# andrewcsmith/vox_box.rs

Hardware: AMD Instinct MI355X
Metric: frames/sec (pitch+LPC+formants), 48 kHz 25 ms/10 ms hop, 1→8 MI355X (higher is better)
Workload: dtype f64

## Files before the change

vox_box.rs_amd/csrc/k_spectral.hip:

```cpp
#include "vbx_spectral_1200.hpp"

namespace vbx {

static size_t spectral_lds_bytes(int n) {
    size_t need = (size_t)pitch_refine_lds_bytes(n);
    const size_t t2_end = (size_t)SP_T2_LDS_OFFSET + 60 * sizeof(double2);
    if (t2_end > need) need = t2_end;
    return (need + 15) & ~(size_t)15;
}

int spectral_plan(int n) {
    static const int min_n = [] { const char *e = getenv("VBX_SPECTRAL_MIN_N"); return e ? atoi(e) : SPECTRAL_MIN_N; }();
    if (n < min_n || n < 64) return SPECTRAL_PLAN_NONE;
    if (n <= 1024) return SPECTRAL_PLAN_1024;
    if (n <= SP_N) return SPECTRAL_PLAN_1200;
    if (n <= 2048) return SPECTRAL_PLAN_2048;
    if (n <= 4096) return SPECTRAL_PLAN_4096;
    return SPECTRAL_PLAN_NONE;
}

int spectral_plan_nc(int plan) {
    return plan == SPECTRAL_PLAN_1200 ? SP_N : plan == SPECTRAL_PLAN_1024 ? 1024 : plan == SPECTRAL_PLAN_2048 ? 2048 :
           plan == SPECTRAL_PLAN_4096 ? 4096 : 0;
}

int spectral_tab_complex(int plan) {
    return plan == SPECTRAL_PLAN_1200 ? SPECTRAL_TAB_COMPLEX : spectral_pow2_tab_complex(plan);
}

void spectral_fill_tab(int plan, double *h) {
    if (plan != SPECTRAL_PLAN_1200) { spectral_pow2_fill_tab(plan, h); return; }
    const long double two_pi = 6.283185307179586476925286766559005768L;
    size_t o = 0;
    auto put = [&](long num, long den) {
        const long double ang = two_pi * (long double)(num % den) / (long double)den;
        h[o++] = (double)cosl(ang); h[o++] = (double)(-sinl(ang));
    };
    for (long np = 0; np < 60; np++) for (long ka = 0; ka < 20; ka++) put(np * ka, 1200);
    for (long c = 0; c < 3; c++) for (long kb = 0; kb < 20; kb++) put(c * kb, 60);
    for (long m = 0; m <= 600; m++) put(m, 2400);
}

bool spectral_supported(int n, int lpc_order, int mfcc_nb, int mfcc_b_lo, int num_coeffs) {
    const int plan = spectral_plan(n);
    if (plan == SPECTRAL_PLAN_NONE) return false;
    if (lpc_order != 0 && lpc_order != SP_LPC_P) return false;
    if (num_coeffs != 0 && ((2 * spectral_plan_nc(plan)) % n != 0 || (n & 1) || num_coeffs > 64 || mfcc_nb < 1 || mfcc_b_lo < 0 || mfcc_b_lo + mfcc_nb > n / 2)) return false;
    return true;
}

int spectral_plan_mfcc(int n) {
    const int plan = spectral_plan(n);
    if (plan == SPECTRAL_PLAN_NONE) return plan;
    if ((2 * spectral_plan_nc(plan)) % n == 0) return plan;
    if (n <= SP_N && (2 * SP_N) % n == 0 && !(n & 1)) return SPECTRAL_PLAN_1200;
    return plan;
}
bool spectral_supported_plan(int plan, int n, int lpc_order, int mfcc_nb, int mfcc_b_lo, int num_coeffs) {
    if (plan == SPECTRAL_PLAN_NONE || n > spectral_plan_nc(plan)) return false;
    if (lpc_order != 0 && lpc_order != SP_LPC_P) return false;
    if (num_coeffs != 0 && ((2 * spectral_plan_nc(plan)) % n != 0 || (n & 1) || num_coeffs > 64 || mfcc_nb < 1 || mfcc_b_lo < 0 || mfcc_b_lo + mfcc_nb > n / 2)) return false;
    return true;
}

static void mfcc_interp_geom(int plan, long *M, int *nt, int *lds_cap) {
    *M = 2L * spectral_plan_nc(plan);
    *nt = plan == SPECTRAL_PLAN_4096 ? 128 : 64;
    *lds_cap = (plan == SPECTRAL_PLAN_1200 || plan == SPECTRAL_PLAN_1024) ? (160 * 1024) / 11 : plan == SPECTRAL_PLAN_2048 ? (160 * 1024) / 7 : (160 * 1024) / 4;
}
static int mfcc_interp_slots(int plan, int nb) { long M; int nt, cap; mfcc_interp_geom(plan, &M, &nt, &cap); return (nb + nt - 1) / nt; }

int mfcc_interp_taps(int plan, int n) {
    long M; int nt, cap; mfcc_interp_geom(plan, &M, &nt, &cap);
    const double tau = 0.5 - (double)n / (2.0 * (double)M);
#ifdef VBX_EXP_INTERP_FEWER_TAPS
    return tau >= 0.36 ? 24 : tau >= 0.268 ? 32 : MFCC_INTERP_MAX_TAPS;
#endif
    return tau >= 0.401 ? 24 : tau >= 0.298 ? 32 : MFCC_INTERP_MAX_TAPS;
}

size_t mfcc_interp_table_bytes(int plan, int nb) {
    long M; int nt, cap; mfcc_interp_geom(plan, &M, &nt, &cap);
    const size_t slots = (size_t)mfcc_interp_slots(plan, nb);
    return (size_t)(M / 4 + 1) * 16 + slots * (MFCC_INTERP_MAX_TAPS / 2) * nt * 16 + slots * nt * 4;
}
size_t mfcc_interp_coef_offset(int plan) { return (size_t)(2L * spectral_plan_nc(plan) / 4 + 1) * 16; }
size_t mfcc_interp_j0_offset(int plan, int nb) {
    long M; int nt, cap; mfcc_interp_geom(plan, &M, &nt, &cap);
    return mfcc_interp_coef_offset(plan) + (size_t)mfcc_interp_slots(plan, nb) * (MFCC_INTERP_MAX_TAPS / 2) * nt * 16;
}

bool mfcc_interp_fill(int plan, int n, int b_lo, int nb, void *h_table, mfcc_interp_t *d) {
    if (plan == SPECTRAL_PLAN_NONE) return false;
    long M; int NT, cap;
    mfcc_interp_geom(plan, &M, &NT, &cap);
    const long quarter = M / 4;
    if (n < 2 || 2L * n > M || M % n == 0 || nb < 1 || nb > 4096 || b_lo < 0) return false;
    const int SL = mfcc_interp_slots(plan, nb);
    const int W = mfcc_interp_taps(plan, n), HT = W / 2;
    const long double pi = 3.141592653589793238462643383279502884L;
    const long double tau = 0.5L - (long double)n / (2.0L * (long double)M);
    const long double beta = pi * tau * (long double)W;
    auto sinhc = [](long double s) { return s < 1e-6L ? 1.0L + s * s / 6.0L : sinhl(s) / s; };
    const long double norm = sinhc(beta);
    char *base = static_cast<char *>(h_table);
    double *rot = reinterpret_cast<double *>(base);
    double *coef = reinterpret_cast<double *>(base + mfcc_interp_coef_offset(plan));
    int32_t *j0t = reinterpret_cast<int32_t *>(base + mfcc_interp_j0_offset(plan, nb));
    for (long j = 0; j <= quarter; j++) {
        const long double ang = 2.0L * pi * (long double)((j * (long)(n - 1)) % (2 * M)) / (long double)(2 * M);
        rot[2 * j] = (double)cosl(ang); rot[2 * j + 1] = (double)sinl(ang);
    }
    long jmin = 1L << 40, jmax = -(1L << 40);
    for (int i = 0; i < nb; i++) {
        const long first = ((long)(b_lo + i) * M) / n - W / 2 + 1;
        if (first < jmin) jmin = first;
        if (first + W - 1 > jmax) jmax = first + W - 1;
    }
    if (jmax > quarter || jmin < -quarter) return false;
    for (int i = 0; i < NT * SL; i++) {
        const int u = i / NT, th = i % NT;
        const long k = b_lo + i;
        const long first = (i < nb) ? (k * M) / n - W / 2 + 1 : jmin;
        j0t[i] = (int32_t)(first - jmin);
        for (int t = 0; t < W; t++) {
            long double c = 0.0L;
            if (i < nb) {
                const long num = k * M - (first + t) * (long)n;
                if (num == 0) c = 1.0L;
                else {
                    const long double nu = (long double)num / (long double)n;
                    long r = num % (2L * n); if (r < 0) r += 2L * n;
                    const long double sn = sinl(pi * (long double)r / (long double)n);
                    const long double arg = beta * beta - (2.0L * pi * tau * nu) * (2.0L * pi * tau * nu);
                    const long double bump = sinhc(arg > 0.0L ? sqrtl(arg) : 0.0L) / norm;
                    c = sn / (pi * nu) * bump;
                }
            }
            coef[(((size_t)u * HT + t / 2) * NT + th) * 2 + (t & 1)] = (double)c;
        }
    }
    const int zn = (int)(jmax - jmin + 1), nbp = (nb + 1) & ~1;
    d->jmin = (int)jmin; d->jmax = (int)jmax; d->taps = W;
    d->pu_off = 2 * zn;
    d->lds_bytes = (2 * zn + 2 * nbp + 64) * 8;
    d->rot = nullptr; d->coef = nullptr; d->j0 = nullptr;
    return d->lds_bytes <= cap;
}

bool spectral_list_parked(const spectral_launch_t &L) {
    const bool rows16 = (((uintptr_t)L.out_cand) & 15) == 0 && (L.cand_ld & 1) == 0;
    return L.plan == SPECTRAL_PLAN_1200 && pitch_full_list_bytes(L.n, L.kmax) != 0 && L.kmax >= pitch_full_list_entries(L.n) &&
           L.out_r == nullptr && !L.mfcc_only && rows16;
}

int launch_analyze(hipStream_t s, const spectral_launch_t &L) {
    if (L.x.kind != SAMPLE_F64 && (L.plan != SPECTRAL_PLAN_1200 || L.n != SP_N)) return -1;
    spectral_args_t a;
    a.frames = static_cast<const double *>(L.x.p);
    a.n_frames = L.F; a.stride = L.stride; a.window = L.window; a.lag_window = L.lag_window;
    a.tab = reinterpret_cast<const double2 *>(L.tab);
    a.n = L.n;
    a.pp.sample_rate = L.sample_rate; a.pp.threshold = L.threshold; a.pp.fmin = L.fmin; a.pp.fmax = L.fmax; a.pp.kmax = L.kmax; a.pp.f32 = 0;
    a.out_cand = reinterpret_cast<double *>(L.out_cand); a.cand_ld = L.cand_ld; a.out_count = L.out_count;
    a.pitch_status = L.pitch_status; a.work = L.work;
    a.out_lpc = L.out_lpc; a.lpc_ld = L.lpc_ld;
    a.out_mfcc = L.out_mfcc; a.mfcc_ld = L.mfcc_ld; a.mfcc_status = L.mfcc_status;
    a.bins = L.bins; a.slopes = L.slopes; a.dct = L.dct; a.num_coeffs = L.num_coeffs; a.nb = L.nb;
    a.unsure_list = L.unsure_list; a.unsure_count = L.unsure_count;
    a.out_r = L.out_r; a.n_lags = L.n_lags;
    a.pcm = (L.x.kind == SAMPLE_PCM16 ? SP_FLAG_PCM : 0) | (L.lag_rcp ? SP_FLAG_LAG_RCP : 0) | ((L.mfcc_defer && L.num_coeffs <= 16) ? SP_FLAG_MFCC_DEFER : 0);
    a.mfcc_q = (L.plan != SPECTRAL_PLAN_NONE && L.n > 0) ? (2 * spectral_plan_nc(L.plan)) / L.n : 2;
    a.ip = mfcc_interp_t{};
    if (L.plan != SPECTRAL_PLAN_1200) return launch_analyze_pow2(s, L, a);
    const dim3 grid((unsigned)L.F), block(64);
    const size_t base = spectral_lds_bytes(L.n);
    size_t extra = pitch_full_list_bytes(L.n, L.kmax);
    a.pp.full_off = extra ? (int)base : 0;
    if (spectral_list_parked(L)) { a.pp.full_off = -1; extra = 0; }
    const size_t lds = base + extra;
    const bool lpc = L.out_lpc != nullptr, mf = L.out_mfcc != nullptr;
    if (L.mfcc_only) {
        if (L.interp && L.n != SP_N) {
            a.ip = L.ip;
            const size_t li = spectral_lds_bytes(0) > (size_t)L.ip.lds_bytes ? spectral_lds_bytes(0) : (((size_t)L.ip.lds_bytes + 15) & ~(size_t)15);
            hipLaunchKernelGGL((analyze_kernel<false, true, false, SP_MFCC_ONLY_INTERP>), grid, block, li, s, a);
        } else hipLaunchKernelGGL((analyze_kernel<false, true, true, SP_MFCC_ONLY>), grid, block, spectral_lds_bytes(0), s, a);
        return 0;
    }
    if (L.out_r != nullptr) {
        if (L.n == SP_N) hipLaunchKernelGGL((analyze_kernel<false, false, true, SP_AC_ONLY>), grid, block, spectral_lds_bytes(0), s, a);
        else hipLaunchKernelGGL((analyze_kernel<false, false, false, SP_AC_ONLY>), grid, block, spectral_lds_bytes(0), s, a);
        return 0;
    }
    static const bool want3 = [] { const char *e = getenv("VBX_SPECTRAL_W3"); return e == nullptr || atoi(e) != 0; }();
    const bool w3 = want3 && extra == 0 && 12 * lds <= 160 * 1024;
    if (L.x.kind == SAMPLE_F32) {
        launch_analyze_f32in(s, a, (unsigned)L.F, lds, lpc, mf, w3);
        return 0;
    }
#define VBX_SP_LAUNCH(LPC_, MF_, FULL_)                                                                              \
    do {                                                                                                              \
        if (w3) hipLaunchKernelGGL((analyze_kernel<LPC_, MF_, FULL_, SP_ANALYZE, 3>), grid, block, lds, s, a);        \
        else hipLaunchKernelGGL((analyze_kernel<LPC_, MF_, FULL_>), grid, block, lds, s, a);                          \
    } while (0)
    if (L.interp && mf && L.n != SP_N) {
        a.ip = L.ip;
        const size_t li = lds > (size_t)L.ip.lds_bytes ? lds : (((size_t)L.ip.lds_bytes + 15) & ~(size_t)15);
        const bool w3i = want3 && extra == 0 && 12 * li <= 160 * 1024;
        if (lpc) { if (w3i) hipLaunchKernelGGL((analyze_kernel<true, true, false, SP_ANALYZE_INTERP, 3>), grid, block, li, s, a);
                   else hipLaunchKernelGGL((analyze_kernel<true, true, false, SP_ANALYZE_INTERP>), grid, block, li, s, a); }
        else { if (w3i) hipLaunchKernelGGL((analyze_kernel<false, true, false, SP_ANALYZE_INTERP, 3>), grid, block, li, s, a);
               else hipLaunchKernelGGL((analyze_kernel<false, true, false, SP_ANALYZE_INTERP>), grid, block, li, s, a); }
    } else if (L.n != SP_N) {
        if (lpc && mf) VBX_SP_LAUNCH(true, true, false);
        else if (mf) VBX_SP_LAUNCH(false, true, false);
        else if (lpc) VBX_SP_LAUNCH(true, false, false);
        else VBX_SP_LAUNCH(false, false, false);
    } else if (lpc && mf) VBX_SP_LAUNCH(true, true, true);
    else if (lpc) VBX_SP_LAUNCH(true, false, true);
    else if (mf) VBX_SP_LAUNCH(false, true, true);
    else VBX_SP_LAUNCH(false, false, true);
#undef VBX_SP_LAUNCH
    return 0;
}

}
```

vox_box.rs_amd/csrc/k_spectral_f32in.hip:

```cpp
#include "vbx_spectral_1200.hpp"

namespace vbx {

void launch_analyze_f32in(hipStream_t s, const spectral_args_t &a, unsigned grid, size_t lds, bool lpc, bool mfcc, bool waves3) {
    const dim3 g(grid), b(64);
#define VBX_SP32_LAUNCH(LPC_, MF_)                                                                                \
    do {                                                                                                           \
        if (waves3) hipLaunchKernelGGL((analyze_kernel<LPC_, MF_, true, SP_ANALYZE, 3, float>), g, b, lds, s, a);                     \
        else hipLaunchKernelGGL((analyze_kernel<LPC_, MF_, true, SP_ANALYZE, VBX_SPECTRAL_WAVES, float>), g, b, lds, s, a);           \
    } while (0)
    if (lpc && mfcc) VBX_SP32_LAUNCH(true, true);
    else if (lpc) VBX_SP32_LAUNCH(true, false);
    else if (mfcc) VBX_SP32_LAUNCH(false, true);
    else VBX_SP32_LAUNCH(false, false);
#undef VBX_SP32_LAUNCH
}

}
```

vox_box.rs_amd/csrc/vbx_api.hip:

```cpp
#include "vbx_ctx.hpp"

#include <cmath>
#include <cstdio>
#include <cstdlib>
#include <cstring>
#include <dlfcn.h>
#include <string>
#include <vector>

using namespace vbx;

extern "C" const double VBX_MALE_FORMANT_ESTIMATES[4] = {320., 1440., 2760., 3200.};
extern "C" const double VBX_FEMALE_FORMANT_ESTIMATES[4] = {480., 1760., 3200., 3520.};

namespace {

thread_local std::string g_last_error;

}

namespace vbx {

int fail(vbx_ctx *ctx, int code, const std::string &msg) {
    g_last_error = msg;
    if (ctx) ctx->last_error = msg;
    return code;
}

int check_launch(vbx_ctx *ctx, const char *what) {
    hipError_t e = hipGetLastError();
    if (e != hipSuccess) return fail(ctx, VBX_E_RUNTIME, std::string(what) + " launch: " + hipGetErrorString(e));
    return VBX_SUCCESS;
}

int ws_get(vbx_ctx *ctx, int slot, size_t bytes, void **out) {
    if (bytes == 0) bytes = 16;
    if (ctx->ws_bytes[slot] < bytes) {
        if (ctx->ws[slot]) {
            VBX_HIP(ctx, hipStreamSynchronize(ctx->stream));
            if (ctx->side) VBX_HIP(ctx, hipStreamSynchronize(ctx->side));
            if (ctx->trk) VBX_HIP(ctx, hipStreamSynchronize(ctx->trk));
            VBX_HIP(ctx, hipFree(ctx->ws[slot]));
            ctx->ws[slot] = nullptr; ctx->ws_bytes[slot] = 0;
        }
        size_t cap = bytes + bytes / 8;
        VBX_HIP(ctx, hipMalloc(&ctx->ws[slot], cap));
        ctx->ws_bytes[slot] = cap;
    }
    *out = ctx->ws[slot];
    return VBX_SUCCESS;
}

int get_bins_dev(vbx_ctx *ctx, size_t n, size_t k, double lo, double hi, double sr,
                 const int32_t **out, std::vector<int32_t> &host_bins, bool &bad) {
    mel_bins_host(n, k, lo, hi, sr, host_bins, bad);
    for (size_t i = 0; i + 1 < host_bins.size(); i++) if (host_bins[i + 1] < host_bins[i]) bad = true;
    if (host_bins.back() > (int32_t)n) bad = true;
    VBX_HIP(ctx, ctx->tables.bins(n, k, lo, hi, sr, host_bins, out));
    return VBX_SUCCESS;
}

int check_frames(vbx_ctx *ctx, const char *fn, const void *x, size_t n_frames, size_t frame_len, size_t stride,
                 size_t max_len) {
    if (!ctx) return fail(nullptr, VBX_E_INVALID, std::string(fn) + ": null context");
    ctx->lpc_list_armed = false;
    ctx->path_last = false;
    ctx->shard.live = false;
    if (n_frames == 0) return 1;
    if (!x) return fail(ctx, VBX_E_INVALID, std::string(fn) + ": null frame pointer");
    if (frame_len < 1 || frame_len > max_len)
        return fail(ctx, VBX_E_INVALID, std::string(fn) + ": frame_len must be in [1, " + std::to_string(max_len) + "]");
    if (stride < 1) return fail(ctx, VBX_E_INVALID, std::string(fn) + ": stride must be >= 1");
    if (n_frames > 0x7fffffffull) return fail(ctx, VBX_E_INVALID, std::string(fn) + ": too many frames for one launch");
    return VBX_SUCCESS;
}

int stage_upload(vbx_ctx *ctx, int which, int ws_slot, const void *h_src, size_t bytes, hipStream_t st, void **d_out) {
    void *d = nullptr;
    const bool grown = ctx->ws_bytes[ws_slot] < bytes;
    int rc = ws_get(ctx, ws_slot, bytes, &d);
    if (rc != VBX_SUCCESS) return rc;
    *d_out = d;
    std::vector<char> &have = ctx->staged[which];
    if (!grown && have.size() == bytes && std::memcmp(have.data(), h_src, bytes) == 0) return VBX_SUCCESS;
    if (!ctx->stage_ev[which]) VBX_HIP(ctx, hipEventCreateWithFlags(&ctx->stage_ev[which], hipEventDisableTiming));
    else VBX_HIP(ctx, hipEventSynchronize(ctx->stage_ev[which]));
    if (ctx->stage_cap[which] < bytes) {
        if (ctx->stage[which]) VBX_HIP(ctx, hipHostFree(ctx->stage[which]));
        ctx->stage[which] = nullptr; ctx->stage_cap[which] = 0;
        VBX_HIP(ctx, hipHostMalloc(&ctx->stage[which], bytes + bytes / 2, hipHostMallocDefault));
        ctx->stage_cap[which] = bytes + bytes / 2;
    }
    std::memcpy(ctx->stage[which], h_src, bytes);
    VBX_HIP(ctx, hipMemcpyAsync(d, ctx->stage[which], bytes, hipMemcpyHostToDevice, st));
    VBX_HIP(ctx, hipEventRecord(ctx->stage_ev[which], st));
    have.assign((const char *)h_src, (const char *)h_src + bytes);
    return VBX_SUCCESS;
}

int upload_segments(vbx_ctx *ctx, hipStream_t st, const int64_t *h_seg, size_t n_seg, size_t n_frames, const int64_t **d_seg, size_t *n_out) {
    if (h_seg == nullptr || n_seg == 0) { *d_seg = nullptr; *n_out = 1; return VBX_SUCCESS; }
    if (h_seg[0] != 0) return fail(ctx, VBX_E_INVALID, "seg_start[0] must be 0");
    for (size_t i = 1; i < n_seg; i++)
        if (h_seg[i] < h_seg[i - 1] || (size_t)h_seg[i] > n_frames) return fail(ctx, VBX_E_INVALID, "seg_start must ascend within [0, n_frames]");
    void *d = nullptr;
    int rc = stage_upload(ctx, 0, vbx_ctx::WS_SEG, h_seg, n_seg * sizeof(int64_t), st, &d);
    if (rc != VBX_SUCCESS) return rc;
    *d_seg = (const int64_t *)d; *n_out = n_seg;
    return VBX_SUCCESS;
}

int upload_estimates(vbx_ctx *ctx, hipStream_t st, const vbx_resonance *h_est, size_t n_est, const res_t **d_est) {
    void *d = nullptr;
    int rc = stage_upload(ctx, 1, vbx_ctx::WS_EST, h_est, n_est * sizeof(vbx_resonance), st, &d);
    if (rc != VBX_SUCCESS) return rc;
    *d_est = (const res_t *)d;
    return VBX_SUCCESS;
}

}

extern "C" {

int vbx_internal_fail(vbx_ctx *ctx, int code, const char *msg) { return fail(ctx, code, msg ? msg : ""); }
void *vbx_internal_stream(vbx_ctx *ctx) { return ctx ? (void *)ctx->stream : nullptr; }

int vbx_abi_version(void) { return VBX_ABI_VERSION; }

int vbx_ctx_set_lpc_policy(vbx_ctx *ctx, int policy) {
    VBX_REQUIRE(ctx, ctx != nullptr, "null context");
    VBX_REQUIRE(ctx, policy == VBX_LPC_POLICY_EXACT || policy == VBX_LPC_POLICY_PLAIN || policy == VBX_LPC_POLICY_REFERENCE,
                "vbx_ctx_set_lpc_policy: unknown policy");
    ctx->lpc_policy = policy;
    return VBX_SUCCESS;
}

int vbx_ctx_get_lpc_policy(const vbx_ctx *ctx, int *h_policy) {
    if (!ctx || !h_policy) return fail(const_cast<vbx_ctx *>(ctx), VBX_E_INVALID, "vbx_ctx_get_lpc_policy: null argument");
    *h_policy = ctx->lpc_policy;
    return VBX_SUCCESS;
}

int vbx_ctx_create(vbx_ctx **out, int device, void *hip_stream) {
    if (!out) return fail(nullptr, VBX_E_INVALID, "vbx_ctx_create: null out");
    *out = nullptr;
    int count = 0;
    hipError_t e = hipGetDeviceCount(&count);
    if (e != hipSuccess || count <= 0)
        return fail(nullptr, VBX_E_NODEVICE, "vbx_ctx_create: no HIP device (this library has no CPU fallback)");
    if (device < 0 || device >= count) return fail(nullptr, VBX_E_INVALID, "vbx_ctx_create: bad device ordinal");
    VBX_HIP(nullptr, hipSetDevice(device));
    hipDeviceProp_t prop;
    VBX_HIP(nullptr, hipGetDeviceProperties(&prop, device));
    if (std::strncmp(prop.gcnArchName, "gfx950", 6) != 0)
        return fail(nullptr, VBX_E_NODEVICE, std::string("vbx_ctx_create: device is ") + prop.gcnArchName + ", kernels are built for gfx950 only");
    vbx_ctx *ctx = new vbx_ctx();
    ctx->device = device;
    ctx->arch = prop.gcnArchName;
    ctx->cu_count = prop.multiProcessorCount;
    { const char *e = std::getenv("VBX_MFCC_GOERTZEL"); ctx->mfcc_force_goertzel = e && e[0] == '1'; }
    { const char *e = std::getenv("VBX_MFCC_DFT2"); ctx->mfcc_force_dft2 = e && e[0] == '1'; }
    { const char *e = std::getenv("VBX_MFCC_MFMA"); ctx->mfcc_force_mfma = e && e[0] == '1'; }
    { const char *e = std::getenv("VBX_MFCC_CZT"); ctx->mfcc_czt = e ? (e[0] == '1' ? 1 : 0) : -1; }
    { const char *e = std::getenv("VBX_MFCC_DEFER"); ctx->mfcc_defer = (e && e[0] == '0') ? 0 : 1; }
    { const char *e = std::getenv("VBX_LPC_EXACT"); ctx->lpc_policy = (e && e[0] == '0') ? VBX_LPC_POLICY_PLAIN : VBX_LPC_POLICY_EXACT; }
    { const char *e = std::getenv("VBX_POW2_SPLIT"); ctx->pow2_split = e ? (e[0] == '0' ? 0 : 1) : -1; }
    { const char *e = std::getenv("VBX_MFCC_INTERP"); ctx->mfcc_interp = e ? (e[0] == '0' ? 0 : 1) : -1; }
    { const char *e = std::getenv("VBX_MFCC_CZT_SPLIT"); ctx->mfcc_czt_split = e != nullptr && e[0] == '1'; }
    { const char *e = std::getenv("VBX_PITCH_CURVE_CUT"); ctx->pitch_whole_curve = e != nullptr && e[0] == '0'; }
    if (const char *e = std::getenv("VBX_ROCTX"); e != nullptr && e[0] == '1') {
        void *h = dlopen("librocprofiler-sdk-roctx.so", RTLD_NOW | RTLD_GLOBAL);
        if (h == nullptr) h = dlopen("libroctx64.so", RTLD_NOW | RTLD_GLOBAL);
        if (h != nullptr) {
            ctx->roctx_push = reinterpret_cast<int (*)(const char *)>(dlsym(h, "roctxRangePushA"));
            ctx->roctx_pop = reinterpret_cast<int (*)()>(dlsym(h, "roctxRangePop"));
            if (ctx->roctx_push == nullptr || ctx->roctx_pop == nullptr) { ctx->roctx_push = nullptr; ctx->roctx_pop = nullptr; }
        }
    }
    { const char *e = std::getenv("VBX_PITCH_MFMA"); ctx->pitch_force_mfma = e && e[0] == '1'; }
    if (hip_stream) { ctx->stream = (hipStream_t)hip_stream; ctx->owns_stream = false; }
    else {
        e = hipStreamCreateWithFlags(&ctx->stream, hipStreamNonBlocking);
        if (e != hipSuccess) { delete ctx; return fail(nullptr, VBX_E_RUNTIME, "hipStreamCreate failed"); }
        ctx->owns_stream = true;
    }
    hipEventCreate(&ctx->t0);
    hipEventCreate(&ctx->t1);
    *out = ctx;
    return VBX_SUCCESS;
}

void vbx_ctx_destroy(vbx_ctx *ctx) {
    if (!ctx) return;
    hipSetDevice(ctx->device);
    hipStreamSynchronize(ctx->stream);
    for (int i = 0; i < vbx_ctx::WS_N; i++) if (ctx->ws[i]) hipFree(ctx->ws[i]);
    if (ctx->pitch_work) hipFree(ctx->pitch_work);
    if (ctx->stitch_state) hipFree(ctx->stitch_state);
    ctx->tables.clear();
    for (auto &r : ctx->recs) { hipEventDestroy(r.a); hipEventDestroy(r.b); }
    if (ctx->side) { hipStreamSynchronize(ctx->side); hipStreamDestroy(ctx->side); }
    if (ctx->ev_fork) hipEventDestroy(ctx->ev_fork);
    if (ctx->ev_join) hipEventDestroy(ctx->ev_join);
    if (ctx->ev_peak) hipEventDestroy(ctx->ev_peak);
    for (auto &e : ctx->ev_slice) if (e) hipEventDestroy(e);
    if (ctx->ev_trk) hipEventDestroy(ctx->ev_trk);
    if (ctx->trk) { hipStreamSynchronize(ctx->trk); hipStreamDestroy(ctx->trk); }
    if (ctx->copy) { hipStreamSynchronize(ctx->copy); hipStreamDestroy(ctx->copy); }
    for (int i = 0; i < 2; i++) {
        if (ctx->host_raw[i]) hipFree(ctx->host_raw[i]);
        if (ctx->host_ready[i]) hipEventDestroy(ctx->host_ready[i]);
        if (ctx->host_freed[i]) hipEventDestroy(ctx->host_freed[i]);
    }
    for (int i = 0; i < vbx_ctx::N_STAGE; i++) { if (ctx->stage[i]) hipHostFree(ctx->stage[i]); if (ctx->stage_ev[i]) hipEventDestroy(ctx->stage_ev[i]); }
    if (ctx->t0) hipEventDestroy(ctx->t0);
    if (ctx->t1) hipEventDestroy(ctx->t1);
    if (ctx->owns_stream) hipStreamDestroy(ctx->stream);
    delete ctx;
}

int vbx_sync(vbx_ctx *ctx) {
    if (!ctx) return fail(nullptr, VBX_E_INVALID, "vbx_sync: null context");
    VBX_HIP(ctx, hipStreamSynchronize(ctx->stream));
    if (ctx->side) VBX_HIP(ctx, hipStreamSynchronize(ctx->side));
    if (ctx->trk) VBX_HIP(ctx, hipStreamSynchronize(ctx->trk));
    if (ctx->copy) VBX_HIP(ctx, hipStreamSynchronize(ctx->copy));
    return VBX_SUCCESS;
}

const char *vbx_last_error(const vbx_ctx *ctx) { return ctx ? ctx->last_error.c_str() : g_last_error.c_str(); }

int vbx_device_info(const vbx_ctx *ctx, char *h_name, size_t name_cap, int *h_cu_count) {
    if (!ctx) return fail(nullptr, VBX_E_INVALID, "vbx_device_info: null context");
    if (h_name && name_cap) { std::strncpy(h_name, ctx->arch.c_str(), name_cap - 1); h_name[name_cap - 1] = 0; }
    if (h_cu_count) *h_cu_count = ctx->cu_count;
    return VBX_SUCCESS;
}

int vbx_malloc(vbx_ctx *ctx, void **out_dptr, size_t bytes) {
    VBX_REQUIRE(ctx, ctx && out_dptr, "null argument");
    VBX_HIP(ctx, hipSetDevice(ctx->device));
    VBX_HIP(ctx, hipMalloc(out_dptr, bytes ? bytes : 16));
    return VBX_SUCCESS;
}
int vbx_free(vbx_ctx *ctx, void *dptr) {
    VBX_REQUIRE(ctx, ctx != nullptr, "null context");
    if (dptr) { VBX_HIP(ctx, hipStreamSynchronize(ctx->stream)); VBX_HIP(ctx, hipFree(dptr)); }
    return VBX_SUCCESS;
}
int vbx_memcpy_h2d(vbx_ctx *ctx, void *dst, const void *h_src, size_t bytes) {
    VBX_REQUIRE(ctx, ctx && (bytes == 0 || (dst && h_src)), "null argument");
    if (bytes == 0) return VBX_SUCCESS;
    VBX_HIP(ctx, hipMemcpyAsync(dst, h_src, bytes, hipMemcpyHostToDevice, ctx->stream));
    VBX_HIP(ctx, hipStreamSynchronize(ctx->stream));
    return VBX_SUCCESS;
}
int vbx_memcpy_d2h(vbx_ctx *ctx, void *h_dst, const void *src, size_t bytes) {
    VBX_REQUIRE(ctx, ctx && (bytes == 0 || (h_dst && src)), "null argument");
    if (bytes == 0) return VBX_SUCCESS;
    VBX_HIP(ctx, hipMemcpyAsync(h_dst, src, bytes, hipMemcpyDeviceToHost, ctx->stream));
    VBX_HIP(ctx, hipStreamSynchronize(ctx->stream));
    return VBX_SUCCESS;
}
int vbx_memset(vbx_ctx *ctx, void *dst, int value, size_t bytes) {
    VBX_REQUIRE(ctx, ctx && (bytes == 0 || dst), "null argument");
    if (bytes == 0) return VBX_SUCCESS;
    VBX_HIP(ctx, hipMemsetAsync(dst, value, bytes, ctx->stream));
    return VBX_SUCCESS;
}

int vbx_timer_begin(vbx_ctx *ctx) {
    VBX_REQUIRE(ctx, ctx != nullptr, "null context");
    VBX_HIP(ctx, hipEventRecord(ctx->t0, ctx->stream));
    return VBX_SUCCESS;
}
int vbx_timer_end(vbx_ctx *ctx, float *h_ms) {
    VBX_REQUIRE(ctx, ctx && h_ms, "null argument");
    VBX_HIP(ctx, hipEventRecord(ctx->t1, ctx->stream));
    VBX_HIP(ctx, hipEventSynchronize(ctx->t1));
    VBX_HIP(ctx, hipEventElapsedTime(h_ms, ctx->t0, ctx->t1));
    return VBX_SUCCESS;
}

static int prof_flush(vbx_ctx *ctx) {
    if (ctx->recs.empty()) return VBX_SUCCESS;
    VBX_HIP(ctx, hipStreamSynchronize(ctx->stream));
    if (ctx->side) VBX_HIP(ctx, hipStreamSynchronize(ctx->side));
    if (ctx->trk) VBX_HIP(ctx, hipStreamSynchronize(ctx->trk));
    for (auto &r : ctx->recs) {
        float ms = 0.f;
        if (hipEventElapsedTime(&ms, r.a, r.b) == hipSuccess) {
            auto &acc = ctx->prof_acc[r.name];
            acc.first += ms; acc.second += 1;
            ctx->prof_stream[r.name] = (r.stream == ctx->stream) ? 0 : (r.stream == ctx->side) ? 1 : 2;
        }
        hipEventDestroy(r.a); hipEventDestroy(r.b);
    }
    ctx->recs.clear();
    return VBX_SUCCESS;
}
int vbx_profile_enable(vbx_ctx *ctx, int on) {
    VBX_REQUIRE(ctx, ctx != nullptr, "null context");
    int rc = prof_flush(ctx);
    ctx->prof = on != 0;
    return rc;
}
int vbx_profile_reset(vbx_ctx *ctx) {
    VBX_REQUIRE(ctx, ctx != nullptr, "null context");
    int rc = prof_flush(ctx);
    ctx->prof_acc.clear();
    ctx->prof_stream.clear();
    if (ctx->pitch_work)
        VBX_HIP(ctx, hipMemsetAsync(ctx->pitch_work, 0, PITCH_WORK_WORDS * sizeof(unsigned long long), ctx->stream));
    return rc;
}
int vbx_profile_pitch_work(vbx_ctx *ctx, uint64_t *h_out4) {
    VBX_REQUIRE(ctx, ctx && h_out4, "null argument");
// ... 16 lines not shown
    return VBX_SUCCESS;
}
int vbx_profile_get(vbx_ctx *ctx, const char *kernel_name, double *h_total_ms, long *h_launches) {
    VBX_REQUIRE(ctx, ctx && kernel_name, "null argument");
    int rc = prof_flush(ctx);
    if (rc != VBX_SUCCESS) return rc;
    auto it = ctx->prof_acc.find(kernel_name);
    if (h_total_ms) *h_total_ms = (it == ctx->prof_acc.end()) ? 0.0 : it->second.first;
    if (h_launches) *h_launches = (it == ctx->prof_acc.end()) ? 0 : it->second.second;
    return VBX_SUCCESS;
}
int vbx_profile_stream(vbx_ctx *ctx, const char *kernel_name, int *h_stream) {
    VBX_REQUIRE(ctx, ctx && kernel_name && h_stream, "null argument");
    int rc = prof_flush(ctx);
    if (rc != VBX_SUCCESS) return rc;
    auto it = ctx->prof_stream.find(kernel_name);
    *h_stream = (it == ctx->prof_stream.end()) ? -1 : it->second;
    return VBX_SUCCESS;
}
int vbx_profile_names(vbx_ctx *ctx, char *h_buf, size_t cap) {
    VBX_REQUIRE(ctx, ctx && h_buf && cap, "null argument");
    int rc = prof_flush(ctx);
    if (rc != VBX_SUCCESS) return rc;
    std::string s;
    for (auto &kv : ctx->prof_acc) { s += kv.first; s += '\n'; }
    std::strncpy(h_buf, s.c_str(), cap - 1); h_buf[cap - 1] = 0;
    return VBX_SUCCESS;
}



static int run_autocorrelate(vbx_ctx *ctx, hipStream_t st, const double *x, size_t n_frames, size_t frame_len, size_t stride,
                             const double *window, size_t n_lags, double *out) {
    if (frame_len > VBX_MAX_FRAME_LEN) {
        void *w = nullptr;
        int rc = ws_get(ctx, vbx_ctx::WS_LONG, autocorr_long_scratch_bytes((long)n_frames, (long)frame_len, (long)n_lags), &w);
        if (rc != VBX_SUCCESS) return rc;
        Prof p(ctx, "autocorr_long", st);
        launch_autocorr_long(st, x, (long)n_frames, (long)frame_len, (long)stride, window, (long)n_lags, out, (double *)w);
        return VBX_SUCCESS;
    }
    if (fewlags_supported((int)frame_len, (int)n_lags, false)) {
        Prof p(ctx, "autocorr_fewlags", st);
        launch_autocorr_fewlags(st, x, (long)n_frames, (int)frame_len, (long)stride, window, (int)n_lags, 0, out, nullptr);
    } else if (!ctx->pitch_force_mfma && spectral_plan((int)frame_len) != SPECTRAL_PLAN_NONE &&
               (n_lags >= SPECTRAL_AC_MIN_LAGS || frame_len >= 1024)) {
        const double *tab = nullptr;
        spectral_launch_t L{};
        L.plan = spectral_plan((int)frame_len); L.n = (int)frame_len;
        VBX_HIP(ctx, ctx->tables.spectral(L.plan, &tab));
        L.x = x; L.F = (long)n_frames; L.stride = (long)stride; L.window = window; L.tab = tab;
        L.out_r = out; L.n_lags = (int)n_lags;
        Prof p(ctx, "autocorr_fft", st);
        launch_analyze(st, L);
    } else {
        Prof p(ctx, "autocorr_tiles", st);
        launch_autocorr_tiles(st, x, (long)n_frames, (int)frame_len, (long)stride, window, (int)n_lags, out);
    }
    return VBX_SUCCESS;
}

int vbx_autocorrelate_f64(vbx_ctx *ctx, const double *x, size_t n_frames, size_t frame_len,
                          size_t stride, const double *window, size_t n_lags, double *out) {
    int rc = check_frames(ctx, __func__, x, n_frames, frame_len, stride, VBX_MAX_LONG_FRAME_LEN);
    if (rc != VBX_SUCCESS) return rc < 0 ? rc : VBX_SUCCESS;
    VBX_REQUIRE(ctx, out != nullptr, "null output");
    VBX_REQUIRE(ctx, n_lags >= 1 && n_lags <= frame_len, "n_lags must be in [1, frame_len] (the reference panics beyond)");
    VBX_HIP(ctx, hipSetDevice(ctx->device));
    if (ctx->lpc_policy == VBX_LPC_POLICY_REFERENCE) {
        VBX_REQUIRE(ctx, frame_len <= 0x7fffffffull, "frame_len too large");
        { Prof p(ctx, "autocorr_ref"); launch_lpc_ref(ctx->stream, x, (long)n_frames, (int)frame_len, (long)stride, window, (int)n_lags, 0, 0,
                                                      out, (long)n_lags, nullptr, 0); }
        return check_launch(ctx, __func__);
    }
    rc = run_autocorrelate(ctx, ctx->stream, x, n_frames, frame_len, stride, window, n_lags, out);
    if (rc != VBX_SUCCESS) return rc;
    return check_launch(ctx, __func__);
}

int vbx_normalize_f64(vbx_ctx *ctx, double *data, size_t n_rows, size_t n) {
    VBX_REQUIRE(ctx, ctx != nullptr, "null context");
    if (n_rows == 0) return VBX_SUCCESS;
    VBX_REQUIRE(ctx, data && n >= 1 && n <= 0x7fffffff && n_rows <= 0x7fffffff, "bad argument");
    VBX_HIP(ctx, hipSetDevice(ctx->device));
    { Prof p(ctx, "normalize_rows"); launch_normalize_rows(ctx->stream, data, (long)n_rows, (int)n); }
    return check_launch(ctx, __func__);
}

int vbx_interpolate_sinc_f64(vbx_ctx *ctx, const double *y, size_t ylen, long offset, size_t nx,
                             const double *xs, size_t m, size_t max_depth, double *out, int32_t *status) {
    VBX_REQUIRE(ctx, ctx != nullptr, "null context");
    if (m == 0) return VBX_SUCCESS;
    VBX_REQUIRE(ctx, y && xs && out && ylen >= 1 && ylen <= 0x7fffffff && m <= 0x7fffffff, "bad argument");
    VBX_REQUIRE(ctx, max_depth <= 0x3fffffff && nx <= 0x3fffffff && ylen <= 0x3fffffff &&
                offset > -0x3fffffffL && offset < 0x3fffffffL, "depth / nx / offset / ylen too large");
    VBX_HIP(ctx, hipSetDevice(ctx->device));
    { Prof p(ctx, "sinc_points"); launch_sinc_points(ctx->stream, y, (int)ylen, offset, (long)nx, xs, (long)m, (long)max_depth, out, status); }
    return check_launch(ctx, __func__);
}

int vbx_improve_extremum_ex_f64(vbx_ctx *ctx, const double *y, size_t ylen, long offset, size_t nx,
                                const double *ixmid, size_t m, int interpolation, size_t depth, int is_max,
                                double *out_xy, int32_t *status) {
    VBX_REQUIRE(ctx, ctx != nullptr, "null context");
    if (m == 0) return VBX_SUCCESS;
    VBX_REQUIRE(ctx, y && ixmid && out_xy && ylen >= 1 && ylen <= 0x7fffffff && m <= 0x7fffffff, "bad argument");
    VBX_REQUIRE(ctx, interpolation >= VBX_INTERP_NONE && interpolation <= VBX_INTERP_SINC, "interpolation must be NONE, PARABOLIC or SINC");
    VBX_REQUIRE(ctx, depth <= 0x3fffffff && nx <= 0x3fffffff && ylen <= 0x3fffffff &&
                offset > -0x3fffffffL && offset < 0x3fffffffL, "depth / nx / offset / ylen too large");
    VBX_HIP(ctx, hipSetDevice(ctx->device));
    { Prof p(ctx, "extremum_points"); launch_extremum_points(ctx->stream, y, (int)ylen, offset, (long)nx, ixmid, (long)m, (long)depth, out_xy, status, interpolation, is_max ? 1 : 0); }
    return check_launch(ctx, __func__);
}

int vbx_improve_extremum_f64(vbx_ctx *ctx, const double *y, size_t ylen, long offset, size_t nx,
                             const double *ixmid, size_t m, size_t depth, double *out_xy, int32_t *status) {
    return vbx_improve_extremum_ex_f64(ctx, y, ylen, offset, nx, ixmid, m, VBX_INTERP_SINC, depth, 1, out_xy, status);
}

}

namespace vbx {

int launch_spectral(vbx_ctx *ctx, hipStream_t st, spectral_launch_t &L, const char *prof_name) {
    void *w = nullptr;
    int rc = ws_get(ctx, vbx_ctx::WS_UNSURE, ((size_t)L.F + 4) * sizeof(int32_t), &w);
    if (rc != VBX_SUCCESS) return rc;
    L.unsure_count = (int32_t *)w;
    L.unsure_list = (int32_t *)w + 4;
    VBX_HIP(ctx, hipMemsetAsync(L.unsure_count, 0, sizeof(int32_t), st));
    L.lpc_list = nullptr; L.lpc_count = nullptr;
    if (L.out_lpc != nullptr && ctx->lpc_policy == VBX_LPC_POLICY_EXACT) {
        void *lw = nullptr;
        rc = ws_get(ctx, vbx_ctx::WS_LPC_LIST, ((size_t)L.F + 4) * sizeof(int32_t), &lw);
        if (rc != VBX_SUCCESS) return rc;
        L.lpc_count = (int32_t *)lw; L.lpc_list = (int32_t *)lw + 4;
        VBX_HIP(ctx, hipMemsetAsync(L.lpc_count, 0, sizeof(int32_t), st));
        ctx->lpc_list_armed = true;
    }
    L.curve_ws = nullptr; L.curve_ws_bytes = 0;
    const size_t rowb = (ctx->pow2_split != 0 && !L.whole_curve && !L.mfcc_only && L.out_r == nullptr && pitch_full_list_bytes(L.n, L.kmax) == 0)
                            ? spectral_split_row_bytes(L.n, L.sample_rate, L.fmin) : 0;
    if (rowb) {
        const size_t frames = (size_t)L.F < 131072 ? (size_t)L.F : 131072;
        const size_t need = (frames < 1024 ? 1024 : frames) * rowb + 64;
        void *cw = nullptr;
        if (ctx->curve_failed_bytes == 0 || need < ctx->curve_failed_bytes) {
            const std::string before = ctx->last_error;
            if (ws_get(ctx, vbx_ctx::WS_CURVE, need, &cw) == VBX_SUCCESS) { L.curve_ws = (double *)cw; L.curve_ws_bytes = need; }
            else { (void)hipGetLastError(); ctx->curve_failed_bytes = need; ctx->last_error = before; g_last_error = before; }
        }
    }
    L.mfcc_defer = L.out_mfcc != nullptr && !L.mfcc_only && L.num_coeffs >= 1 && L.num_coeffs <= 16 && ctx->mfcc_defer && L.plan == SPECTRAL_PLAN_1200;
    { Prof p(ctx, prof_name, st); ctx->last_spectral_split = launch_analyze(st, L); }
    if (L.mfcc_defer && L.out_lpc == nullptr) { Prof p(ctx, "mfcc_rows", st); launch_mfcc_rows(st, L.out_mfcc, L.F, L.mfcc_ld, L.num_coeffs, L.dct); }
    {
        Prof p(ctx, "pitch_direct_fallback", st);
        const int cus = ctx->cu_count > 0 ? ctx->cu_count : 256;
        const int grid = pitch_lds_bytes(L.n) > 24 * 1024 ? cus : cus * 4;
        launch_pitch_list(st, L.unsure_list, L.unsure_count, grid, L.x, L.n, L.stride, L.window, L.lag_window,
                          L.sample_rate, L.threshold, L.fmin, L.fmax, L.kmax, L.out_cand, L.cand_ld, L.out_count,
                          L.pitch_status, L.work);
    }
    if (L.out_lpc != nullptr) {
        { Prof p(ctx, "lpc_rows", st);
          launch_levinson_rows_probe(st, L.out_lpc, L.F, L.lpc_ld, SPECTRAL_LPC_ORDER, L.out_lpc, L.lpc_ld, L.lpc_list, L.lpc_count,
                                     L.mfcc_defer ? L.out_mfcc : nullptr, L.mfcc_ld, L.num_coeffs, L.dct); }
        if (L.lpc_list != nullptr) {
            Prof p(ctx, "lpc_exact_list", st);
            const int cus = ctx->cu_count > 0 ? ctx->cu_count : 256;
            launch_lpc_exact_list(st, L.lpc_list, L.lpc_count, cus, L.x, L.n, L.stride, L.window, SPECTRAL_LPC_ORDER, L.out_lpc, L.lpc_ld);
        }
        if (ctx->lpc_policy == VBX_LPC_POLICY_REFERENCE) {
            Prof p(ctx, "lpc_ref", st);
            launch_lpc_ref(st, L.x, L.F, L.n, L.stride, L.window, SPECTRAL_LPC_ORDER + 1, SPECTRAL_LPC_ORDER, 0, nullptr, 0, L.out_lpc, L.lpc_ld);
        }
    }
    return check_launch(ctx, "launch_spectral");
}

const char *pitch_shape_error(size_t frame_len, size_t kmax) {
    const size_t kcap = frame_len > VBX_MAX_FRAME_LEN ? VBX_PITCH_MAX_CANDIDATES(frame_len) : (size_t)VBX_MAX_PITCH_CANDIDATES;
    if (!(kmax >= 1 && kmax <= kcap)) return "kmax must be in [1, VBX_MAX_PITCH_CANDIDATES] (long frames: [1, frame_len / 4 + 2])";
    if (frame_len < 4) return "frame_len must be >= 4";
    if (frame_len > VBX_MAX_FRAME_LEN) return frame_len <= 0x3fffffff ? nullptr : "frame_len too large for the lag curve's 32-bit indices";
    if (pitch_lds_bytes((int)frame_len) + pitch_full_list_bytes((int)frame_len, (int)kmax) + 16 > 160 * 1024) return "frame does not fit the LDS";
    return nullptr;
}

int run_pitch(vbx_ctx *ctx, hipStream_t st, const double *x, size_t n_frames, size_t frame_len, size_t stride,
              const double *window, double sample_rate, double threshold, double fmin, double fmax,
              size_t kmax, vbx_pitch *out_cand, size_t cand_ld, int32_t *out_count, int32_t *status) {
    VBX_REQUIRE(ctx, out_cand != nullptr, "null output");
    if (const char *e = pitch_shape_error(frame_len, kmax)) return fail(ctx, VBX_E_INVALID, std::string(__func__) + ": " + e);
    VBX_REQUIRE(ctx, cand_ld >= 2 * kmax && cand_ld % 2 == 0, "candidate rows must hold kmax entries and their leading dimension must be even");
    const double *lagw = nullptr; bool lag_rcp = false;
    int rc;
    VBX_HIP(ctx, ctx->tables.window(VBX_WINDOW_HANNING_LAG, frame_len, &lagw, &lag_rcp));
    if (frame_len > VBX_MAX_FRAME_LEN) {
        size_t per = (size_t(1) << 31) / pitch_long_scratch_bytes(1, (long)frame_len);
        if (per < 1) per = 1;
        if (per > n_frames) per = n_frames;
        void *w2 = nullptr;
        rc = ws_get(ctx, vbx_ctx::WS_LONG2, pitch_long_scratch_bytes((long)per, (long)frame_len), &w2);
        if (rc != VBX_SUCCESS) return rc;
        for (size_t f0 = 0; f0 < n_frames; f0 += per) {
            const size_t m = (n_frames - f0 < per) ? n_frames - f0 : per;
            double *r = pitch_long_r(w2);
            rc = run_autocorrelate(ctx, st, x + f0 * stride, m, frame_len, stride, window, frame_len, r);
            if (rc != VBX_SUCCESS) return rc;
            { Prof p(ctx, "normalize_rows", st); launch_normalize_rows(st, r, (long)m, (int)frame_len); }
            ctx->last_pitch_form = 100;
            { Prof p(ctx, "pitch_long", st);
              launch_pitch_long(st, (long)m, (long)frame_len, lagw, sample_rate, threshold, fmin, fmax, (int)kmax,
                                (double *)out_cand + f0 * cand_ld, (long)cand_ld, out_count ? out_count + f0 : nullptr,
                                status ? status + f0 : nullptr, w2); }
        }
        return check_launch(ctx, "vbx_pitch_f64");
    }
    if (ctx->prof && !ctx->pitch_work) {
        const size_t wb = PITCH_WORK_WORDS * sizeof(unsigned long long);
        VBX_HIP(ctx, hipMalloc((void **)&ctx->pitch_work, wb));
        VBX_HIP(ctx, hipMemsetAsync(ctx->pitch_work, 0, wb, st));
    }
    if (!ctx->pitch_force_mfma && spectral_supported((int)frame_len, 0, 0, 0, 0)) {
        const double *tab = nullptr;
        spectral_launch_t L{};
        L.plan = spectral_plan((int)frame_len); L.n = (int)frame_len;
        VBX_HIP(ctx, ctx->tables.spectral(L.plan, &tab));
        L.x = x; L.F = (long)n_frames; L.stride = (long)stride; L.window = window; L.lag_window = lagw; L.tab = tab;
        L.lag_rcp = lag_rcp;
        L.sample_rate = sample_rate; L.threshold = threshold; L.fmin = fmin; L.fmax = fmax; L.kmax = (int)kmax;
        L.whole_curve = ctx->pitch_whole_curve;
        L.out_cand = (pitch_t *)out_cand; L.cand_ld = (long)cand_ld; L.out_count = out_count; L.pitch_status = status;
        L.work = ctx->prof ? ctx->pitch_work : nullptr;
        ctx->last_pitch_form = 100 * (3 + L.plan) + (pitch_full_list_bytes(L.n, L.kmax) == 0 ? 0 : spectral_list_parked(L) ? 2 : 1);
        return launch_spectral(ctx, st, L, "pitch");
    }
    {
        ctx->last_pitch_form = 200 + (pitch_full_list_bytes((int)frame_len, (int)kmax) == 0 ? 0 : 1);
        Prof p(ctx, "pitch", st);
        launch_pitch(st, x, (long)n_frames, (int)frame_len, (long)stride, window, lagw, sample_rate, threshold,
                     fmin, fmax, (int)kmax, (pitch_t *)out_cand, (long)cand_ld, out_count, status,
                     ctx->prof ? ctx->pitch_work : nullptr);
    }
    return check_launch(ctx, "vbx_pitch_f64");
}

}

extern "C" {

int vbx_pitch_f64(vbx_ctx *ctx, const double *x, size_t n_frames, size_t frame_len, size_t stride,
                  const double *window, double sample_rate, double threshold, double fmin, double fmax,
                  size_t kmax, vbx_pitch *out_cand, int32_t *out_count, int32_t *status) {
    int rc = check_frames(ctx, __func__, x, n_frames, frame_len, stride, VBX_MAX_LONG_FRAME_LEN);
    if (rc != VBX_SUCCESS) return rc < 0 ? rc : VBX_SUCCESS;
    VBX_HIP(ctx, hipSetDevice(ctx->device));
    return run_pitch(ctx, ctx->stream, x, n_frames, frame_len, stride, window, sample_rate, threshold, fmin, fmax,
                     kmax, out_cand, 2 * kmax, out_count, status);
}


int vbx_lpc_mut_f64(vbx_ctx *ctx, const double *r, size_t n_frames, size_t r_stride, size_t n_coeffs, double *out_ac,
                    double *out_kc) {
    VBX_REQUIRE(ctx, ctx != nullptr, "null context");
    if (n_frames == 0) return VBX_SUCCESS;
    VBX_REQUIRE(ctx, r && out_ac, "null argument");
    VBX_REQUIRE(ctx, n_coeffs >= 1 && n_coeffs <= VBX_MAX_LPC_ORDER && r_stride >= n_coeffs + 1, "bad order / stride");
    VBX_REQUIRE(ctx, n_frames <= 0x7fffffffull, "too many rows");
    VBX_HIP(ctx, hipSetDevice(ctx->device));
    if (ctx->lpc_policy == VBX_LPC_POLICY_REFERENCE) {
        Prof p(ctx, "levinson_ref_rows");
        launch_levinson_ref_rows(ctx->stream, r, (long)n_frames, (long)r_stride, (int)n_coeffs, out_ac, (long)n_coeffs + 1, out_kc);
        return check_launch(ctx, __func__);
    }
    { Prof p(ctx, "levinson_rows"); launch_levinson_rows(ctx->stream, r, (long)n_frames, (long)r_stride, (int)n_coeffs, out_ac, (long)n_coeffs + 1, out_kc); }
    return check_launch(ctx, __func__);
}

int vbx_lpc_f64(vbx_ctx *ctx, const double *r, size_t n_frames, size_t r_stride, size_t n_coeffs, double *out) {
    return vbx_lpc_mut_f64(ctx, r, n_frames, r_stride, n_coeffs, out, nullptr);
}

}

namespace vbx {

bool lpc_order_ok(size_t frame_len, size_t n_coeffs) {
    return n_coeffs >= 1 && n_coeffs <= VBX_MAX_LPC_ORDER && n_coeffs + 1 <= frame_len;
}

int run_autocorr_lpc(vbx_ctx *ctx, hipStream_t st, const double *x, size_t n_frames, size_t frame_len,
                     size_t stride, const double *window, size_t n_coeffs, int normalize,
                     double *out_r, double *out_lpc, size_t lpc_ld) {
    VBX_REQUIRE(ctx, out_r || out_lpc, "both outputs null");
    VBX_REQUIRE(ctx, lpc_order_ok(frame_len, n_coeffs), "bad order");
    VBX_REQUIRE(ctx, lpc_ld >= n_coeffs + 1, "LPC rows must hold n_coeffs + 1 entries");
    const int n_lags = (int)n_coeffs + 1;
    int rc;
    if (ctx->lpc_policy == VBX_LPC_POLICY_REFERENCE) {
        VBX_REQUIRE(ctx, frame_len <= 0x7fffffffull, "frame_len too large");
        { Prof p(ctx, "lpc_ref", st);
          launch_lpc_ref(st, x, (long)n_frames, (int)frame_len, (long)stride, window, n_lags, (int)n_coeffs, normalize, out_r, n_lags,
                         out_lpc, (long)lpc_ld); }
        return check_launch(ctx, "vbx_autocorr_lpc_f64");
    }
// ... 273 lines not shown
                                           const int32_t *res_count, const int64_t *h_seg_start, size_t n_segments,
                                           const vbx_resonance *h_est_init, size_t n_est,
                                           const int32_t *frame_status, vbx_resonance *out) {
    VBX_REQUIRE(ctx, ctx != nullptr, "null context");
    if (n_frames == 0) return VBX_SUCCESS;
    VBX_REQUIRE(ctx, res && res_count && h_est_init && out, "null argument");
    VBX_REQUIRE(ctx, n_res >= 1 && n_res <= 0x7fffffff && n_est >= 1 && n_est <= VBX_FORMANT_SLOTS, "bad size");
    VBX_HIP(ctx, hipSetDevice(ctx->device));
    const int64_t *d_seg = nullptr; size_t nseg = 1; const res_t *d_est = nullptr;
    int rc = upload_segments(ctx, ctx->stream, h_seg_start, n_segments, n_frames, &d_seg, &nseg);
    if (rc != VBX_SUCCESS) return rc;
    rc = upload_estimates(ctx, ctx->stream, h_est_init, n_est, &d_est);
    if (rc != VBX_SUCCESS) return rc;
    rc = run_tracker(ctx, ctx->stream, tracker_wants_chunks(h_seg_start, n_segments, n_frames), (const res_t *)res, (long)n_frames,
                     (int)n_res, res_count, d_seg, (long)nseg, d_est, (int)n_est, frame_status, (res_t *)out, 2 * (long)n_est);
    if (rc != VBX_SUCCESS) return rc;
    return check_launch(ctx, __func__);
}

static int run_formant_resonances(vbx_ctx *ctx, hipStream_t stm, const double *coeffs, long F, int p, double sample_rate,
                                  res_t *res, int32_t *cnt, int32_t *st, frame_map_t map = frame_map_t{0, 0, 0}) {
    if (formant_resonances_fast_supported(p)) {
        void *w = nullptr;
        int rc = ws_get(ctx, vbx_ctx::WS_ROOTS_LIST, 4 * sizeof(int32_t), &w);
        if (rc != VBX_SUCCESS) return rc;
        int32_t *redo = (int32_t *)w;
        ctx->roots_list_count = redo;
        if (map.seg_len == 0 || map.t0 == 0) VBX_HIP(ctx, hipMemsetAsync(redo, 0, sizeof(int32_t), stm));
        Prof pr(ctx, "formant_resonances", stm);
        launch_formant_resonances_fast(stm, coeffs, F, p, sample_rate, res, cnt, st, map, redo);
        return VBX_SUCCESS;
    }
    ctx->roots_list_count = nullptr;
    Prof pr(ctx, "formant_resonances", stm);
    launch_formant_resonances(stm, coeffs, F, p, sample_rate, res, cnt, st, map);
    return VBX_SUCCESS;
}

}

namespace vbx {

int run_find_formants(vbx_ctx *ctx, hipStream_t stm, frames_t x, size_t n_frames, size_t frame_len,
                      size_t stride, double sample_rate, size_t n_coeffs,
                      const int64_t *h_seg_start, size_t n_segments,
                      const vbx_resonance *h_est_init, size_t n_est,
                      vbx_resonance *out_formants, size_t formants_ld, vbx_resonance *out_res, int32_t *out_res_count,
                      double *out_coeffs, int32_t *status,
                      const resample_plan_t *rp ) {
    VBX_REQUIRE(ctx, h_est_init && out_formants, "null argument");
    if (rp) frame_len = rp->m;
    VBX_REQUIRE(ctx, burg_order_ok(frame_len, n_coeffs), "frame_len must be >= 2, order in [1, 62]");
    VBX_REQUIRE(ctx, n_est >= 1 && n_est <= VBX_FORMANT_SLOTS, "n_est must be in [1, 6]");
    VBX_REQUIRE(ctx, formants_ld >= 2 * n_est && formants_ld % 2 == 0, "formant rows must be 16-byte aligned and hold n_est entries");
    const long F = (long)n_frames; const int p = (int)n_coeffs;
    int rc;
    void *w = nullptr;
    double *coeffs = out_coeffs;
    if (!coeffs) { rc = ws_get(ctx, vbx_ctx::WS_COEFFS, n_frames * n_coeffs * sizeof(double), &w); if (rc) return rc; coeffs = (double *)w; }
    res_t *res = (res_t *)out_res;
    if (!res) { rc = ws_get(ctx, vbx_ctx::WS_RES, n_frames * VBX_MAX_RESONANCES * sizeof(vbx_resonance), &w); if (rc) return rc; res = (res_t *)w; }
    int32_t *cnt = out_res_count;
    if (!cnt) { rc = ws_get(ctx, vbx_ctx::WS_COUNT, n_frames * sizeof(int32_t), &w); if (rc) return rc; cnt = (int32_t *)w; }
    int32_t *st = status;
    if (!st) { rc = ws_get(ctx, vbx_ctx::WS_STATUS, n_frames * sizeof(int32_t), &w); if (rc) return rc; st = (int32_t *)w; }
    const double *hann = nullptr;
    VBX_HIP(ctx, ctx->tables.window(VBX_WINDOW_HANNING_PERIODIC, frame_len, &hann));
    const int64_t *d_seg = nullptr; size_t nseg = 1; const res_t *d_est = nullptr;
    rc = upload_segments(ctx, stm, h_seg_start, n_segments, n_frames, &d_seg, &nseg);
    if (rc != VBX_SUCCESS) return rc;
    rc = upload_estimates(ctx, stm, h_est_init, n_est, &d_est);
    if (rc != VBX_SUCCESS) return rc;
    long seg_len = 0;
    const bool chunked = tracker_wants_chunks(h_seg_start, n_segments, n_frames);
    if (!chunked && h_seg_start != nullptr && n_segments >= 64 && F >= 65536 && !(rp && !rp->direct)) {
        seg_len = (n_segments > 1) ? (long)h_seg_start[1] : 0;
        for (size_t i = 0; i < n_segments && seg_len > 0; i++) if (h_seg_start[i] != (int64_t)i * seg_len) seg_len = 0;
        if (seg_len > 0 && ((long)(n_segments - 1) * seg_len >= F || (long)n_segments * seg_len < F || seg_len < 64)) seg_len = 0;
    }
    static const int want_slices = [] { const char *e = getenv("VBX_FF_SLICES"); const int v = e ? atoi(e) : 6; return v < 1 ? 1 : (v > 8 ? 8 : v); }();
    const int n_slices = seg_len > 0 ? want_slices : 1;
    const long tc = (seg_len + n_slices - 1) / n_slices;
    ctx->last_track.res = res; ctx->last_track.cnt = cnt; ctx->last_track.st = st; ctx->last_track.F = F;
    ctx->last_track.n_est = (int)n_est; ctx->last_track.out = (res_t *)out_formants; ctx->last_track.out_ld = (long)formants_ld;
    if (n_slices == 1) {
        rc = run_burg(ctx, stm, x, F, (int)frame_len, (long)stride, hann, p, coeffs, st, frame_map_t{0, 0, 0}, rp);
        if (rc != VBX_SUCCESS) return rc;
        rc = run_formant_resonances(ctx, stm, coeffs, F, p, sample_rate, res, cnt, st);
        if (rc != VBX_SUCCESS) return rc;
        rc = run_tracker(ctx, stm, chunked, res, F, VBX_MAX_RESONANCES, cnt, d_seg, (long)nseg, d_est, (int)n_est, st,
                         (res_t *)out_formants, (long)formants_ld);
        if (rc != VBX_SUCCESS) return rc;
        return check_launch(ctx, "vbx_find_formants_f64");
    }
    if (!ctx->trk) {
        VBX_HIP(ctx, hipStreamCreateWithFlags(&ctx->trk, hipStreamNonBlocking));
        for (auto &e : ctx->ev_slice) VBX_HIP(ctx, hipEventCreateWithFlags(&e, hipEventDisableTiming));
        VBX_HIP(ctx, hipEventCreateWithFlags(&ctx->ev_trk, hipEventDisableTiming));
    }
    for (int j = 0; j < n_slices && j * tc < seg_len; j++) {
        const frame_map_t map{seg_len, j * tc, (seg_len - j * tc < tc) ? seg_len - j * tc : tc};
        rc = run_burg(ctx, stm, x, F, (int)frame_len, (long)stride, hann, p, coeffs, st, map, rp);
        if (rc != VBX_SUCCESS) return rc;
        rc = run_formant_resonances(ctx, stm, coeffs, F, p, sample_rate, res, cnt, st, map);
        if (rc != VBX_SUCCESS) return rc;
        VBX_HIP(ctx, hipEventRecord(ctx->ev_slice[j], stm));
        VBX_HIP(ctx, hipStreamWaitEvent(ctx->trk, ctx->ev_slice[j], 0));
        { Prof pr(ctx, "tracker", ctx->trk); launch_tracker(ctx->trk, res, F, VBX_MAX_RESONANCES, cnt, d_seg, (long)nseg, d_est, (int)n_est, st, (res_t *)out_formants, (long)formants_ld, j * tc, tc); }
    }
    VBX_HIP(ctx, hipEventRecord(ctx->ev_trk, ctx->trk));
    VBX_HIP(ctx, hipStreamWaitEvent(stm, ctx->ev_trk, 0));
    return check_launch(ctx, "vbx_find_formants_f64");
}

}

extern "C" {

int vbx_find_formants_f64(vbx_ctx *ctx, const double *x, size_t n_frames, size_t frame_len,
                          size_t stride, double sample_rate, size_t n_coeffs,
                          const int64_t *h_seg_start, size_t n_segments,
                          const vbx_resonance *h_est_init, size_t n_est,
                          vbx_resonance *out_formants, vbx_resonance *out_res, int32_t *out_res_count,
                          double *out_coeffs, int32_t *status) {
    int rc = check_frames(ctx, __func__, x, n_frames, frame_len, stride, VBX_MAX_LONG_FRAME_LEN);
    if (rc != VBX_SUCCESS) return rc < 0 ? rc : VBX_SUCCESS;
    VBX_HIP(ctx, hipSetDevice(ctx->device));
    return run_find_formants(ctx, ctx->stream, x, n_frames, frame_len, stride, sample_rate, n_coeffs, h_seg_start, n_segments,
                             h_est_init, n_est, out_formants, 2 * n_est, out_res, out_res_count, out_coeffs, status);
}

int vbx_internal_track_stitch(vbx_ctx *ctx, void *stream, vbx_resonance *formants, size_t n_frames, size_t formants_ld,
                              size_t first, size_t stop, const double *d_state_in, int32_t *d_changed) {
    VBX_REQUIRE(ctx, ctx != nullptr, "null context");
    VBX_REQUIRE(ctx, formants && d_state_in, "null argument");
    const auto &lt = ctx->last_track;
    VBX_REQUIRE(ctx, lt.res != nullptr && lt.out == (res_t *)formants && lt.F == (long)n_frames && lt.out_ld == (long)formants_ld,
                "the formant rows are not the ones the last find_formants / analyze_frames call on this context wrote");
    VBX_REQUIRE(ctx, first <= stop && stop <= n_frames, "need first <= stop <= n_frames");
    VBX_HIP(ctx, hipSetDevice(ctx->device));
    hipStream_t st = stream ? (hipStream_t)stream : ctx->stream;
    { Prof p(ctx, "tracker_stitch", st);
      launch_tracker_stitch(st, lt.res, lt.F, VBX_MAX_RESONANCES, lt.cnt, lt.n_est, lt.st, lt.out, lt.out_ld, (long)first, (long)stop,
                            d_state_in, d_changed); }
    return check_launch(ctx, "vbx_track_stitch_f64");
}

int vbx_track_stitch_f64(vbx_ctx *ctx, vbx_resonance *formants, size_t n_frames, size_t formants_ld, size_t first, size_t stop,
                         const vbx_resonance *d_state_in, int32_t *d_changed) {
    return vbx_internal_track_stitch(ctx, nullptr, formants, n_frames, formants_ld, first, stop, (const double *)d_state_in, d_changed);
}

int vbx_internal_last_spectral_split(vbx_ctx *ctx) { return ctx ? ctx->last_spectral_split : 0; }
int vbx_internal_last_mfcc_interp(vbx_ctx *ctx) { return ctx ? ctx->last_mfcc_interp : 0; }
int vbx_internal_last_mfcc_form(vbx_ctx *ctx) { return ctx ? ctx->last_mfcc_form : 0; }
int vbx_internal_last_pitch_form(vbx_ctx *ctx) { return ctx ? ctx->last_pitch_form : 0; }

int vbx_internal_mfcc_interp_table(size_t frame_len, int b_lo, int nb, int32_t *desc, void *buf, size_t cap, size_t *need) {
    if (!desc || !need || frame_len < 2 || frame_len > VBX_MAX_FRAME_LEN || nb < 1 || nb > 4096) return VBX_E_INVALID;
    const int plan = spectral_plan_mfcc((int)frame_len);
    if (plan == SPECTRAL_PLAN_NONE || (2 * spectral_plan_nc(plan)) % (int)frame_len == 0) return 0;
    const size_t bytes = mfcc_interp_table_bytes(plan, nb);
    *need = bytes;
    std::vector<char> h(bytes, 0);
    mfcc_interp_t d{};
    if (!mfcc_interp_fill(plan, (int)frame_len, b_lo, nb, h.data(), &d)) return 0;
    const int nt = plan == SPECTRAL_PLAN_4096 ? 128 : 64;
    desc[0] = 4 * spectral_plan_nc(plan) / 2; desc[1] = nt; desc[2] = (nb + nt - 1) / nt; desc[3] = d.taps;
    desc[4] = d.jmin; desc[5] = d.jmax; desc[6] = (int32_t)mfcc_interp_coef_offset(plan); desc[7] = (int32_t)mfcc_interp_j0_offset(plan, nb);
    if (buf && cap >= bytes) std::memcpy(buf, h.data(), bytes);
    return 1;
}

int vbx_internal_mfcc_table_plans(size_t frame_len, int b_lo, int nb, int32_t *out) {
    if (!out || frame_len < 2 || frame_len > VBX_MAX_FRAME_LEN || b_lo < 0 || nb < 1 || nb > 4096) return VBX_E_INVALID;
    const mfcc_mplan_t m = mfcc_mfma_plan((int)frame_len, b_lo, nb);
    const mfcc_plan_t p = mfcc_plan((int)frame_len, nb);
    const int32_t v[14] = {m.ok, m.n1, m.n2, m.k2, m.mt, m.ntd, m.ntm, m.src0, m.src1, p.ok, p.n1, p.n2, p.nc, p.tm};
    std::memcpy(out, v, sizeof v);
    return VBX_SUCCESS;
}


}

namespace vbx {

int run_mfcc(vbx_ctx *ctx, hipStream_t stm, const double *x, size_t n_frames, size_t frame_len, size_t stride,
             const double *window, size_t num_coeffs, double lo_hz, double hi_hz,
             double sample_rate, double *out, size_t out_ld, int32_t *status) {
    VBX_REQUIRE(ctx, out != nullptr, "null output");
    VBX_REQUIRE(ctx, num_coeffs >= 1 && num_coeffs <= 64, "num_coeffs must be in [1, 64]");
    VBX_REQUIRE(ctx, out_ld >= num_coeffs, "output rows must hold num_coeffs entries");
    std::vector<int32_t> hb; bool bad = false; const int32_t *d_bins = nullptr;
    ctx->last_mfcc_interp = 0;
    ctx->last_mfcc_form = 0;
    int rc = get_bins_dev(ctx, frame_len, num_coeffs, lo_hz, hi_hz, sample_rate, &d_bins, hb, bad);
    if (rc != VBX_SUCCESS) return rc;
    if (bad) {
        ctx->last_mfcc_form = 8;
        { Prof p(ctx, "fill_rows", stm); launch_fill_rows(stm, out, (long)n_frames, (int)num_coeffs, (long)out_ld, 0.0, status, VBX_FRAME_ERR_PANIC); }
        return check_launch(ctx, "vbx_mfcc_f64");
    }
    const int nb = hb.back() - hb.front();
    const double *dct = nullptr, *slopes = nullptr;
    VBX_HIP(ctx, ctx->tables.dct(num_coeffs, &dct));
    VBX_HIP(ctx, ctx->tables.slopes(frame_len, num_coeffs, lo_hz, hi_hz, sample_rate, hb, &slopes));
    if (frame_len > VBX_MAX_FRAME_LEN) {
        VBX_REQUIRE(ctx, nb >= 1, "no mel bins");
        const double *tw = nullptr;
        VBX_HIP(ctx, ctx->tables.goertzel(frame_len, hb.front(), nb, &tw));
        void *w = nullptr;
        rc = ws_get(ctx, vbx_ctx::WS_CZT, mfcc_long_scratch_bytes((long)n_frames, nb), &w); if (rc != VBX_SUCCESS) return rc;
        ctx->last_mfcc_form = 7;
        { Prof p(ctx, "mfcc_long", stm);
          launch_mfcc_long(stm, x, (long)n_frames, (long)frame_len, (long)stride, window, tw, d_bins, slopes, dct, (int)num_coeffs, nb, out,
                           (long)out_ld, status, (double *)w); }
        return check_launch(ctx, "vbx_mfcc_f64");
    }
    {
        int plan = spectral_plan((int)frame_len);
        if (frame_len == 2048) plan = SPECTRAL_PLAN_1024; else if (frame_len == 4096) plan = SPECTRAL_PLAN_2048;
        if (!ctx->mfcc_force_goertzel && !ctx->mfcc_force_dft2 && !ctx->mfcc_force_mfma && plan != SPECTRAL_PLAN_NONE &&
            ((int)frame_len == spectral_plan_nc(plan) || (int)frame_len == 2 * spectral_plan_nc(plan)) &&
            num_coeffs <= 64 && nb >= 1 && hb.front() >= 0 && hb.front() + nb <= (int)frame_len / 2) {
            const double *tab = nullptr;
            VBX_HIP(ctx, ctx->tables.spectral(plan, &tab));
            spectral_launch_t L{};
            L.plan = plan; L.n = (int)frame_len; L.mfcc_only = true;
            L.x = x; L.F = (long)n_frames; L.stride = (long)stride; L.window = window; L.tab = tab;
            L.out_mfcc = out; L.mfcc_ld = (long)out_ld; L.mfcc_status = status;
            L.bins = d_bins; L.slopes = slopes; L.dct = dct; L.num_coeffs = (int)num_coeffs; L.nb = nb;
            ctx->last_mfcc_form = 1;
            { Prof p(ctx, "mfcc", stm); launch_analyze(stm, L); }
            return check_launch(ctx, "vbx_mfcc_f64");
        }
    }
    const bool composite_ok = nb > 0 && !ctx->mfcc_force_goertzel;
    const mfcc_mplan_t mp = (composite_ok && !ctx->mfcc_force_dft2 && ctx->mfcc_czt != 1) ? mfcc_mfma_plan((int)frame_len, hb.front(), nb) : mfcc_mplan_t{};
    const mfcc_plan_t pl = (composite_ok && !mp.ok) ? mfcc_plan((int)frame_len, nb) : mfcc_plan_t{false, 0, 0, 0, 0};
    if ((!mp.ok || frame_len >= 1400) && ctx->mfcc_interp != 0 && ctx->mfcc_czt != 1 && !ctx->mfcc_force_goertzel && !ctx->mfcc_force_dft2 && !ctx->mfcc_force_mfma &&
        num_coeffs <= 64 && nb >= 1 && nb <= 4096 && hb.front() >= 0 && hb.front() + nb <= (int)frame_len / 2) {
        const int plan = spectral_plan_mfcc((int)frame_len);
        bool ok = false;
        mfcc_interp_t ip{};
        if (plan != SPECTRAL_PLAN_NONE && (2 * spectral_plan_nc(plan)) % (int)frame_len != 0 && (int)frame_len < spectral_plan_nc(plan)) {
            VBX_HIP(ctx, ctx->tables.interp(plan, (int)frame_len, hb.front(), nb, &ip, &ok));
        }
        if (ok) {
            const double *tab = nullptr;
            VBX_HIP(ctx, ctx->tables.spectral(plan, &tab));
            spectral_launch_t L{};
            L.plan = plan; L.n = (int)frame_len; L.mfcc_only = true; L.interp = true; L.ip = ip;
            ctx->last_mfcc_interp = 1;
            ctx->last_mfcc_form = 2;
            L.x = x; L.F = (long)n_frames; L.stride = (long)stride; L.window = window; L.tab = tab;
            L.out_mfcc = out; L.mfcc_ld = (long)out_ld; L.mfcc_status = status;
            L.bins = d_bins; L.slopes = slopes; L.dct = dct; L.num_coeffs = (int)num_coeffs; L.nb = nb;
            { Prof p(ctx, "mfcc", stm); launch_analyze(stm, L); }
            return check_launch(ctx, "vbx_mfcc_f64");
        }
    }
    const int czt_top = hb.back();
    int czt_plan = (nb >= 1 && hb.front() >= 0 && num_coeffs <= 64) ? mfcc_czt_plan((int)frame_len, czt_top) : SPECTRAL_PLAN_NONE;
    int czt_n1 = 0;
    if (nb >= 1 && hb.front() >= 0 && num_coeffs <= 64 && (czt_plan == SPECTRAL_PLAN_NONE || ctx->mfcc_czt_split)) {
        int n1 = 0;
        const int p2 = mfcc_czt_split_plan((int)frame_len, czt_top, &n1);
        if (p2 != SPECTRAL_PLAN_NONE) { czt_plan = p2; czt_n1 = n1; }
    }
    const bool czt_over_mfma = mp.ok && czt_plan == SPECTRAL_PLAN_2048 && czt_n1 == 0 && frame_len >= 1400 && ctx->mfcc_czt == -1 &&
                               !(ctx->mfcc_force_goertzel || ctx->mfcc_force_dft2 || ctx->mfcc_force_mfma);
    if (!mp.ok || czt_over_mfma) {
        const int top = czt_top;
        const int cplan = czt_plan;
        const bool forced = ctx->mfcc_force_goertzel || ctx->mfcc_force_dft2 || ctx->mfcc_force_mfma;
        const bool want = ctx->mfcc_czt == 1 || czt_over_mfma || (ctx->mfcc_czt == -1 && !forced && frame_len >= 600);
        if (cplan != SPECTRAL_PLAN_NONE && want) {
            const double *tab = nullptr, *chirp = nullptr, *bhat = nullptr;
            VBX_HIP(ctx, ctx->tables.spectral(cplan, &tab));
            VBX_HIP(ctx, ctx->tables.czt(frame_len, top, spectral_plan_nc(cplan), czt_n1, &chirp, &bhat));
            void *cw = nullptr;
            rc = ws_get(ctx, vbx_ctx::WS_CZT, (czt_n1 ? 4 : 2) * (size_t)spectral_plan_nc(cplan) * sizeof(double), &cw); if (rc != VBX_SUCCESS) return rc;
            ctx->last_mfcc_form = 3;
            { Prof p(ctx, "mfcc", stm);
              launch_mfcc_czt(stm, cplan, x, (long)n_frames, (int)frame_len, czt_n1, (long)stride, window, tab, chirp, bhat, d_bins, slopes, dct,
                              (int)num_coeffs, nb, out, (long)out_ld, status, (double *)cw); }
            return check_launch(ctx, "vbx_mfcc_f64");
        }
    }
    if (mp.ok) {
        const double *ctab = nullptr, *twd = nullptr, *twm = nullptr, *wm = nullptr;
        VBX_HIP(ctx, ctx->tables.mfma(frame_len, mp, &ctab, &twd, &twm, &wm));
        ctx->last_mfcc_form = 4;
        Prof p(ctx, "mfcc", stm);
        launch_mfcc_mfma(stm, x, (long)n_frames, (int)frame_len, (long)stride, window, mp, ctab, twd, twm, wm, d_bins,
                         slopes, dct, (int)num_coeffs, out, (long)out_ld, status, nb, ctx->cu_count);
    } else if (pl.ok) {
        const double *ctab = nullptr, *twid = nullptr;
        VBX_HIP(ctx, ctx->tables.dft2(frame_len, pl, &ctab, &twid));
        ctx->last_mfcc_form = 5;
        Prof p(ctx, "mfcc", stm);
        launch_mfcc_dft2(stm, x, (long)n_frames, (int)frame_len, (long)stride, window, pl, ctab, twid, d_bins,
                         slopes, dct, (int)num_coeffs, out, (long)out_ld, status, nb, ctx->cu_count);
    } else {
        VBX_REQUIRE(ctx, mfcc_fits((int)frame_len, nb), "frame / bin range does not fit the LDS");
// ... 183 lines not shown
```

vox_box.rs_amd/csrc/vbx_ctx.hpp:

```cpp
#pragma once

#include "../../include/voxbox_hip.h"
#include "vbx_kernels.hpp"
#include "vbx_host.hpp"
#include "vbx_table_cache.hpp"

#include <hip/hip_runtime.h>

#include <map>
#include <string>
#include <vector>

namespace vbx {

struct ProfRec { std::string name; hipEvent_t a, b; hipStream_t stream; };

struct pp_plan_t {
    pp_par_t P{};
    int G = 4;
    long nch = 0, max_per_seg = 1, n_guessed = 0;
    size_t nseg = 1;
    const int64_t *d_seg_chunk0 = nullptr;
    double *cpk = nullptr;
    uint8_t *map_a = nullptr, *map_b = nullptr;
    long c_first = 0, c_end = 0;
};

}

struct vbx_ctx {
    int device = 0;
    hipStream_t stream = nullptr;
    bool owns_stream = false;
    std::string last_error;
    size_t curve_failed_bytes = 0;
    std::string arch;
    int cu_count = 0;
    enum { WS_COEFFS, WS_RES, WS_COUNT, WS_STATUS, WS_MISC, WS_SEG, WS_EST, WS_UNSURE, WS_F32_IN, WS_F32_OUT, WS_TRK, WS_BURG_LIST, WS_ROOTS_LIST, WS_LONG, WS_LONG2, WS_CZT, WS_CURVE, WS_LPC_LIST, WS_PATH, WS_PATH_TAB, WS_TRACK, WS_EX, WS_HOST, WS_HOST_TYPED, WS_CLIPS_TAB, WS_CLIPS_PLANE, WS_CLIPS_ROWS, WS_CLIPS_LISTS, WS_N };
    void *ws[WS_N] = {nullptr};
    const int32_t *burg_list_count = nullptr;
    const int32_t *roots_list_count = nullptr;
    size_t ws_bytes[WS_N] = {0};
    vbx::device_tables_t tables;
    bool pitch_whole_curve = false;
    bool mfcc_czt_split = false;
    int mfcc_czt = -1;
    int last_mfcc_interp = 0;
    int last_spectral_split = 0;
    int last_mfcc_form = 0;
    int last_pitch_form = 0;
    int mfcc_defer = 1;
    int lpc_policy = VBX_LPC_POLICY_EXACT;
    bool lpc_list_armed = false;
    int pow2_split = -1;
    int mfcc_interp = -1;
    hipEvent_t t0 = nullptr, t1 = nullptr;
    bool prof = false;
    int (*roctx_push)(const char *) = nullptr;
    int (*roctx_pop)() = nullptr;
    std::vector<vbx::ProfRec> recs;
    std::map<std::string, std::pair<double, long>> prof_acc;
    std::map<std::string, int> prof_stream;
    bool pitch_force_mfma = false;
    bool mfcc_force_goertzel = false;
    bool mfcc_force_dft2 = false;
    bool mfcc_force_mfma = false;
    unsigned long long *pitch_work = nullptr;
    hipStream_t side = nullptr;
    hipEvent_t ev_fork = nullptr, ev_join = nullptr;
    hipEvent_t ev_peak = nullptr;
    hipStream_t trk = nullptr;
    hipEvent_t ev_slice[8] = {nullptr}, ev_trk = nullptr;
    enum { N_STAGE = 4 };
    void *stage[N_STAGE] = {nullptr};
    size_t stage_cap[N_STAGE] = {0};
    std::vector<char> staged[N_STAGE];
    hipEvent_t stage_ev[N_STAGE] = {nullptr};
    struct { const vbx::res_t *res = nullptr; const int32_t *cnt = nullptr, *st = nullptr; long F = 0; int n_est = 0;
             vbx::res_t *out = nullptr; long out_ld = 0; } last_track;
    double *stitch_state = nullptr;
    const unsigned long long *path_redone = nullptr;
    bool path_last = false;
    struct { bool live = false, entered = false; vbx::pp_plan_t S; int prev = 0, next = 0; } shard;
    hipStream_t copy = nullptr;
    void *host_raw[2] = {nullptr, nullptr};
    size_t host_raw_bytes = 0;
    hipEvent_t host_ready[2] = {nullptr, nullptr}, host_freed[2] = {nullptr, nullptr};
};

struct vbx_path_stream {
    vbx_ctx *ctx = nullptr;
    size_t kmax = 0, max_pending = 0;
    int G = 4;
    vbx_pitch_path_params pr{};
    double peak_ref = 0.0;
    void *mem = nullptr;
    vbx::pp_online_t O{};
};

extern "C" int vbx_internal_track_stitch(vbx_ctx *ctx, void *stream, vbx_resonance *formants, size_t n_frames, size_t formants_ld,
                                         size_t first, size_t stop, const double *d_state_in, int32_t *d_changed);

namespace vbx {


int fail(vbx_ctx *ctx, int code, const std::string &msg);
int check_launch(vbx_ctx *ctx, const char *what);

#define VBX_HIP(ctx, expr)                                                                     \
    do {                                                                                       \
        hipError_t e_ = (expr);                                                                \
        if (e_ != hipSuccess)                                                                  \
            return vbx::fail(ctx, VBX_E_RUNTIME, std::string(#expr) + ": " + hipGetErrorString(e_)); \
    } while (0)

#define VBX_REQUIRE_FN(ctx, fn, cond, msg) \
    do { if (!(cond)) return vbx::fail(ctx, VBX_E_INVALID, std::string(fn) + ": " + (msg)); } while (0)
#define VBX_REQUIRE(ctx, cond, msg) VBX_REQUIRE_FN(ctx, __func__, cond, msg)

struct Prof {
    vbx_ctx *ctx; const char *name; hipStream_t st; hipEvent_t a = nullptr, b = nullptr;
    Prof(vbx_ctx *c, const char *n, hipStream_t stream = nullptr) : ctx(c), name(n), st(stream ? stream : c->stream) {
        if (ctx->roctx_push) ctx->roctx_push(name);
        if (ctx->prof) { hipEventCreate(&a); hipEventCreate(&b); hipEventRecord(a, st); }
    }
    ~Prof() {
        if (ctx->prof) { hipEventRecord(b, st); ctx->recs.push_back({name, a, b, st}); }
        if (ctx->roctx_pop) ctx->roctx_pop();
    }
};


int ws_get(vbx_ctx *ctx, int slot, size_t bytes, void **out);
int get_bins_dev(vbx_ctx *ctx, size_t n, size_t k, double lo, double hi, double sr,
                 const int32_t **out, std::vector<int32_t> &host_bins, bool &bad);
int check_frames(vbx_ctx *ctx, const char *fn, const void *x, size_t n_frames, size_t frame_len, size_t stride,
                 size_t max_len = VBX_MAX_FRAME_LEN);
int stage_upload(vbx_ctx *ctx, int which, int ws_slot, const void *h_src, size_t bytes, hipStream_t st, void **d_out);
int upload_segments(vbx_ctx *ctx, hipStream_t st, const int64_t *h_seg, size_t n_seg, size_t n_frames, const int64_t **d_seg, size_t *n_out);
int upload_estimates(vbx_ctx *ctx, hipStream_t st, const vbx_resonance *h_est, size_t n_est, const res_t **d_est);


struct resample_plan_t { resample_src_t rs; size_t n_src, m; bool direct; };

int launch_spectral(vbx_ctx *ctx, hipStream_t st, spectral_launch_t &L, const char *prof_name);
const char *pitch_shape_error(size_t frame_len, size_t kmax);
int run_pitch(vbx_ctx *ctx, hipStream_t st, const double *x, size_t n_frames, size_t frame_len, size_t stride,
              const double *window, double sample_rate, double threshold, double fmin, double fmax,
              size_t kmax, vbx_pitch *out_cand, size_t cand_ld, int32_t *out_count, int32_t *status);
bool lpc_order_ok(size_t frame_len, size_t n_coeffs);
int run_autocorr_lpc(vbx_ctx *ctx, hipStream_t st, const double *x, size_t n_frames, size_t frame_len,
                     size_t stride, const double *window, size_t n_coeffs, int normalize,
                     double *out_r, double *out_lpc, size_t lpc_ld);
bool burg_order_ok(size_t frame_len, size_t n_coeffs);
int run_burg(vbx_ctx *ctx, hipStream_t stm, frames_t x, long F, int n, long stride, const double *window, int p, double *coeffs,
             int32_t *st, frame_map_t map = frame_map_t{0, 0, 0}, const resample_plan_t *rp = nullptr);
int run_find_formants(vbx_ctx *ctx, hipStream_t stm, frames_t x, size_t n_frames, size_t frame_len,
                      size_t stride, double sample_rate, size_t n_coeffs,
                      const int64_t *h_seg_start, size_t n_segments,
                      const vbx_resonance *h_est_init, size_t n_est,
                      vbx_resonance *out_formants, size_t formants_ld, vbx_resonance *out_res, int32_t *out_res_count,
                      double *out_coeffs, int32_t *status,
                      const resample_plan_t *rp = nullptr );
int run_mfcc(vbx_ctx *ctx, hipStream_t stm, const double *x, size_t n_frames, size_t frame_len, size_t stride,
             const double *window, size_t num_coeffs, double lo_hz, double hi_hz,
             double sample_rate, double *out, size_t out_ld, int32_t *status);


int make_resample_plan(vbx_ctx *ctx, const char *fn, double ratio, size_t frame_len, size_t order, resample_plan_t *rp, bool *have);
int analyze_ex(vbx_ctx *ctx, const char *fn, frames_t x, size_t n_frames, size_t frame_len, size_t stride,
               const vbx_analysis_params *h_p, const vbx_analysis_ext *h_ext, const vbx_pitch_track_params *h_track,
               const int64_t *h_seg_start, size_t n_segments, double *out_records, size_t record_ld, int32_t *status3,
               const vbx_pitch_track_outputs *h_out, bool defer_path = false );


bool sample_format_ok(int f);
inline int sample_name_slot(int f) { return f >= VBX_SAMPLE_U8 ? f - VBX_SAMPLE_U8 + 6 : f; }
size_t sample_src_bytes(int f);
sample_kind_t sample_plane_kind(int f);
size_t sample_out_bytes(int f);
int ensure_host_slots(vbx_ctx *ctx, size_t bytes);
bool channel_selection_ok(const int32_t *h_channels, size_t n_sel, int channels, unpack_sel_t *sel);


int check_pitch_path(vbx_ctx *ctx, const char *fn, const vbx_pitch_path_params &pr, size_t n_frames, size_t kmax, bool have_peak,
                     const int64_t *h_seg_start, size_t n_segments);
int run_pitch_path(vbx_ctx *ctx, hipStream_t st, const vbx_pitch *cand, const int32_t *count, const int32_t *status,
                   size_t n_frames, size_t kmax, const double *local_peak, const int64_t *h_seg_start, size_t n_segments,
                   const vbx_pitch_path_params &pr, vbx_pitch *out_path, size_t path_ld, int32_t *out_index, const char *fn);
int path_stream_open(vbx_ctx *ctx, const char *fn, size_t kmax, const vbx_pitch_path_params &pr, double peak_ref, size_t max_pending,
                     vbx_path_stream **out);
int path_stream_launch(vbx_path_stream *ps, const char *fn, const vbx_pitch *cand, const int32_t *count, const int32_t *status,
                       const double *local_peak, size_t n, int end_utterance, vbx_pitch *out_path, size_t path_ld, int32_t *out_index,
                       uint8_t *out_forced, vbx_path_commit *d_commit);
int path_stream_launch_all(vbx_path_stream *const *ps, size_t n_sel, const char *fn, const vbx_pitch *cand, const int32_t *count,
                           const int32_t *status, const double *local_peak, size_t plane_frames, size_t n, int end_utterance,
                           const vbx_channel_path_outputs *out, size_t path_ld);
int path_stream_reset(vbx_path_stream *ps);
void path_stream_free(vbx_path_stream *ps);

}
// ... 1 lines not shown
```

vox_box.rs_amd/csrc/vbx_kernels.hpp:

```cpp
#pragma once

#include <hip/hip_runtime.h>
#include <stdint.h>

#define VBX_MAX_LPC_ORDER_K 62
#define VBX_MAX_FRAME_LEN_K 4096
#define VBX_MAX_RESONANCES_K 32
#define VBX_FORMANT_SLOTS_K 6

namespace vbx {

struct frame_map_t { long seg_len, t0, tc; };
__host__ __device__ inline long frame_map(const frame_map_t &m, long i, long n_frames) {
    if (m.seg_len == 0) return (i < n_frames) ? i : -1;
    const long t = m.t0 + i % m.tc, f = (i / m.tc) * m.seg_len + t;
    return (t < m.seg_len && t < m.t0 + m.tc && f < n_frames) ? f : -1;
}
inline long frame_map_items(const frame_map_t &m, long n_frames) {
    return m.seg_len == 0 ? n_frames : ((n_frames + m.seg_len - 1) / m.seg_len) * m.tc;
}


struct res_t { double frequency, bandwidth; };
struct pitch_t { double frequency, strength; };
struct cplx_t { double re, im; };
struct cplx32_t { float re, im; };

enum sample_kind_t { SAMPLE_F64, SAMPLE_PCM16, SAMPLE_F32 };
struct frames_t {
    const void *p; sample_kind_t kind;
    frames_t(const double *x = nullptr) : p(x), kind(SAMPLE_F64) {}
    frames_t(const int16_t *x) : p(x), kind(SAMPLE_PCM16) {}
    frames_t(const float *x) : p(x), kind(SAMPLE_F32) {}
    frames_t(const void *x, sample_kind_t k) : p(x), kind(k) {}
    const double *f64() const { return kind == SAMPLE_F64 ? static_cast<const double *>(p) : nullptr; }
    const int16_t *pcm16() const { return kind == SAMPLE_PCM16 ? static_cast<const int16_t *>(p) : nullptr; }
    const float *f32in() const { return kind == SAMPLE_F32 ? static_cast<const float *>(p) : nullptr; }
};

bool fewlags_supported(int n, int n_lags, bool want_lpc);
void launch_autocorr_fewlags(hipStream_t s, const double *x, long F, int n, long stride, const double *window,
                             int n_lags, int normalize, double *out_r, double *out_lpc, long lpc_ld = 0 ,
                             int32_t *lpc_list = nullptr, int32_t *lpc_count = nullptr );
void launch_autocorr_tiles(hipStream_t s, const double *x, long F, int n, long stride, const double *window,
                           int n_lags, double *out);
void launch_normalize_rows(hipStream_t s, double *data, long rows, int n);
void launch_levinson_rows(hipStream_t s, const double *r, long rows, long r_stride, int p, double *out, long out_ld,
                          double *out_kc = nullptr );
constexpr double LPC_PROBE_EPS = 16.0 * 2.220446049250313e-16;
#ifndef VBX_EXP_LPC_PROBE_TOL
#define VBX_EXP_LPC_PROBE_TOL 1e-6
#endif
constexpr double LPC_PROBE_TOL = VBX_EXP_LPC_PROBE_TOL;
void launch_levinson_rows_probe(hipStream_t s, const double *r, long rows, long r_stride, int p, double *out, long out_ld,
                                int32_t *lpc_list, int32_t *lpc_count, double *mfcc_rows = nullptr, long mfcc_ld = 0, int num_coeffs = 0,
                                const double *dct = nullptr );

bool burg_supported(int n, int p);
void launch_burg(hipStream_t s, frames_t x, long F, int n, long stride, const double *window, int p, double *out, int32_t *status,
                 frame_map_t map);
void launch_burg_list(hipStream_t s, frames_t x, long F, int n, long stride, const double *window, int p, double *out, int32_t *status,
                      const int32_t *list, const int32_t *count);

bool burg_fast_supported(int n, int p);
long burg_fast_chunk(long F);
size_t burg_fast_scratch_bytes(long F, int p);
int32_t *burg_fast_list(void *ws, long F, int p);
bool launch_burg_lags(hipStream_t s, frames_t x, long F, int n, long stride, const double *window, int p, frame_map_t map, long i0,
                      long m, void *ws);
void launch_burg_recursion(hipStream_t s, long F, int p, frame_map_t map, long i0, long m, double *out, int32_t *status, void *ws);

void launch_count_accumulate(hipStream_t s, const int32_t *count, int32_t *total, bool reset);

struct resample_src_t { const int32_t *li; const double *frac; int n_src; };
bool burg_resampled_supported(int n_src, int m, int p);
void launch_burg_resampled(hipStream_t s, frames_t x, long F, int m, long stride, const double *window, resample_src_t rs, int p,
                           double *out, int32_t *status, frame_map_t map);
void launch_burg_resampled_list(hipStream_t s, frames_t x, long F, int m, long stride, const double *window, resample_src_t rs, int p,
                                double *out, int32_t *status, const int32_t *list, const int32_t *count);
bool launch_burg_lags_resampled(hipStream_t s, frames_t x, long F, int m, long stride, const double *window, resample_src_t rs, int p,
                                frame_map_t map, long i0, long n_items, void *ws);

void launch_find_roots(hipStream_t s, cplx_t *polys, long F, int len, int32_t *status);
void launch_laguerre(hipStream_t s, const cplx_t *polys, long F, int len, cplx_t start, cplx_t *out);
void launch_div_polynomial(hipStream_t s, cplx_t *polys, const cplx_t *others, long F, int len, cplx_t *rem, int32_t *status);
void launch_find_roots_f32(hipStream_t s, cplx32_t *polys, long F, int len, int32_t *status);
void launch_laguerre_f32(hipStream_t s, const cplx32_t *polys, long F, int len, cplx32_t start, cplx32_t *out);
void launch_to_resonance(hipStream_t s, const cplx_t *roots, long F, int n_roots, double sample_rate,
                         int strict_im, res_t *out, int out_stride, int32_t *out_count, const int32_t *status);
void launch_formant_resonances(hipStream_t s, const double *coeffs, long F, int p, double sample_rate,
                               res_t *out_res, int32_t *out_count, int32_t *status, frame_map_t map = frame_map_t{0, 0, 0});
bool formant_resonances_fast_supported(int p);
void launch_formant_resonances_fast(hipStream_t s, const double *coeffs, long F, int p, double sample_rate,
                                    res_t *out_res, int32_t *out_count, int32_t *status, frame_map_t map, int32_t *redo_count);

void launch_tracker(hipStream_t s, const res_t *res, long F, int n_res, const int32_t *res_count,
                    const int64_t *seg_start, long n_seg, const res_t *est_init, int n_est,
                    const int32_t *frame_status, res_t *out, long out_ld ,
                    long t0 = 0 , long tc = 0x7fffffffffffffffL );

size_t tracker_chunked_workspace_bytes(long F);
void launch_tracker_chunked(hipStream_t s, const res_t *res, long F, int n_res, const int32_t *res_count,
                            const int64_t *seg_start, long n_seg, const res_t *est_init, int n_est,
                            const int32_t *frame_status, res_t *out, long out_ld, void *ws);

void launch_tracker_stitch(hipStream_t s, const res_t *res, long F, int n_res, const int32_t *res_count, int n_est,
                           const int32_t *frame_status, res_t *out, long out_ld, long first, long stop,
                           const double *state_in , int32_t *changed );

size_t pitch_lds_bytes(int n);
constexpr int PITCH_LIST_LANES = 64;
size_t pitch_full_list_bytes(int n, int kmax);
constexpr int PITCH_WORK_SLOTS = 64;
constexpr int PHASE_SLOTS = 16;
constexpr int PITCH_WORK_WORDS = PITCH_WORK_SLOTS * 4 + PITCH_WORK_SLOTS * PHASE_SLOTS;
#ifdef VBX_EXP_PHASES
#define VBX_PHASE_INIT() unsigned long long _tp = __builtin_readcyclecounter()
#define VBX_PHASE(work_, f_, k_)                                                                                   \
    do {                                                                                                            \
        asm volatile("s_waitcnt vmcnt(0) lgkmcnt(0)" ::: "memory");                                                 \
        const unsigned long long _t = __builtin_readcyclecounter();                                                 \
        if ((work_) != nullptr && lane_id() == 0)                                                                   \
            atomicAdd((work_) + PITCH_WORK_SLOTS * 4 + ((f_) & (PITCH_WORK_SLOTS - 1)) * PHASE_SLOTS + (k_), _t - _tp); \
        _tp = _t;                                                                                                   \
    } while (0)
#else
#define VBX_PHASE_INIT() do { } while (0)
#define VBX_PHASE(work_, f_, k_) do { } while (0)
#endif
void launch_pitch(hipStream_t s, const double *x, long F, int n, long stride, const double *window,
                  const double *lag_window, double sample_rate, double threshold, double fmin, double fmax,
                  int kmax, pitch_t *out_cand, long cand_ld ,
                  int32_t *out_count, int32_t *status, unsigned long long *work);
void launch_pitch_list(hipStream_t s, const int32_t *frame_list, const int32_t *list_count, int grid, frames_t x, int n, long stride,
                       const double *window, const double *lag_window, double sample_rate, double threshold, double fmin, double fmax,
                       int kmax, pitch_t *out_cand, long cand_ld, int32_t *out_count, int32_t *status, unsigned long long *work);
void launch_sinc_points(hipStream_t s, const double *y, int ylen, long offset, long nx, const double *xs, long m,
                        long depth, double *out, int32_t *status);
void launch_extremum_points(hipStream_t s, const double *y, int ylen, long offset, long nx, const double *ix, long m,
                            long depth, double *out_xy, int32_t *status, int interp = 2 ,
                            int is_max = 1);

constexpr int SPECTRAL_N = 1200;
constexpr int SPECTRAL_LPC_ORDER = 12;
constexpr int SPECTRAL_TAB_COMPLEX = 60 * 20 + 3 * 20 + 601;
enum { SPECTRAL_PLAN_NONE = 0, SPECTRAL_PLAN_1200 = 1, SPECTRAL_PLAN_1024 = 2, SPECTRAL_PLAN_2048 = 3, SPECTRAL_PLAN_4096 = 4,
       SPECTRAL_PLANS = 5 };
constexpr int SPECTRAL_AC_MIN_LAGS = 64;
constexpr int SPECTRAL_MIN_N = 512;
int spectral_plan(int n);
int spectral_plan_mfcc(int n);
bool spectral_supported_plan(int plan, int n, int lpc_order, int mfcc_nb, int mfcc_b_lo, int num_coeffs);
int spectral_plan_nc(int plan);
int spectral_tab_complex(int plan);
void spectral_fill_tab(int plan, double *h_out);
int spectral_pow2_tab_complex(int plan);
void spectral_pow2_fill_tab(int plan, double *h_out);
constexpr int MFCC_INTERP_MAX_TAPS = 40;
struct mfcc_interp_t {
    const double *rot;
    const double *coef;
    const int32_t *j0;
    int jmin, jmax;
    int taps;
    int pu_off;
    int lds_bytes;
};
int mfcc_interp_taps(int plan, int n);
size_t mfcc_interp_table_bytes(int plan, int nb);
size_t mfcc_interp_coef_offset(int plan);
size_t mfcc_interp_j0_offset(int plan, int nb);
bool mfcc_interp_fill(int plan, int n, int b_lo, int nb, void *h_table, mfcc_interp_t *h_desc );

struct spectral_launch_t {
    int plan; int n;
    frames_t x;
    long F; long stride; const double *window; const double *lag_window; const double *tab;
    bool mfcc_defer;
    bool lag_rcp;
    double sample_rate, threshold, fmin, fmax; int kmax;
    pitch_t *out_cand; long cand_ld; int32_t *out_count; int32_t *pitch_status; unsigned long long *work;
    double *out_lpc; long lpc_ld;
    double *out_mfcc; long mfcc_ld; int32_t *mfcc_status;
    const int32_t *bins; const double *slopes; const double *dct; int num_coeffs; int nb;
    int32_t *unsure_list; int32_t *unsure_count;
    int32_t *lpc_list; int32_t *lpc_count;
    bool mfcc_only;
    double *out_r; int n_lags;
    bool whole_curve;
    bool interp; mfcc_interp_t ip;
    double *curve_ws; size_t curve_ws_bytes;
};
size_t spectral_split_row_bytes(int n, double sample_rate, double fmin);
bool spectral_supported(int n, int lpc_order, int mfcc_nb, int mfcc_b_lo, int num_coeffs);
bool spectral_list_parked(const spectral_launch_t &L);
int launch_analyze(hipStream_t s, const spectral_launch_t &L);
void launch_mfcc_rows(hipStream_t s, double *rows, long F, long ld, int num_coeffs, const double *dct);
bool lpc_exact_supported(int n, int p);
void launch_lpc_exact_list(hipStream_t s, const int32_t *frame_list, const int32_t *list_count, int cus, frames_t x, int n, long stride,
                           const double *window, int p, double *out_lpc, long lpc_ld);

void launch_lpc_ref(hipStream_t s, frames_t x, long F, int n, long stride, const double *window, int n_lags, int p, int normalize,
                    double *out_r, long r_ld, double *out_lpc, long lpc_ld);
void launch_levinson_ref_rows(hipStream_t s, const double *r, long rows, long r_stride, int p, double *out, long out_ld, double *out_kc);

void launch_autocorr_fewlags_f32(hipStream_t s, const float *x, long F, int n, long stride, const float *window,
                                 int n_lags, int normalize, float *out_r, float *out_lpc, long lpc_ld = 0);
void launch_autocorr_tiles_f32(hipStream_t s, const float *x, long F, int n, long stride, const float *window,
                               int n_lags, float *out);
void launch_normalize_rows_f32(hipStream_t s, float *data, long rows, int n);
void launch_levinson_rows_f32(hipStream_t s, const float *r, long rows, long r_stride, int p, float *out, long out_ld,
                              float *out_kc = nullptr);
void launch_burg_f32(hipStream_t s, const float *x, long F, int n, long stride, const float *window,
                     int p, float *out, int32_t *status);
void launch_widen_frames(hipStream_t s, const float *x, long F, int n, long stride, const float *window, double *out);
void launch_autocorr_f32_exact(hipStream_t s, const float *x, long F, int n, long stride, const float *window, int n_lags, float *out);
size_t pitch_f32_exact_lds_bytes(int n, int kmax);
void launch_pitch_f32_exact(hipStream_t s, const float *x, long F, int n, long stride, const float *window, const float *lag_window32,
                            double sample_rate, double threshold, double fmin, double fmax, int kmax, pitch_t *out_cand, long cand_ld,
                            int32_t *out_count, int32_t *status);
void launch_levinson_f32_exact(hipStream_t s, const float *r, long rows, long r_stride, int p, float *out, long out_ld, float *out_kc);
size_t burg_f32_exact_scratch_bytes(long frames, int n);
void launch_burg_f32_exact(hipStream_t s, const float *x, long f0, long f1, long F, int n, long stride, const float *window, int p,
                           float *out, int32_t *status, float *scratch);
void launch_narrow(hipStream_t s, const double *in, long count, float *out);

bool mfcc_fits(int n, int nb);
struct mfcc_plan_t { bool ok; int n1, n2, nc, tm; };
mfcc_plan_t mfcc_plan(int n, int nb);
void launch_mfcc_dft2(hipStream_t s, const double *x, long F, int n, long stride, const double *window,
                      const mfcc_plan_t &pl, const double *ctab , const double *twid ,
                      const int32_t *bins_dev, const double *slopes, const double *dct_table, int num_coeffs, double *out,
                      long out_ld , int32_t *status , int nb, int cu_count);
struct mfcc_mplan_t { bool ok; int n1, n2, k2, mt, ntd, ntm, src0, src1; };
mfcc_mplan_t mfcc_mfma_plan(int n, int b_lo, int nb);
void launch_mfcc_mfma(hipStream_t s, const double *x, long F, int n, long stride, const double *window,
                      const mfcc_mplan_t &pl, const double *ctab, const double *twd, const double *twm, const double *wm,
                      const int32_t *bins_dev, const double *slopes, const double *dct_table, int num_coeffs, double *out,
                      long out_ld , int32_t *status , int nb, int cu_count);
void launch_mfcc(hipStream_t s, const double *x, long F, int n, long stride, const double *window,
                 const double *kappa_sigma , const int32_t *bins ,
                 const double *slopes , const double *dct_table ,
                 int num_coeffs, double *out, long out_ld, int32_t *status, int nb );
int mfcc_czt_plan(int n, int top );
int mfcc_czt_split_plan(int n, int top, int *n1);
void mfcc_czt_fill_tabs(int n, int top, int L, int n1, double *h_chirp , double *h_bhat);
void launch_mfcc_czt(hipStream_t s, int plan, const double *x, long F, int n, int n1, long stride, const double *window,
                     const double *tab , const double *chirp, const double *bhat, const int32_t *bins,
                     const double *slopes, const double *dct, int num_coeffs, int nb, double *out, long out_ld, int32_t *status,
                     double *cw_scratch );
void launch_fill_rows(hipStream_t s, double *out, long rows, int n, long ld, double value, int32_t *status, int32_t code);
void launch_dct_rows(hipStream_t s, const double *in, long rows, int n, const double *dct_table, double *out);

void launch_resample(hipStream_t s, const double *x, long F, int n, long stride, const int32_t *tab_idx,
                     const double *tab_frac, int m, double *out);
void launch_ring_frames(hipStream_t s, const double *ring, long capacity, long head, long F, int n, long stride, double *out);
void launch_pcm16(hipStream_t s, const int16_t *pcm, size_t n, double denom, double *out);
void launch_frame_peak(hipStream_t s, frames_t x, long F, long n, long stride, double *out);
void launch_rms(hipStream_t s, const double *x, long F, int n, long stride, const double *window, double *out);
void launch_preemphasis(hipStream_t s, const double *x, long F, int n, long stride, double c, double *out);

enum { UNPACK_PCM16 = 1, UNPACK_PCM24 = 2, UNPACK_PCM32 = 3, UNPACK_F32 = 4, UNPACK_F64 = 5, UNPACK_U8 = 16, UNPACK_ULAW = 17, UNPACK_ALAW = 18 };
void launch_unpack(hipStream_t s, int format, const void *src, size_t n, size_t channels, size_t channel, void *out);
#define UNPACK_MAX_SEL 64
struct unpack_sel_t { int32_t ch[UNPACK_MAX_SEL]; };
void launch_unpack_all(hipStream_t s, int format, const void *src, size_t n, size_t channels, const unpack_sel_t &sel, size_t n_sel,
                       void *out, size_t plane_ld);
void launch_host_rows(hipStream_t s, const double *src, size_t src_ld, size_t row0, size_t rows, size_t c0, size_t c1, double *dst,
                      size_t dst_ld, const int32_t *src_st, size_t src_n, int32_t *dst_st, size_t dst_n);

void launch_session_ingest(hipStream_t s, int format, const void *old, size_t drop, size_t keep, const void *raw, size_t n_new,
                           size_t channels, size_t channel, void *out);
struct session_deliver_t {
    const double *src; size_t src_ld, row0, rows, c0, c1; double *dst; size_t dst_ld;
    const int32_t *src_st; size_t src_n; int32_t *dst_st; size_t dst_st_ld;
    const double *src_cand; double *dst_cand; size_t kmax;
    const int32_t *src_count; int32_t *dst_count;
    const double *src_peak; double *dst_peak;
    double *state; size_t n_state;
};
void launch_session_deliver(hipStream_t s, const session_deliver_t &d);

void launch_session_ingest_all(hipStream_t s, int format, const void *old, size_t old_ld, size_t drop, size_t keep, const void *raw,
                               size_t n_new, size_t channels, const unpack_sel_t &sel, size_t n_sel, void *out, size_t out_ld);
struct session_deliver_all_t {
    const double *src; size_t src_ld, plane_frames, row0, rows, c0, c1, dst_ld;
    const int32_t *src_st; size_t src_n, dst_st_ld;
    const double *src_cand; size_t kmax;
    const int32_t *src_count;
    const double *src_peak;
    double *state; size_t n_state;
    struct { double *rec; int32_t *st; double *cand; int32_t *count; double *peak; } ch[UNPACK_MAX_SEL];
};
void launch_session_deliver_all(hipStream_t s, const session_deliver_all_t &d, size_t n_sel);
struct clip_entry_t {
    const void *src;
    uint64_t len, off;
    int64_t plane_frame, row_start, n_rows;
};
void launch_clips_pack(hipStream_t s, int format, const clip_entry_t *tab, size_t n, size_t total, void *plane);
void launch_session_ingest_all8(hipStream_t s, int format, const void *old, size_t old_ld, size_t drop, size_t keep, const void *raw,
                                size_t n_new, size_t channels, const unpack_sel_t &sel, size_t n_sel, void *out, size_t out_ld);
void launch_clips_pack8(hipStream_t s, int format, const clip_entry_t *tab, size_t n, size_t total, void *plane);
struct clips_deliver_t {
    const clip_entry_t *tab; size_t n, row0, rows;
    const double *src; size_t src_ld, c0, c1; double *dst; size_t dst_ld;
    const int32_t *src_st; size_t src_n; int32_t *dst_st[3];
    const double *src_cand; double *dst_cand; size_t kmax;
    const int32_t *src_count; int32_t *dst_count;
    const double *src_peak; double *dst_peak;
};
void launch_clips_deliver(hipStream_t s, const clips_deliver_t &d);

void launch_tracker_stitch_all(hipStream_t s, const res_t *res, long F, int n_res, const int32_t *res_count, int n_est,
                               const int32_t *frame_status, res_t *out, long out_ld, long plane_frames, long first, long stop,
                               const double *state, long n_sel);

void launch_frame_rms(hipStream_t s, frames_t x, long F, int n, long stride, double *out_rms, long rms_ld, double *out_peak);

void launch_f32_to_f64(hipStream_t s, const float *x, size_t n, double *out);

void launch_burg(hipStream_t s, const double *x, long F, int n, long stride, const double *window,
                 int p, double *out, int32_t *status, frame_map_t map = frame_map_t{0, 0, 0});
void launch_burg_pcm16(hipStream_t s, const int16_t *x, long F, int n, long stride, const double *window,
                       int p, double *out, int32_t *status, frame_map_t map = frame_map_t{0, 0, 0});
void launch_burg_list(hipStream_t s, const double *x, long F, int n, long stride, const double *window,
                      int p, double *out, int32_t *status, const int32_t *list, const int32_t *count);
void launch_burg_pcm16_list(hipStream_t s, const int16_t *x, long F, int n, long stride, const double *window,
                            int p, double *out, int32_t *status, const int32_t *list, const int32_t *count);
void launch_burg_lags(hipStream_t s, const double *x, long F, int n, long stride, const double *window, int p,
                      frame_map_t map, long i0, long m, void *ws);
void launch_burg_lags_pcm16(hipStream_t s, const int16_t *x, long F, int n, long stride, const double *window, int p,
                            frame_map_t map, long i0, long m, void *ws);
void launch_burg_resampled(hipStream_t s, const double *x, const int16_t *pcm, long F, int m, long stride, const double *window,
                           resample_src_t rs, int p, double *out, int32_t *status, frame_map_t map);
void launch_burg_resampled_list(hipStream_t s, const double *x, const int16_t *pcm, long F, int m, long stride, const double *window,
                                resample_src_t rs, int p, double *out, int32_t *status, const int32_t *list, const int32_t *count);
void launch_burg_lags_resampled(hipStream_t s, const double *x, const int16_t *pcm, long F, int m, long stride, const double *window,
                                resample_src_t rs, int p, frame_map_t map, long i0, long n_items, void *ws);
void launch_pitch_list(hipStream_t s, const int32_t *frame_list, const int32_t *list_count, int grid,
                       const double *x, int n, long stride, const double *window,
                       const double *lag_window, double sample_rate, double threshold, double fmin, double fmax,
                       int kmax, pitch_t *out_cand, long cand_ld, int32_t *out_count, int32_t *status,
                       unsigned long long *work, bool pcm );
void launch_lpc_exact_list(hipStream_t s, const int32_t *frame_list, const int32_t *list_count, int cus, const double *x, int n,
                           long stride, const double *window, bool pcm , int p, double *out_lpc, long lpc_ld);
void launch_lpc_ref(hipStream_t s, const void *x, bool pcm , long F, int n, long stride, const double *window, int n_lags,
                    int p, int normalize, double *out_r, long r_ld, double *out_lpc, long lpc_ld);
void launch_frame_peak_pcm16(hipStream_t s, const int16_t *pcm, long F, long n, long stride, double *out);
// ... 100 lines not shown
```

vox_box.rs_amd/csrc/vbx_pitch_refine.hpp:

```cpp
#pragma once
#include <type_traits>

#include "vbx_device.hpp"
#include "vbx_kernels.hpp"

namespace vbx {


__device__ __forceinline__ double fma_sc(double p, double x, const double c) {
    double r;
    asm("v_fma_f64 %0, %1, %2, %3" : "=v"(r) : "v"(p), "v"(x), "s"(c));
    return r;
}

__device__ __forceinline__ double sin_poly_q(double x) {
    const double x2 = x * x;
    double p = -1.9572941063391261231e-20;
    p = fma_sc(p, x2, 8.2206352466243297170e-18);
    p = fma_sc(p, x2, -2.8114572543455207632e-15);
    p = fma_sc(p, x2, 7.6471637318198164759e-13);
    p = fma_sc(p, x2, -1.6059043836821614599e-10);
    p = fma_sc(p, x2, 2.5052108385441718775e-08);
    p = fma_sc(p, x2, -2.7557319223985890653e-06);
    p = fma_sc(p, x2, 1.9841269841269841270e-04);
// ... 649 lines not shown
        }
    }
    head *= s0;
    double tail = first_eval_tail<2, 4>(p16, nblk, offset, nl, nr, D, nh, phil, phir, hl, hr);
    tail *= s0;
    const double ub = head + tail * (1.0 + 1.0e-9) + (1.0e-9 + 1.0e-11 * p16[nblk]);
    return (ub != ub) ? INF : ub;
}

__device__ __forceinline__ double first_eval_bound_quad(const double *ys, const double *p16, int nblk, int nvalid, int ylen,
                                                        int offset, int nx, double nn, int depth, int sub, bool have) {
    const double INF = __builtin_inf();
    bool inf = !have;
    double v0 = 0.;
    if (!inf) {
        if (nn == 0. || nn >= (double)nx || !(nn - 1. < nn + 1.)) inf = true;
        else {
#pragma clang fp contract(off)
            const double golden = 1. - 0.6180339887498948482045868343656381177203091798057628621;
            const double ba = nn - 1., bb = nn + 1.;
            if (!(ba >= (double)(-offset))) inf = true;
            v0 = ba + golden * (bb - ba);
        }
    }
    if (!inf && (nx < 1 || v0 > (double)nx || v0 < 0.0)) inf = true;
    int nl = 0, nr = 1, D = 0;
    double phil = 0.5, phir = 0.5;
    if (!inf) {
        const double fl = floor(v0);
        nl = (int)fl; nr = nl + 1;
        phil = v0 - (double)nl; phir = 1.0 - phil;
        if (fabs(v0 - (double)nl) < 1.0e-10 || fabs(v0 - (double)nr) < 1.0e-10) inf = true;
        D = depth;
        if ((offset + nr) < D) D = ((offset + nr) < 0) ? 0 : (offset + nr);
        if ((offset + nl + D) >= nx) D = nx - offset + nl - 1;
        if (D < 0 || offset + nr >= ylen || D > offset + nr || offset + nl < 0 || offset + nl + D >= ylen) inf = true;
    }
    double head = 0.0, tail = 0.0;
    if (!inf) {
        const double s0 = sin_poly(M_PI * fmin(phil, phir)) * 0.31830988618379067154;
        const double hl = M_PI * rcp_nr1(phil + (double)D), hr = M_PI * rcp_nr1(phir + (double)D);
        const int nh = (BOUND_HEAD < D + 1) ? BOUND_HEAD : D + 1;
        double yl[BOUND_HEAD / 4], yr[BOUND_HEAD / 4];
#pragma unroll
        for (int j = 0; j < BOUND_HEAD / 4; j++) {
            const int m = sub + 4 * j;
            const bool in = m < nh;
            yl[j] = y_at_padded(ys, nvalid, in ? offset + nr - m : 0);
            yr[j] = y_at_padded(ys, nvalid, in ? offset + nl + m : 0);
        }
#pragma unroll
        for (int j = 0; j < BOUND_HEAD / 4; j++) {
            const int m = sub + 4 * j;
            if (m >= nh) break;
            const double pl = phil + (double)m, pr = phir + (double)m;
            const double tl = yl[j] * rcp_nr1(pl) * fma(0.5, cos_0_pi(hl * pl), 0.5);
            const double tr = yr[j] * rcp_nr1(pr) * fma(0.5, cos_0_pi(hr * pr), 0.5);
            const double t = tl + tr;
            head += (m & 1) ? -t : t;
        }
        head *= s0;
        tail = first_eval_tail<16, 2>(p16, nblk, offset, nl, nr, D, nh << sub, phil, phir, hl, hr);
        tail *= s0;
    }
    head = group_sum<4>(head);
    tail = group_sum<4>(tail);
    const double ub = head + tail * (1.0 + 1.0e-9) + (1.0e-9 + 1.0e-11 * p16[nblk]);
    return (inf || ub != ub) ? INF : ub;
}

__device__ __forceinline__ int pick_best(float *keys, int ncand, double bar, int lane) {
    double bv = -__builtin_inf(); int bi = 0x7fffffff;
    for (int i = lane; i < ncand; i += 64) { const double v = (double)keys[i]; if (v > bv) { bv = v; bi = i; } }
    const double gm = wave_max(bv);
    int pick = (bv == gm) ? bi : 0x7fffffff;
    for (int o = 32; o > 0; o >>= 1) { const int other = __shfl_xor(pick, o, 64); pick = (other < pick) ? other : pick; }
    if (pick == 0x7fffffff || !(gm >= bar)) return -1;
    if (lane == 0) keys[pick] = -__builtin_inff();
    wave_sync();
    return pick;
}


template <bool EARLY = false>
__device__ __forceinline__ int pick_best_pred(float *keys, const cand_t *cand_list, const double *ys, int ncand, double bar, int lane) {
    double bv = -__builtin_inf(); int bi = 0x7fffffff;
    if (EARLY && ncand <= 64) {
        const float kv = (lane < ncand) ? keys[lane] : -__builtin_inff();
        const bool eligible = kv > -__builtin_inff() && (double)kv >= bar;
        if (!__any(eligible)) return -1;
        if (eligible) {
            const int k = (int)cand_list[lane];
            double p = fmin(ys[k - 1], ys[k + 1]);
            if (!(p == p)) p = __builtin_inf();
            bv = p; bi = lane;
        }
    } else {
    for (int i = lane; i < ncand; i += 64) {
        const float kv = keys[i];
        if (kv > -__builtin_inff() && (double)kv >= bar) {
            const int k = (int)cand_list[i];
            double p = fmin(ys[k - 1], ys[k + 1]);
            if (!(p == p)) p = __builtin_inf();
            if (bi == 0x7fffffff || p > bv) { bv = p; bi = i; }
        }
    }
    }
    const double gm = wave_max(bv);
    int pick = (bi != 0x7fffffff && bv == gm) ? bi : 0x7fffffff;
    for (int o = 32; o > 0; o >>= 1) { const int other = __shfl_xor(pick, o, 64); pick = (other < pick) ? other : pick; }
    if (pick == 0x7fffffff) return -1;
    if (lane == 0) keys[pick] = -__builtin_inff();
    wave_sync();
    return pick;
}


__host__ __device__ constexpr int pitch_refine_lds_bytes(int n, int nst = 0, int cap = 0) {
    const int m = (nst > 0) ? nst : n;
    return (m + Y_PAD + ((((m + PB - 1) / PB) + 2) & ~1)) * 8 + ((cap > 0) ? cap : n / 4 + 8) * (int)(sizeof(float) + sizeof(cand_t));
}

inline int pitch_curve_reach(int n, double sample_rate, double fmin) {
    if (!(fmin > 0.0) || !(sample_rate > 0.0)) return 0;
    const double reach = 2.0 * ceil(sample_rate / fmin) + 16.0;
    if (!(reach < (double)n)) return 0;
    return ((int)reach + 1) & ~1;
}
inline int pitch_curve_entries(int n, double sample_rate, double fmin) {
    if ((n & 1) || !(fmin > 0.0) || !(sample_rate > 0.0)) return 0;
    const double reach = 2.0 * ceil(sample_rate / fmin) + 16.0;
    if (!(reach < (double)n)) return 0;
    int m = (int)reach;
    if (m < n / 2 + 2) m = n / 2 + 2;
    m = (m + 1) & ~1;
    return (m < n) ? m : 0;
}

struct pitch_params_t { double sample_rate, threshold, fmin, fmax; int kmax; int full_off; int f32 = 0; int ncurve = 0; };
__host__ __device__ constexpr int pitch_full_list_entries(int n) { return n / 4 + 2; }

#ifndef VBX_EXP_CELL_NB_PITCH
#define VBX_EXP_CELL_NB_PITCH 0
#endif
#ifndef VBX_EXP_CELL_NB_REFINE_LIST
#define VBX_EXP_CELL_NB_REFINE_LIST 3
#endif
constexpr int PITCH_CELL_NB = VBX_EXP_CELL_NB_PITCH, REFINE_LIST_CELL_NB = VBX_EXP_CELL_NB_REFINE_LIST;
#ifndef VBX_EXP_STOP
#define VBX_EXP_STOP 0
#endif
#define VBX_STOP_AT(k_) do { if (VBX_EXP_STOP == (k_)) return true; } while (0)
#define VBX_STOP_AT_PICK(k_, c_) do { if (VBX_EXP_STOP == (k_)) { if (lane == 0 && out_count != nullptr) out_count[f] = (c_); return true; } } while (0)
template <int STAGE = 0, int NB = 0, bool ONCE = false>
__device__ __forceinline__ bool pitch_refine_store(double *ys, int n, const pitch_params_t &pp, long f,
                                                   double *__restrict__ out_cand, long cand_ld,
                                                   int32_t *__restrict__ out_count, int32_t *__restrict__ status,
                                                   unsigned long long *__restrict__ work, double unc_tol = 0.0,
                                                   double2 *full = nullptr, int *io_ncand = nullptr, int cand_cap = 0,
                                                   uint16_t *list_at = nullptr) {
    const int lane = lane_id();
    const double sample_rate = pp.sample_rate, threshold = pp.threshold, fmin = pp.fmin, fmax = pp.fmax;
    const int kmax = pp.kmax;
    const bool f32 = pp.f32 != 0;
    const int nst = (pp.ncurve > 0) ? pp.ncurve : n;
    const int nblk = (nst + PB - 1) / PB;
    double *p16 = ys + nst + Y_PAD;
    float *keys = reinterpret_cast<float *>(p16 + ((nblk + 2) & ~1));
    cand_t *cand_list = (STAGE == 1 && list_at != nullptr) ? reinterpret_cast<cand_t *>(list_at)
                                                           : reinterpret_cast<cand_t *>(keys + ((STAGE == 2 && cand_cap > 0) ? cand_cap : n / 4 + 8));
    const int b = (int)floor(0.5 * (double)n);
    const int offset = -b - 1;
    const int nx = b - offset;
    const int ylen = 2 * n;
    const int nvalid = nst + Y_PAD;

    constexpr int NN_PARKED = 16;
    constexpr bool NN_PARK = ONCE && STAGE == 0;
    double *nn_park = reinterpret_cast<double *>(keys);
    bool parked = false;
    VBX_PHASE_INIT();
    int ncand = 0;
    if constexpr (STAGE == 2) ncand = *io_ncand;
    else {
    int npeak = 0;
    bool unsure = false;
    for (int base = 0; base < b; base += 64) {
        const int k = base + lane;
        bool peak = false;
        if (k >= 1 && k + 1 < b) {
            const double c = ys[k];
            const double d1 = c - ys[k - 1], d2 = c - ys[k + 1];
            peak = (ys[k - 1] < c) && (ys[k + 1] < c);
            unsure = unsure || (fabs((d1 < d2) ? d1 : d2) <= unc_tol);
        }
        const unsigned long long mask = __ballot(peak);
        if (peak) cand_list[npeak + __popcll(mask & ((1ull << lane) - 1ull))] = (cand_t)k;
        npeak += __popcll(mask);
    }
    wave_sync();
    if (unc_tol > 0.0 && __any(unsure)) return false;
    VBX_PHASE(work, f, 6);
    VBX_STOP_AT(1);
    unsure = false;
    parked = NN_PARK && !f32 && npeak <= 64 && n / 4 + 8 >= 2 * NN_PARKED;
    for (int base = 0; base < npeak; base += 64) {
        const int i = base + lane;
        bool pass = false;
        int k = 0;
        double nn_i = 0.0;
        if (i < npeak) {
            k = cand_list[i];
            double freq, nn;
            cand_from_peak(ys, k, sample_rate, offset, freq, nn, f32);
            if (parked) nn_i = nn_from_freq(sample_rate, freq, offset);
            pass = (freq == 0.0) || (freq > fmin && freq < fmax);
            if (unc_tol > 0.0) {
                const double c = ys[k], d2r = 2. * c - (ys[k - 1] - ys[k + 1]), dr = 0.5 * (ys[k + 1] - ys[k - 1]);
                const double dlag = unc_tol * (1.0 + 4.0 * fabs(dr / d2r)) / fabs(d2r);
                const double tol_f = 2.0 * freq * dlag / fabs((double)k + dr / d2r);
                if (!(fabs(freq - fmin) > tol_f && fabs(freq - fmax) > tol_f)) unsure = true;
            }
        }
        wave_sync();
        const unsigned long long mask = __ballot(pass);
        const int ci = ncand + __popcll(mask & ((1ull << lane) - 1ull));
        if (pass) cand_list[ci] = (cand_t)k;
        if (parked && pass && ci < NN_PARKED) nn_park[ci] = nn_i;
        ncand += __popcll(mask);
        wave_sync();
    }

    if (unc_tol > 0.0 && __any(unsure)) return false;
    VBX_PHASE(work, f, 7);
    VBX_STOP_AT(2);
    }
    if constexpr (STAGE == 1) { *io_ncand = ncand; return true; }

    const bool in_order = full != nullptr || kmax > ncand || f32;
    double nn_kept = 0.0;
    int n_kept = 0;
    if (!in_order) {
        const int per = (nblk + 63) >> 6;
        constexpr int PER_REG = 4;
        if (ONCE && per <= PER_REG) {
            double bs[PER_REG];
            double tot = 0.0;
#pragma unroll
            for (int q = 0; q < PER_REG; q++) {
                const int j = lane * per + q;
                const bool in = q < per && j < nblk;
                bs[q] = in ? block_abs_sum(ys + PB * j) : 0.0;
                if (in) tot += bs[q];
            }
            const double incl = wave_inclusive_scan(tot);
            double run = incl - tot;
            if (lane == 0) p16[0] = 0.0;
#pragma unroll
            for (int q = 0; q < PER_REG; q++) {
                const int j = lane * per + q;
                if (q < per && j < nblk) {
                    run += bs[q];
                    p16[j + 1] = run;
                }
            }
        } else {
        double tot = 0.0;
        for (int q = 0; q < per; q++) {
            const int j = lane * per + q;
            if (j < nblk) tot += block_abs_sum(ys + PB * j);
        }
        const double incl = wave_inclusive_scan(tot);
        double run = incl - tot;
        if (lane == 0) p16[0] = 0.0;
        for (int q = 0; q < per; q++) {
            const int j = lane * per + q;
            if (j < nblk) {
                run += block_abs_sum(ys + PB * j);
                p16[j + 1] = run;
            }
        }
        }
        wave_sync();
        VBX_STOP_AT(3);
        const bool quad = ((ncand + 15) / 16) * 7 < ((ncand + 63) / 64) * 25;
        if (quad) {
            for (int base = 0; base < ncand; base += 16) {
                const int c = base + (lane >> 2);
                const bool have = c < ncand;
                double freq = 0., nn = 0.;
                if (parked && base == 0) { if (have) nn = nn_park[c]; }
                else if (have) cand_from_peak(ys, cand_list[c], sample_rate, offset, freq, nn, f32);
                if (ONCE && base == 0) { nn_kept = nn; n_kept = (ncand < 16) ? ncand : 16; }
                const double ub = first_eval_bound_quad(ys, p16, nblk, nvalid, ylen, offset, nx, nn, 1200, lane & 3, have);
                const double kb = (ub <= 1.) ? ub : ((ub != ub) ? __builtin_inf() : ((ub == __builtin_inf()) ? ub : 1.));
                if (have && (lane & 3) == 0) keys[c] = __double2float_ru(kb);
            }
        } else {
            for (int c = lane; c < ncand; c += 64) {
                double freq, nn;
                cand_from_peak(ys, cand_list[c], sample_rate, offset, freq, nn, f32);
                const double ub = first_eval_bound(ys, p16, nblk, nvalid, ylen, offset, nx, nn, 1200);
                const double kb = (ub <= 1.) ? ub : ((ub != ub) ? __builtin_inf() : ((ub == __builtin_inf()) ? ub : 1.));
                keys[c] = __double2float_ru(kb);
            }
        }
        wave_sync();
    }

    VBX_PHASE(work, f, 8);
    VBX_STOP_AT(4);
    int st = 0;
    int kept = 0;
// ... 34 lines not shown
            }
            insert(xm, ym, c);
        };
        int c_general = -1;
#ifndef VBX_EXP_NO_WAVE_BRENT
        for (;;) {
            const double bar = VBX_BAR();
            const int c = in_order ? next_full-- : pick_best_pred<ONCE>(keys, cand_list, ys, ncand, bar, lane);
            VBX_STOP_AT_PICK(5, c);
            if (c < 0) break;
            double freq, nn, xmid, ymid;
            if (ONCE && c < n_kept) nn = readlane_f64(nn_kept, 4 * __builtin_amdgcn_readfirstlane(c));
            else cand_from_peak(ys, cand_list[c], sample_rate, offset, freq, nn, f32);
            bool dropped = false;
            if (__builtin_expect(!improve_extremum_sinc_wave<NB>(ys, nvalid, ylen, offset, nx, nn, 1200, xmid, ymid, cterms, cevals, bar, dropped), 0)) {
                c_general = c;
                break;
            }
            if (dropped) continue;
            enter(c, xmid, ymid);
        }
        if (c_general >= 0)
#endif
        for (;;) {
            const double bar = VBX_BAR();
            int c = c_general;
            c_general = -1;
            if (c < 0) c = in_order ? next_full-- : pick_best_pred<ONCE>(keys, cand_list, ys, ncand, bar, lane);
            if (c < 0) break;
            double freq, nn, xmid, ymid;
            cand_from_peak(ys, cand_list[c], sample_rate, offset, freq, nn, f32);
            bool dropped = false;
            improve_extremum_sinc<64>(ys, nvalid, ylen, offset, nx, nn, 1200, true, xmid, ymid, st, &cterms, &cevals, bar, &dropped);
            if (dropped) continue;
            enter(c, xmid, ymid);
        }
    } else {
      auto run_groups = [&](auto pg_tag, auto dual_tag) {
        constexpr int PG = decltype(pg_tag)::value;
        constexpr bool DUAL = decltype(dual_tag)::value;
        bool exhausted = false;
        const int gid = lane / PG;
        int ci = -1, it = 0;
        bool special = false, safe = false, trusted = false;
        double ba = 0., bb = 0., v = 0., w = 0., x = 0., fv = 0., fw = 0., fx = 0., xmid = 0., ymid = 0.;
        constexpr unsigned long long LEADERS = (PG == 16) ? 0x0001000100010001ull : (PG == 8) ? 0x0101010101010101ull
                                             : (PG == 32) ? 0x0000000100000001ull : (PG == 4) ? 0x1111111111111111ull : 1ull;
        const double golden = 1. - 0.6180339887498948482045868343656381177203091798057628621;
        const double sqrt_epsilon = 1.4901161193847656e-08, eps = 2.220446049250313e-16, tol = 1e-10;
        for (;;) {
#pragma clang fp contract(off)
            bool finished = false;
            double range = 0., middle_range = 0., tol_act = 0.;
            if (ci >= 0) {
                if (special) finished = true;
                else if (it > 0) {
                    range = bb - ba;
                    middle_range = (ba + bb) * 0.5;
                    tol_act = sqrt_epsilon * fabs(x) + tol / 3.;
                    if (it > 60 || fabs(x - middle_range) + range * 0.5 <= 2. * tol_act) { finished = true; xmid = x; ymid = fx; }
                }
            }
            if (__any(finished)) {
                unsigned long long fm = __ballot(finished) & LEADERS;
                double xm = xmid + (double)offset;
                double ym = ymid;
                if (ym > 1.) ym = 1. / ym;
                double cf = sample_rate / (f32 ? (double)(float)xm : xm), cs = ym;
                if (f32) { cf = (double)(float)cf; cs = (double)(float)cs; }
                while (fm) {
                    const int ld = __builtin_ctzll(fm);
                    fm &= fm - 1;
                    insert(readlane_f64(cf, ld), readlane_f64(cs, ld), __builtin_amdgcn_readlane(ci, ld));
                }
                if (finished) ci = -1;
            }
            {
                unsigned long long im = __ballot(ci < 0) & LEADERS;
                while (im != 0ull && !exhausted) {
                    const int c = in_order ? next_full-- : pick_best_pred<ONCE>(keys, cand_list, ys, ncand, VBX_BAR(), lane);
                    if (VBX_EXP_STOP == 5 || c < 0) { exhausted = true; break; }
                    const int g = __builtin_ctzll(im) / PG;
                    im &= im - 1ull;
                    if (gid == g) {
                        ci = c;
                        double freq, nn;
                        cand_from_peak(ys, cand_list[ci], sample_rate, offset, freq, nn, f32);
                        it = 0; special = false; xmid = 0.; ymid = 0.;
                        if (nn == 0.) { special = true; xmid = 0.; ymid = ys[0]; }
                        else if (nn >= (double)nx) { special = true; xmid = (double)nx; ymid = y_at(ys, nvalid, nx - 1); }
                        else if (!(nn - 1. < nn + 1.)) { special = true; st |= 4; }
                        ba = nn - 1.; bb = nn + 1.;
                        safe = ba >= (double)(-offset);
                        trusted = !special && sinc_bracket_trusted(ba, bb, nvalid, ylen, offset, nx, 1200);
                    }
                }
            }
            if (!__any(ci >= 0)) break;
            const double bar = VBX_BAR();

            bool need = false;
            double t = 0.;
            if (ci >= 0 && !special) {
                if (it == 0) { v = ba + golden * (bb - ba); t = v; }
                else {
                    double new_step = (x < middle_range) ? golden * (bb - x) : golden * (ba - x);
                    if (fabs(x - w) >= tol_act) {
                        const double tt = (x - w) * (fx - fv);
                        double q = (x - v) * (fx - fw);
                        double pp = (x - v) * q - (x - w) * tt;
                        q = 2. * q - tt;
                        if (q > 0.) pp = -pp; else q = -q;
                        if (fabs(pp) < fabs(new_step * q) && pp > q * (ba - x + 2. * tol_act) && pp < q * (bb - x - 2. * tol_act))
                            new_step = pp / q;
                    }
                    if (fabs(new_step) < tol_act) new_step = (new_step > 0.) ? tol_act : -tol_act;
                    t = x + new_step;
                }
                need = true;
            }
            const double ft = sinc_interp<PG, DUAL>(ys, nvalid, ylen, offset, nx, t, 1200, need, st, &nterms, trusted);
            nevals += need ? 1u : 0u;
            if (need) {
                if (it == 0) {
                    x = v; w = v; fv = ft; fx = ft; fw = ft; it = 1;
                    const double ub = (ft <= 1.) ? ft : 1.;
                    if (ub < bar && safe) ci = -1;
                } else {
                    if (ft <= fx) {
                        if (t < x) bb = x; else ba = x;
                        v = w; w = x; x = t;
                        fv = fw; fw = fx; fx = ft;
                    } else {
                        if (t < x) ba = t; else bb = t;
                        if (ft <= fw || fabs(w - x) < eps) {
                            v = w; w = t;
                            fv = fw; fw = ft;
                        } else if (ft <= fv || fabs(v - x) < eps || fabs(v - w) < eps) {
                            v = t;
                            fv = ft;
                        }
                    }
                    it++;
                    if (safe && fx < bar) ci = -1;
                }
            }
        }
      };
      const bool dual_ok = in_order || (kmax >= 8 && ncand >= 12);
      if (RG == 16 && dual_ok && ncand >= DUAL_MIN_CAND) { run_groups(std::integral_constant<int, RG / 2>{}, std::true_type{}); group_lanes = RG / 2; }
      else run_groups(std::integral_constant<int, RG>{}, std::false_type{});
    }
#undef VBX_BAR
    VBX_PHASE(work, f, 9);
    const int total_cand = ncand + 1;
    st = __any(st & 4) ? 4 : 0;
    if (total_cand > 1 && (any_nan || threshold != threshold)) st |= 8;
    int code = 0;
    if (st & 4) code = 4; else if (st & 8) code = 3;
    if (fullm) {
        wave_sync();
        if (pp.full_off < 0) {
            __builtin_amdgcn_fence(__ATOMIC_RELEASE, "agent");
            __builtin_amdgcn_fence(__ATOMIC_ACQUIRE, "agent");
            double2 *lds_list = reinterpret_cast<double2 *>(ys);
            for (int i = lane; i < total_cand; i += 64) lds_list[i] = full[i];
            full = lds_list;
            wave_sync();
        }
        double *row = out_cand + f * cand_ld;
        const int total = (code == 0) ? total_cand : 0;
        for (int i0 = 0; i0 < total; i0 += 64) {
            const int i = i0 + lane;
            const double2 me = (i < total) ? full[i] : double2{0.0, 0.0};
            int rank = 0;
            for (int j = 0; j < total; j++) {
                const double sj = full[j].y;
                rank += (sj > me.y || (sj == me.y && j < i)) ? 1 : 0;
            }
            if (i < total && rank < kmax) store_pair8(row + 2 * rank, me);
        }
        for (int i = total + lane; i < kmax; i += 64) store_pair8(row + 2 * i, double2{0.0, 0.0});
    } else if (lane < kmax) {
        const bool valid = (code == 0) && lane < kept;
        double2 o;
        o.x = valid ? lf : 0.0;
        o.y = valid ? ls : 0.0;
        store_pair8(out_cand + f * cand_ld + 2 * lane, o);
    }
    if (lane == 0) {
        if (out_count != nullptr) out_count[f] = (code == 0) ? total_cand : 0;
        if (status != nullptr) status[f] = code;
    }
    if (work != nullptr) {
        const bool leader = (lane & (group_lanes - 1)) == 0;
        unsigned long long te = leader ? nterms : 0u, ev = leader ? nevals : 0u;
        for (int o = 32; o > 0; o >>= 1) { te += __shfl_xor(te, o, 64); ev += __shfl_xor(ev, o, 64); }
        if (lane == 0) {
            unsigned long long *w = work + 4 * (f & (PITCH_WORK_SLOTS - 1));
            atomicAdd(w + 0, 1ull); atomicAdd(w + 1, (unsigned long long)ncand);
            atomicAdd(w + 2, ev + cevals); atomicAdd(w + 3, te + cterms);
        }
    }
    return true;
}

}
```

vox_box.rs_amd/csrc/vbx_spectral.hpp:

```cpp
#pragma once

#include "vbx_device.hpp"
#include "vbx_kernels.hpp"
#include "vbx_pitch_refine.hpp"

namespace vbx {

enum { SP_ANALYZE = 0, SP_MFCC_ONLY = 1, SP_AC_ONLY = 2, SP_MFCC_HALF = 3, SP_ANALYZE_INTERP = 4, SP_ANALYZE_SPLIT = 5, SP_ANALYZE_INTERP_SPLIT = 6,
       SP_MFCC_ONLY_INTERP = 7 };
__host__ __device__ constexpr bool sp_is_interp(int mode) { return mode == SP_ANALYZE_INTERP || mode == SP_ANALYZE_INTERP_SPLIT || mode == SP_MFCC_ONLY_INTERP; }
__host__ __device__ constexpr bool sp_is_mfcc_only(int mode) { return mode == SP_MFCC_ONLY || mode == SP_MFCC_HALF || mode == SP_MFCC_ONLY_INTERP; }
__host__ __device__ constexpr bool sp_is_split(int mode) { return mode == SP_ANALYZE_SPLIT || mode == SP_ANALYZE_INTERP_SPLIT; }
__host__ __device__ constexpr bool sp_is_analyze(int mode) { return mode == SP_ANALYZE || mode == SP_ANALYZE_INTERP || mode == SP_ANALYZE_SPLIT || mode == SP_ANALYZE_INTERP_SPLIT; }

constexpr double SP_UNC_EPS = 6.0 * 400.0 * 2.220446049250313e-16;

constexpr int SP_FLAG_PCM = 1, SP_FLAG_LAG_RCP = 2, SP_FLAG_MFCC_DEFER = 4;
__host__ __device__ constexpr int lag_rcp_offset(int n) { return (n + 1) & ~1; }
__device__ __forceinline__ double quotient_by_table(double a, double b, double y) {
    const double q0 = a * y;
    const double rem = fma(-q0, b, a);
    return fma(rem, y, q0);
}

__device__ __forceinline__ void dft4(double &r0, double &i0, double &r1, double &i1, double &r2, double &i2,
                                     double &r3, double &i3) {
    const double t0r = r0 + r2, t0i = i0 + i2, t1r = r0 - r2, t1i = i0 - i2;
    const double t2r = r1 + r3, t2i = i1 + i3, t3r = r1 - r3, t3i = i1 - i3;
    r0 = t0r + t2r; i0 = t0i + t2i;
    r2 = t0r - t2r; i2 = t0i - t2i;
    r1 = t1r + t3i; i1 = t1i - t3r;
    r3 = t1r - t3i; i3 = t1i + t3r;
}

struct spectral_args_t {
    const double *frames; long n_frames; long stride; const double *window; const double *lag_window;
    const double2 *tab;
    int n;
    pitch_params_t pp;
    double *out_cand; long cand_ld; int32_t *out_count; int32_t *pitch_status; unsigned long long *work;
    double *out_lpc; long lpc_ld;
    double *out_mfcc; long mfcc_ld; int32_t *mfcc_status;
    const int32_t *bins; const double *slopes; const double *dct; int num_coeffs; int nb;
    int32_t *unsure_list; int32_t *unsure_count;
    double *out_r; int n_lags;
    int mfcc_q;
    int pcm;
    mfcc_interp_t ip;
    long f0, n_batch;
    double *curve; long curve_ld; double *curve_tol;
    int32_t *curve_list; long list_ld; int reach, cand_cap;
    int32_t *far_list;
};

constexpr int SP_TAIL = 16;
__device__ __forceinline__ void spectral_exact_tail(double *ys, int n, const double *__restrict__ xf, const double *__restrict__ window,
                                                    const double *__restrict__ lag_window, double x0, double scale, int lane) {
    wave_sync();
    if (lane < SP_TAIL && lane < n) {
#pragma clang fp contract(off)
        const int L = n - 1 - lane;
        double xu[SP_TAIL], wu[SP_TAIL], xv[SP_TAIL], wv[SP_TAIL];
#pragma unroll
        for (int i = 1; i < SP_TAIL; i++) {
            const int k = (i <= lane) ? i : 0;
            xu[i] = xf[k]; xv[i] = xf[L + k];
            wu[i] = (window != nullptr) ? window[k] : 1.0; wv[i] = (window != nullptr) ? window[L + k] : 1.0;
        }
        const double lw = lag_window[L];
        double acc = x0;
#pragma unroll
        for (int i = 1; i < SP_TAIL; i++) {
            const double u = (window != nullptr) ? xu[i] * wu[i] : xu[i];
            const double v = (window != nullptr) ? xv[i] * wv[i] : xv[i];
            const double next = acc + u * v;
            acc = (i <= lane) ? next : acc;
        }
        ys[L] = (acc * scale) / lw;
    }
}

template <int P>
__device__ __forceinline__ void levinson_regs(const double (&r)[P + 1], double (&ac)[P + 1]) {
    double tmp[P + 1];
    double err = r[0];
    ac[0] = 1.0;
#pragma unroll
    for (int i = 1; i <= P; i++) ac[i] = 0.0;
#pragma unroll
    for (int i = 1; i <= P; i++) {
        double acc = r[i];
#pragma unroll
        for (int j = 1; j < i; j++) acc = acc + ac[j] * r[i - j];
        const double k = -acc / err;
        ac[i] = k;
#pragma unroll
        for (int j = 0; j < P; j++) tmp[j] = ac[j];
#pragma unroll
        for (int j = 1; j < i; j++) ac[j] = ac[j] + k * tmp[i - j];
        err = err * (1.0 - k * k);
    }
}

constexpr int SP_LPC_P = SPECTRAL_LPC_ORDER;


void launch_analyze_f32in(hipStream_t s, const spectral_args_t &a, unsigned grid, size_t lds, bool lpc, bool mfcc, bool waves3);
int launch_analyze_pow2(hipStream_t s, const spectral_launch_t &L, spectral_args_t &a);

}
```

vox_box.rs_amd/csrc/vbx_spectral_1200.hpp:

```cpp
#pragma once

#include <type_traits>
#include "vbx_device.hpp"
#include "vbx_kernels.hpp"
#include "vbx_mfcc_tail.hpp"
#include "vbx_mfcc_interp.hpp"
#include "vbx_pitch_refine.hpp"
#include "vbx_spectral.hpp"

namespace vbx {

constexpr int SP_N = SPECTRAL_N;
constexpr int SP_M = 2 * SP_N;
constexpr int SP_S1 = 61;
constexpr int SP_S2 = 404;
constexpr int SP_T1 = 0;
constexpr int SP_T2 = SP_T1 + 60 * 20;
constexpr int SP_TM = SP_T2 + 3 * 20;
static_assert(SP_TM + 601 == SPECTRAL_TAB_COMPLEX, "table layout");
constexpr int SP_T2_LDS_OFFSET = (2 * 602 + 64) * 8;
static_assert(SP_T2_LDS_OFFSET >= (20 * SP_S1 > 3 * SP_S2 ? 20 * SP_S1 : 3 * SP_S2) * 8 && SP_T2_LDS_OFFSET % 16 == 0, "T2 behind both");

__device__ __forceinline__ void dft5(double &r0, double &i0, double &r1, double &i1, double &r2, double &i2,
                                     double &r3, double &i3, double &r4, double &i4) {
// ... 10 lines not shown
    const double vr = fma(S2, t3r, -(S1 * t4r)), vi = fma(S2, t3i, -(S1 * t4i));
    r0 = r0 + t5r; i0 = i0 + t5i;
    r1 = s1r + ui; i1 = s1i - ur;
    r4 = s1r - ui; i4 = s1i + ur;
    r2 = s2r + vi; i2 = s2i - vr;
    r3 = s2r - vi; i3 = s2i + vr;
}

__host__ __device__ constexpr int dft20_in(int n1, int n2) { return (5 * n1 + 4 * n2) % 20; }
__host__ __device__ constexpr int dft20_slot(int k) { return (5 * (k % 4) + 4 * (k % 5)) % 20; }

__device__ __forceinline__ void dft20(double (&re)[20], double (&im)[20]) {
#pragma unroll
    for (int n2 = 0; n2 < 5; n2++)
        dft4(re[dft20_in(0, n2)], im[dft20_in(0, n2)], re[dft20_in(1, n2)], im[dft20_in(1, n2)],
             re[dft20_in(2, n2)], im[dft20_in(2, n2)], re[dft20_in(3, n2)], im[dft20_in(3, n2)]);
#pragma unroll
    for (int k1 = 0; k1 < 4; k1++)
        dft5(re[dft20_in(k1, 0)], im[dft20_in(k1, 0)], re[dft20_in(k1, 1)], im[dft20_in(k1, 1)],
             re[dft20_in(k1, 2)], im[dft20_in(k1, 2)], re[dft20_in(k1, 3)], im[dft20_in(k1, 3)],
             re[dft20_in(k1, 4)], im[dft20_in(k1, 4)]);
}

#ifndef VBX_EXP_TWB
#define VBX_EXP_TWB 2
#endif
constexpr int TWB = VBX_EXP_TWB;
#ifndef VBX_EXP_MB1
#define VBX_EXP_MB1 3
#endif
template <int TWB = vbx::TWB>
__device__ __forceinline__ void twiddle_tight(double (&re)[20], double (&im)[20], const double2 *tw_row) {
#pragma unroll
    for (int h = 0; h < 20 / TWB; h++) {
        double2 tw[TWB];
#pragma unroll
        for (int k = 0; k < TWB; k++) tw[k] = tw_row[TWB * h + k];
#pragma unroll
        for (int k = 0; k < TWB; k++) {
            if (TWB * h + k == 0) continue;
            const int s = dft20_slot(TWB * h + k);
            const double a = re[s], b = im[s];
            re[s] = fma(a, tw[k].x, -(b * tw[k].y));
            im[s] = fma(a, tw[k].y, b * tw[k].x);
            asm volatile("" : "+v"(re[s]), "+v"(im[s]));
        }
        asm volatile("" ::: "memory");
    }
}

template <int KC, bool TIGHT = false>
__device__ __forceinline__ void fft1200(double (&re)[20], double (&im)[20], double (&xr)[7][3], double (&xi)[7][3],
                                        double *ex, const double2 *tab, const double2 *t2) {
    const int lane = lane_id();
    const int np = (lane < 60) ? lane : 59;
    const bool act = lane < 60;
    dft20(re, im);
    if constexpr (TIGHT) twiddle_tight(re, im, tab + SP_T1 + np * 20);
    else {
#pragma unroll
    for (int h = 0; h < 2; h++) {
        double2 tw[10];
#pragma unroll
        for (int k = 0; k < 10; k++) tw[k] = tab[SP_T1 + np * 20 + 10 * h + k];
#pragma unroll
        for (int k = 0; k < 10; k++) {
            if (10 * h + k == 0) continue;
            const int s = dft20_slot(10 * h + k);
            const double a = re[s], b = im[s];
            re[s] = fma(a, tw[k].x, -(b * tw[k].y));
            im[s] = fma(a, tw[k].y, b * tw[k].x);
        }
    }
    }
    const int ka2 = np % 20, c2 = np / 20;
    double br[20], bi[20];
    wave_sync();
#pragma unroll
    for (int k = 0; k < 20; k++) if (act) ex[k * SP_S1 + lane] = re[dft20_slot(k)];
    wave_sync();
#pragma unroll
    for (int b = 0; b < 20; b++) br[b] = ex[ka2 * SP_S1 + 3 * b + c2];
    wave_sync();
#pragma unroll
    for (int k = 0; k < 20; k++) if (act) ex[k * SP_S1 + lane] = im[dft20_slot(k)];
    wave_sync();
#pragma unroll
    for (int b = 0; b < 20; b++) bi[b] = ex[ka2 * SP_S1 + 3 * b + c2];
    dft20(br, bi);
    if constexpr (TIGHT) twiddle_tight<4>(br, bi, t2 + c2 * 20);
    else {
#pragma unroll
    for (int h = 0; h < 2; h++) {
        double2 tw[10];
#pragma unroll
        for (int k = 0; k < 10; k++) tw[k] = t2[c2 * 20 + 10 * h + k];
#pragma unroll
        for (int k = 0; k < 10; k++) {
            if (10 * h + k == 0) continue;
            const int s = dft20_slot(10 * h + k);
            const double a = br[s], b = bi[s];
            br[s] = fma(a, tw[k].x, -(b * tw[k].y));
            bi[s] = fma(a, tw[k].y, b * tw[k].x);
        }
    }
    }
    double vr[7][3], vi[7][3];
    wave_sync();
#pragma unroll
    for (int k = 0; k < 20; k++) if (act) ex[c2 * SP_S2 + ka2 + 20 * k] = br[dft20_slot(k)];
    wave_sync();
#pragma unroll
    for (int t = 0; t < 7; t++)
#pragma unroll
        for (int c = 0; c < 3; c++) vr[t][c] = (t < 6 || lane < 16) ? ex[c * SP_S2 + lane + 64 * t] : 0.0;
    wave_sync();
#pragma unroll
    for (int k = 0; k < 20; k++) if (act) ex[c2 * SP_S2 + ka2 + 20 * k] = bi[dft20_slot(k)];
    wave_sync();
#pragma unroll
    for (int t = 0; t < 7; t++)
#pragma unroll
        for (int c = 0; c < 3; c++) vi[t][c] = (t < 6 || lane < 16) ? ex[c * SP_S2 + lane + 64 * t] : 0.0;
    wave_sync();
    constexpr double H3 = 0.86602540378443864676;
#pragma unroll
    for (int t = 0; t < 7; t++) {
        const double sr = vr[t][1] + vr[t][2], si = vi[t][1] + vi[t][2];
        const double dr = vr[t][1] - vr[t][2], di = vi[t][1] - vi[t][2];
        xr[t][0] = vr[t][0] + sr; xi[t][0] = vi[t][0] + si;
        const double mr = fma(-0.5, sr, vr[t][0]), mi = fma(-0.5, si, vi[t][0]);
        xr[t][1] = fma(H3, di, mr); xi[t][1] = fma(-H3, dr, mi);
        if (KC == 3) { xr[t][2] = fma(-H3, di, mr); xi[t][2] = fma(H3, dr, mi); }
        else { xr[t][2] = 0.0; xi[t][2] = 0.0; }
    }
}

#ifndef VBX_SPECTRAL_WAVES
#define VBX_SPECTRAL_WAVES 2
#endif
#ifndef VBX_EXP_CELL_NB
#define VBX_EXP_CELL_NB 3
#endif
#ifndef VBX_EXP_CELL_NB_F32IN
#define VBX_EXP_CELL_NB_F32IN VBX_EXP_CELL_NB
#endif
#ifndef VBX_EXP_FRONT_END_ONCE
#define VBX_EXP_FRONT_END_ONCE 1
#endif
__host__ __device__ constexpr bool sp_front_end_once(bool mfcc, bool full, int waves, bool f32) {
    return VBX_EXP_FRONT_END_ONCE != 0 && !(!mfcc && full && waves >= 3 && !f32);
}
__host__ __device__ constexpr int sp_cell_blocks(int waves, bool f32) { return f32 ? VBX_EXP_CELL_NB_F32IN : VBX_EXP_CELL_NB; }
template <bool LPC, bool MFCC, bool FULL, int MODE = SP_ANALYZE, int WAVES = VBX_SPECTRAL_WAVES, typename TIN = double>
__global__ __launch_bounds__(64) __attribute__((amdgpu_waves_per_eu(sp_is_mfcc_only(MODE) ? 2 : WAVES, sp_is_mfcc_only(MODE) ? 4 : WAVES))) void analyze_kernel(const spectral_args_t a) {
    constexpr bool F32 = std::is_same<TIN, float>::value;
    static_assert(!F32 || (FULL && MODE == SP_ANALYZE), "float samples: the fused analysis of full frames");
    static_assert(MODE != SP_MFCC_ONLY || (MFCC && FULL && !LPC), "the MFCC-only form needs the full frame and has no lag sums");
    static_assert(MODE != SP_AC_ONLY || (!MFCC && !LPC), "the autocorrelation-only form");
    static_assert(!sp_is_interp(MODE) || (MFCC && !FULL), "interpolated bins: a padded frame's MFCC");
    static_assert(MODE != SP_MFCC_ONLY_INTERP || !LPC, "the MFCC-only forms have no lag sums");
    constexpr bool PITCH = !sp_is_mfcc_only(MODE);
    constexpr bool INTERP = sp_is_interp(MODE);
    extern __shared__ __attribute__((aligned(16))) double smem[];
    const long f = xcd_item(blockIdx.x, a.n_frames);
    if (f >= a.n_frames) return;
    const int lane = lane_id();
    const int np = (lane < 60) ? lane : 59;
    const int n = FULL ? SP_N : a.n;
    double *ex = smem;
    const double *xf = a.frames + f * a.stride;
    double2 *t2 = reinterpret_cast<double2 *>(reinterpret_cast<char *>(smem) + SP_T2_LDS_OFFSET);
    VBX_PHASE_INIT();

    double re[20], im[20];
    const int16_t *x16 = reinterpret_cast<const int16_t *>(a.frames) + f * a.stride;
    const float *x32 = reinterpret_cast<const float *>(a.frames) + f * a.stride;
    {
        const bool al = ((((uintptr_t)xf) | ((uintptr_t)a.window)) & 15) == 0;
        double2 xv[10], wv[10];
        float2 xs32[F32 ? 10 : 1];
#pragma unroll
        for (int q = 0; q < 10; q++) {
            const int i = 120 * q + 2 * np;
            if constexpr (F32) {
                float lo, hi;
                if ((((uintptr_t)x32) & 7) == 0) { const float2 w = *reinterpret_cast<const float2 *>(x32 + i); lo = w.x; hi = w.y; }
                else { lo = x32[i]; hi = x32[i + 1]; }
                xs32[q] = float2{lo, hi};
                wv[q] = (a.window != nullptr) ? (((uintptr_t)a.window & 15) == 0 ? *reinterpret_cast<const double2 *>(a.window + i)
                                                                                  : double2{a.window[i], a.window[i + 1]}) : double2{1.0, 1.0};
            } else if (FULL && (a.pcm & SP_FLAG_PCM)) {
                int lo, hi;
                if ((((uintptr_t)x16) & 3) == 0) { const int w = *reinterpret_cast<const int *>(x16 + i); lo = (short)(w & 0xffff); hi = w >> 16; }
                else { lo = x16[i]; hi = x16[i + 1]; }
                xv[q] = double2{pcm16_value(lo), pcm16_value(hi)};
                wv[q] = (a.window != nullptr) ? (((uintptr_t)a.window & 15) == 0 ? *reinterpret_cast<const double2 *>(a.window + i)
                                                                                  : double2{a.window[i], a.window[i + 1]}) : double2{1.0, 1.0};
            } else if (al && i + 1 < n) {
                xv[q] = *reinterpret_cast<const double2 *>(xf + i);
                wv[q] = (a.window != nullptr) ? *reinterpret_cast<const double2 *>(a.window + i) : double2{1.0, 1.0};
            } else {
                xv[q] = double2{0.0, 0.0}; wv[q] = double2{1.0, 1.0};
                if (i < n) { xv[q].x = xf[i]; if (a.window != nullptr) wv[q].x = a.window[i]; }
                if (i + 1 < n) { xv[q].y = xf[i + 1]; if (a.window != nullptr) wv[q].y = a.window[i + 1]; }
            }
        }
#pragma unroll
        for (int q = 0; q < 10; q++) {
            if constexpr (F32) xv[q] = double2{(double)xs32[q].x, (double)xs32[q].y};
            re[q] = (a.window != nullptr) ? xv[q].x * wv[q].x : xv[q].x;
            im[q] = (a.window != nullptr) ? xv[q].y * wv[q].y : xv[q].y;
        }
#pragma unroll
        for (int q = 10; q < 20; q++) { re[q] = 0.0; im[q] = 0.0; }
    }
    const double x0 = readlane_f64(re[0], 0);
    if (lane < 60) t2[lane] = a.tab[SP_T2 + lane];
    VBX_PHASE(a.work, f, 0);

    double xr[7][3], xi[7][3];
    fft1200<3, (WAVES >= 3)>(re, im, xr, xi, ex, a.tab, t2);
    VBX_PHASE(a.work, f, 1);

    double ar[10], ai[10], br[10], bi[10];
#pragma unroll
    for (int t = 0; t < 7; t++)
#pragma unroll
        for (int kc = 0; kc < 3; kc++) if (t < 6 || lane < 16) ex[lane + 64 * t + 400 * kc] = xr[t][kc];
    wave_sync();
#pragma unroll
    for (int t = 0; t < 10; t++) {
        const int m = lane + 64 * t;
        const bool ok = m <= 600;
        ar[t] = ok ? ex[m] : 0.0;
        br[t] = ok ? ex[(m == 0) ? 0 : SP_N - m] : 0.0;
    }
    wave_sync();
#pragma unroll
    for (int t = 0; t < 7; t++)
#pragma unroll
        for (int kc = 0; kc < 3; kc++) if (t < 6 || lane < 16) ex[lane + 64 * t + 400 * kc] = xi[t][kc];
    wave_sync();
#pragma unroll
    for (int t = 0; t < 10; t++) {
        const int m = lane + 64 * t;
        const bool ok = m <= 600;
        ai[t] = ok ? ex[m] : 0.0;
        bi[t] = ok ? ex[(m == 0) ? 0 : SP_N - m] : 0.0;
    }
    wave_sync();

    const int b_lo = MFCC ? a.bins[0] : 0;
    double pk[10], pn[10];
    double2 *zc = reinterpret_cast<double2 *>(ex);
    double2 rot_m = double2{1.0, 0.0}, rot_step = double2{1.0, 0.0};
    if constexpr (INTERP) { rot_m = reinterpret_cast<const double2 *>(a.ip.rot)[lane]; rot_step = reinterpret_cast<const double2 *>(a.ip.rot)[64]; }
#pragma unroll
    for (int t = 0; t < 10; t++) {
        const int m = lane + 64 * t;
        const double2 w = a.tab[SP_TM + ((m <= 600) ? m : 0)];
        const double er = 0.5 * (ar[t] + br[t]), ei = 0.5 * (ai[t] - bi[t]);
        const double o_r = 0.5 * (ai[t] + bi[t]), o_i = -0.5 * (ar[t] - br[t]);
        const double tr = fma(w.x, o_r, -(w.y * o_i)), ti = fma(w.x, o_i, w.y * o_r);
        const double pr = er + tr, pi = ei + ti, qr = er - tr, qi = ei - ti;
        pk[t] = fma(pr, pr, pi * pi);
        pn[t] = fma(qr, qr, qi * qi);
        if constexpr (INTERP) {
            asm volatile("" : "+v"(pk[t]), "+v"(pn[t]));
            mfcc_interp_stage(zc, a.ip, m, pr, pi, rot_m, rot_step, t == 0);
        }
    }

    if constexpr (INTERP) {
        wave_sync();
        VBX_PHASE(a.work, f, 13);
        const int nbp = (a.nb + 1) & ~1;
        double *pu = ex + a.ip.pu_off, *pd = pu + nbp, *en = pd + nbp;
        const double2 *cf = reinterpret_cast<const double2 *>(a.ip.coef) + lane;
        const int HT = a.ip.taps >> 1;
        for (int u = 0; u * 64 < a.nb; u++) {
            const int b = lane + 64 * u;
            const double2 *zp = zc + a.ip.j0[u * 64 + lane];
            const double2 sl = *reinterpret_cast<const double2 *>(a.slopes + 2 * ((b < a.nb) ? b : 0));
            double vr, vi;
            mfcc_interp_bin(HT, cf + (u * HT) * 64, 64, zp, vr, vi);
            const double pw = fma(vr, vr, vi * vi);
            if (b < a.nb) {
                pu[b] = fabs(pw) * sl.x;
                pd[b] = fabs(sqrt(pw)) * sl.y;
            }
        }
        wave_sync();
        VBX_PHASE(a.work, f, 14);
        double2 t2v = double2{0.0, 0.0};
        if constexpr (PITCH) t2v = a.tab[SP_T2 + np];
        if (a.num_coeffs <= 16) mfcc_tail_q(pu, pd, en, a.bins, a.dct, a.num_coeffs, b_lo, lane, a.out_mfcc + f * a.mfcc_ld, a.work, f, (a.pcm & SP_FLAG_MFCC_DEFER) != 0);
        else mfcc_tail_m(pu, pd, en, a.bins, a.dct, a.num_coeffs, b_lo, lane, a.out_mfcc + f * a.mfcc_ld);
        if (a.mfcc_status != nullptr && lane == 0) a.mfcc_status[f] = 0;
        wave_sync();
        if (PITCH && lane < 60) t2[lane] = t2v;
        VBX_PHASE(a.work, f, 15);
    }

    if constexpr (PITCH) {
        double2 wm[10];
    #pragma unroll
        for (int t = 0; t < 10; t++) { const int m = lane + 64 * t; wm[t] = a.tab[SP_TM + ((m <= 600) ? m : 0)]; }
    #pragma unroll
        for (int t = 0; t < 10; t++) {
            const int m = lane + 64 * t;
            if (m <= 600) {
                const double2 w = wm[t];
                const double sm = pk[t] + pn[t], d = pk[t] - pn[t];
                ex[m] = fma(d, w.y, sm);
                if (m >= 1 && m < 600) ex[SP_N - m] = fma(-d, w.y, sm);
            }
        }
        wave_sync();
    #pragma unroll
        for (int q = 0; q < 20; q++) re[q] = ex[60 * q + np];
        wave_sync();
    #pragma unroll
        for (int t = 0; t < 10; t++) {
            const int m = lane + 64 * t;
            if (m <= 600) {
                const double2 w = wm[t];
                const double gi = -((pk[t] - pn[t]) * w.x);
                ex[m] = gi;
                if (m >= 1 && m < 600) ex[SP_N - m] = gi;
            }
        }
        wave_sync();
    #pragma unroll
        for (int q = 0; q < 20; q++) im[q] = ex[60 * q + np];
        wave_sync();
    }

    VBX_PHASE(a.work, f, 2);
    if constexpr (MFCC && !INTERP) {
        const int nbp = (a.nb + 1) & ~1;
        const int q = FULL ? 2 : a.mfcc_q, half = FULL ? SP_N / 2 : a.n / 2;
        double *pu = ex, *pd = ex + nbp, *en = ex + 2 * nbp;
        constexpr int MB = 2;
        const bool two_sided = (half - 600 / q) - b_lo < a.nb;
        if (!two_sided) {
            constexpr int MB1 = VBX_EXP_MB1;
#pragma unroll
            for (int h = 0; h < (10 + MB1 - 1) / MB1; h++) {
                double2 s1[MB1];
                int c1[MB1];
#pragma unroll
                for (int u = 0; u < MB1; u++) {
                    const int t = MB1 * h + u, m = lane + 64 * t;
                    if (t >= 10) { c1[u] = -1; continue; }
                    const bool on = m <= 600 && (FULL ? (m & 1) == 0 : m % q == 0);
                    const int b1 = (FULL ? (m >> 1) : m / q) - b_lo;
                    c1[u] = (on && b1 >= 0 && b1 < a.nb) ? b1 : -1;
                    s1[u] = *reinterpret_cast<const double2 *>(a.slopes + 2 * (c1[u] < 0 ? 0 : c1[u]));
                }
#pragma unroll
                for (int u = 0; u < MB1; u++) {
                    const int t = MB1 * h + u;
                    if (t < 10 && c1[u] >= 0) {
                        pu[c1[u]] = fabs(pk[t]) * s1[u].x;
                        pd[c1[u]] = fabs(sqrt(pk[t])) * s1[u].y;
                    }
                }
            }
        } else
#pragma unroll
        for (int h = 0; h < 10 / MB; h++) {
            double2 s1[MB], s2[MB];
            int c1[MB], c2[MB];
#pragma unroll
            for (int u = 0; u < MB; u++) {
                const int t = MB * h + u, m = lane + 64 * t;
                const bool on = m <= 600 && (FULL ? (m & 1) == 0 : m % q == 0);
                const int mq = FULL ? (m >> 1) : m / q;
                const int b1 = mq - b_lo, b2 = (half - mq) - b_lo;
                c1[u] = (on && b1 >= 0 && b1 < a.nb) ? b1 : -1;
                c2[u] = (on && b2 >= 0 && b2 < a.nb && b2 != b1) ? b2 : -1;
                s1[u] = *reinterpret_cast<const double2 *>(a.slopes + 2 * (c1[u] < 0 ? 0 : c1[u]));
                s2[u] = *reinterpret_cast<const double2 *>(a.slopes + 2 * (c2[u] < 0 ? 0 : c2[u]));
            }
#pragma unroll
            for (int u = 0; u < MB; u++) {
                const int t = MB * h + u;
                if (c1[u] >= 0) {
                    pu[c1[u]] = fabs(pk[t]) * s1[u].x;
                    pd[c1[u]] = fabs(sqrt(pk[t])) * s1[u].y;
                }
                if (c2[u] >= 0) {
                    pu[c2[u]] = fabs(pn[t]) * s2[u].x;
                    pd[c2[u]] = fabs(sqrt(pn[t])) * s2[u].y;
                }
            }
        }
        wave_sync();
        VBX_PHASE(a.work, f, 13);
        if (a.num_coeffs <= 16) mfcc_tail_q(pu, pd, en, a.bins, a.dct, a.num_coeffs, b_lo, lane, a.out_mfcc + f * a.mfcc_ld, a.work, f, (a.pcm & SP_FLAG_MFCC_DEFER) != 0);
        else mfcc_tail_m(pu, pd, en, a.bins, a.dct, a.num_coeffs, b_lo, lane, a.out_mfcc + f * a.mfcc_ld);
        if (a.mfcc_status != nullptr && lane == 0) a.mfcc_status[f] = 0;
        wave_sync();
    }

    VBX_PHASE(a.work, f, 3);
    if constexpr (!PITCH) return;

    fft1200<2, (WAVES >= 3)>(re, im, xr, xi, ex, a.tab, t2);
    VBX_PHASE(a.work, f, 4);

    constexpr double INV_M = 1.0 / (double)SP_M;
    double r_e[11], r_o[11];
    int jj[11];
#pragma unroll
    for (int s = 0; s < 11; s++) {
        const int t = (s < 7) ? s : s - 7, kc = (s < 7) ? 0 : 1;
        const int q = lane + 64 * t;
        const bool ok = (kc == 0) ? (q < 400) : (q < 200);
        jj[s] = ok ? q + 400 * kc : -1;
        r_e[s] = xr[t][kc] * INV_M;
        r_o[s] = -(xi[t][kc] * INV_M);
    }
    const double s0 = readlane_f64(r_e[0], 0);
    if (x0 != 0.0) {
#pragma unroll
        for (int s = 0; s < 11; s++) {
            const int i = 2 * jj[s];
            if (jj[s] >= 0 && i < n) {
                const double xs = F32 ? (double)x32[i] : (FULL && (a.pcm & SP_FLAG_PCM)) ? pcm16_value(x16[i]) : xf[i];
                const double xe = (a.window != nullptr) ? xs * a.window[i] : xs;
                r_e[s] = (r_e[s] - x0 * xe) + x0;
            }
            if (jj[s] >= 0 && i + 1 < n) {
                const double xs = F32 ? (double)x32[i + 1] : (FULL && (a.pcm & SP_FLAG_PCM)) ? pcm16_value(x16[i + 1]) : xf[i + 1];
                const double xo = (a.window != nullptr) ? xs * a.window[i + 1] : xs;
                r_o[s] = (r_o[s] - x0 * xo) + x0;
            }
        }
    }
    if constexpr (MODE == SP_AC_ONLY) {
        double *row = a.out_r + f * (long)a.n_lags;
        const bool al = ((((uintptr_t)a.out_r) & 15) == 0) && (a.n_lags & 1) == 0;
#pragma unroll
        for (int s = 0; s < 11; s++) {
            const int i = 2 * jj[s];
            if (jj[s] >= 0 && i + 1 < a.n_lags && al) *reinterpret_cast<double2 *>(row + i) = double2{r_e[s], r_o[s]};
            else {
                if (jj[s] >= 0 && i < a.n_lags) row[i] = r_e[s];
                if (jj[s] >= 0 && i + 1 < a.n_lags) row[i + 1] = r_o[s];
            }
        }
        return;
    }
    if (LPC) {
        static_assert(SP_LPC_P == 12, "seven lanes hold r[0..12]");
        double *row = a.out_lpc + f * a.lpc_ld;
        if (lane < 7) { row[2 * lane] = r_e[0]; if (lane < 6) row[2 * lane + 1] = r_o[0]; }
    }
    double amax = -1.0;
#pragma unroll
    for (int s = 0; s < 11; s++) {
        const int i = 2 * jj[s];
        const double ae = fabs(r_e[s]), ao = fabs(r_o[s]);
        if (jj[s] >= 0 && i < n) amax = (ae > amax) ? ae : amax;
        if (jj[s] >= 0 && i + 1 < n) amax = (ao > amax) ? ao : amax;
    }
    amax = wave_max(amax);
    const double scale = 1.0 / amax;
    double *ys = smem;
    wave_sync();
    const bool by_table = (a.pcm & SP_FLAG_LAG_RCP) != 0 && fabs(scale) < 1e290 && fabs(scale) > 1e-290;
    const double *lag_rcp = a.lag_window + lag_rcp_offset(n);
    if (by_table) {
#ifndef VBX_EXP_LB
#define VBX_EXP_LB 4
#endif
        constexpr int LB = VBX_EXP_LB;
#pragma unroll
        for (int h = 0; h < (11 + LB - 1) / LB; h++) {
            double2 lwv[LB], rwv[LB];
#pragma unroll
            for (int u = 0; u < LB; u++) {
                const int s = LB * h + u;
                if (s >= 11) continue;
                const int i = 2 * jj[s];
                const int at = (jj[s] >= 0 && i + 1 < n) ? i : 0;
                lwv[u] = *reinterpret_cast<const double2 *>(a.lag_window + at);
                rwv[u] = *reinterpret_cast<const double2 *>(lag_rcp + at);
            }
#pragma unroll
            for (int u = 0; u < LB; u++) {
                const int s = LB * h + u;
                if (s >= 11) continue;
                const int i = 2 * jj[s];
                if (jj[s] >= 0 && i + 1 < n) {
                    double2 y;
                    y.x = quotient_by_table(r_e[s] * scale, lwv[u].x, rwv[u].x);
                    y.y = quotient_by_table(r_o[s] * scale, lwv[u].y, rwv[u].y);
                    *reinterpret_cast<double2 *>(ys + i) = y;
                } else if (jj[s] >= 0 && i < n) {
                    ys[i] = (r_e[s] * scale) / a.lag_window[i];
                }
            }
            asm volatile("" ::: "memory");
        }
    } else {
        double2 lwv[11];
#pragma unroll
        for (int s = 0; s < 11; s++) {
            const int i = 2 * jj[s];
            lwv[s] = *reinterpret_cast<const double2 *>(a.lag_window + ((jj[s] >= 0 && i + 1 < n) ? i : 0));
        }
#pragma unroll
        for (int s = 0; s < 11; s++) {
            const int i = 2 * jj[s];
            if (jj[s] >= 0 && i + 1 < n) {
                const double2 lw = lwv[s];
                double2 y;
                y.x = (r_e[s] * scale) / lw.x;
                y.y = (r_o[s] * scale) / lw.y;
                *reinterpret_cast<double2 *>(ys + i) = y;
            } else if (jj[s] >= 0 && i < n) {
                ys[i] = (r_e[s] * scale) / a.lag_window[i];
            }
        }
    }
    if (lane < Y_PAD) ys[n + lane] = 0.0;
#ifndef VBX_EXP_NO_EXACT_TAIL
    if (!FULL) spectral_exact_tail(ys, n, xf, a.window, a.lag_window, x0, scale, lane);
#endif
    wave_sync();
    VBX_PHASE(a.work, f, 5);
    const double unc_tol = SP_UNC_EPS * fabs(s0) * scale;
    double2 *full = a.pp.full_off > 0 ? reinterpret_cast<double2 *>(reinterpret_cast<char *>(smem) + a.pp.full_off)
                  : a.pp.full_off < 0 ? reinterpret_cast<double2 *>(a.out_cand + f * a.cand_ld) : nullptr;
    if (!pitch_refine_store<0, sp_cell_blocks(WAVES, F32), sp_front_end_once(MFCC, FULL, WAVES, F32)>(ys, n, a.pp, f, a.out_cand, a.cand_ld, a.out_count, a.pitch_status, a.work, unc_tol, full)) {
        if (lane == 0) a.unsure_list[atomicAdd(a.unsure_count, 1)] = (int32_t)f;
    }
}

}
```

vox_box.rs_amd/voxbox.py:

```python
import ctypes as C
import os
import re

import numpy as np

_HERE = os.path.dirname(os.path.abspath(__file__))
LIB_PATH = os.environ.get("VBX_LIB_PATH") or os.path.join(_HERE, "lib", "libvoxbox_hip.so")
HEADER_PATH = os.path.join(os.path.dirname(_HERE), "include", "voxbox_hip.h")

WINDOW_HANNING, WINDOW_HANNING_LAG, WINDOW_HANNING_PERIODIC, WINDOW_RECTANGLE = 0, 1, 2, 3
FRAME_OK, FRAME_ERR_LPC, FRAME_ERR_POLYNOMIAL, FRAME_ERR_NAN, FRAME_ERR_PANIC = 0, 1, 2, 3, 4
MALE_FORMANT_ESTIMATES = (320.0, 1440.0, 2760.0, 3200.0)
FEMALE_FORMANT_ESTIMATES = (480.0, 1760.0, 3200.0, 3520.0)
MAX_RESONANCES = 32
MAX_PITCH_CANDIDATES = 1026
LPC_POLICY_EXACT, LPC_POLICY_PLAIN, LPC_POLICY_REFERENCE = 0, 1, 2


def pitch_max_candidates(frame_len):
    return frame_len // 4 + 2


class VoxBoxError(RuntimeError):
    pass
# ... 120 lines not shown
    _fields_ = [("format", C.c_int32), ("reserved", C.c_int32), ("group_frames", C.c_size_t)]

    @classmethod
    def make(cls, format, group_frames=0):
        return cls(int(format), 0, int(group_frames))


class ClipRow(C.Structure):
    _fields_ = [("row_start", C.c_int64), ("n_rows", C.c_int64), ("group", C.c_int64), ("plane_frame", C.c_int64)]

    def as_tuple(self):
        return int(self.row_start), int(self.n_rows), int(self.group), int(self.plane_frame)


class ChannelOutputs(C.Structure):
    _fields_ = [("records", C.c_void_p), ("status3", C.c_void_p), ("outputs", C.POINTER(PitchTrackOutputs))]


class ChannelPathOutputs(C.Structure):
    _fields_ = [("out_path", C.c_void_p), ("out_index", C.c_void_p), ("out_forced", C.c_void_p), ("d_commit", C.c_void_p)]


class SessionPlan(C.Structure):
    _fields_ = [("lo", C.c_size_t), ("hi", C.c_size_t), ("warm", C.c_size_t), ("continues_prev", C.c_int),
                ("read_from", C.c_size_t), ("keep_from", C.c_size_t)]

    def as_dict(self):
        return {k: int(getattr(self, k)) for k, _ in self._fields_}


class SessionChannelsPlan(C.Structure):
    _fields_ = [("push", SessionPlan), ("frames", C.c_size_t), ("base", C.c_size_t), ("keep", C.c_size_t), ("len", C.c_size_t),
                ("plane_frames", C.c_size_t), ("plane_ld", C.c_size_t), ("call_frames", C.c_size_t), ("capacity", C.c_size_t)]

    def as_dict(self):
        d = {k: int(getattr(self, k)) for k, _ in self._fields_ if k != "push"}
        d["push"] = self.push.as_dict()
        return d


class PathCommit(C.Structure):
    _fields_ = [("first", C.c_int64), ("n", C.c_int64), ("n_forced", C.c_int64), ("pending", C.c_int64)]

    def as_tuple(self):
        return int(self.first), int(self.n), int(self.n_forced), int(self.pending)


_lib = None


def exported_symbols():
    with open(HEADER_PATH) as f:
        text = f.read()
    text = re.sub(r"/\*.*?\*/", "", text, flags=re.S)
    return sorted(set(re.findall(r"\b(vbx_[a-z0-9_]+)\s*\(", text)))


def load_library():
    global _lib
    if _lib is not None:
        return _lib
    if not os.path.exists(LIB_PATH):
        raise VoxBoxError(
            f"{LIB_PATH} is missing: build it with `make -C {_HERE}` (or __graft_entry__.build()); "
            "there is no CPU fallback")
    L = C.CDLL(LIB_PATH)
    vp, sz, dbl, i32, i64 = C.c_void_p, C.c_size_t, C.c_double, C.c_int, C.c_int64
    sig = {
        "vbx_abi_version": (C.c_int, []),
        "vbx_ctx_create": (C.c_int, [C.POINTER(vp), i32, vp]),
        "vbx_ctx_destroy": (None, [vp]),
        "vbx_ctx_set_lpc_policy": (C.c_int, [vp, i32]),
        "vbx_ctx_get_lpc_policy": (C.c_int, [vp, C.POINTER(C.c_int)]),
        "vbx_sync": (C.c_int, [vp]),
        "vbx_last_error": (C.c_char_p, [vp]),
        "vbx_device_info": (C.c_int, [vp, C.c_char_p, sz, C.POINTER(C.c_int)]),
        "vbx_malloc": (C.c_int, [vp, C.POINTER(vp), sz]),
        "vbx_free": (C.c_int, [vp, vp]),
        "vbx_memcpy_h2d": (C.c_int, [vp, vp, vp, sz]),
        "vbx_memcpy_d2h": (C.c_int, [vp, vp, vp, sz]),
        "vbx_memset": (C.c_int, [vp, vp, i32, sz]),
        "vbx_timer_begin": (C.c_int, [vp]),
        "vbx_timer_end": (C.c_int, [vp, C.POINTER(C.c_float)]),
        "vbx_profile_enable": (C.c_int, [vp, i32]),
        "vbx_profile_reset": (C.c_int, [vp]),
        "vbx_profile_get": (C.c_int, [vp, C.c_char_p, C.POINTER(C.c_double), C.POINTER(C.c_long)]),
        "vbx_profile_stream": (C.c_int, [vp, C.c_char_p, C.POINTER(C.c_int)]),
        "vbx_profile_names": (C.c_int, [vp, C.c_char_p, sz]),
        "vbx_profile_pitch_work": (C.c_int, [vp, C.POINTER(C.c_uint64)]),
        "vbx_window_table_f64": (C.c_int, [i32, sz, vp]),
        "vbx_frame_count": (sz, [sz, sz, sz]),
        "vbx_hz_to_mel": (dbl, [dbl]),
        "vbx_mel_to_hz": (dbl, [dbl]),
        "vbx_find_formants_real_work_size": (sz, [sz, sz]),
        "vbx_find_formants_complex_work_size": (sz, [sz]),
        "vbx_autocorrelate_f64": (C.c_int, [vp, vp, sz, sz, sz, vp, sz, vp]),
        "vbx_normalize_f64": (C.c_int, [vp, vp, sz, sz]),
        "vbx_interpolate_sinc_f64": (C.c_int, [vp, vp, sz, C.c_long, sz, vp, sz, sz, vp, vp]),
        "vbx_improve_extremum_f64": (C.c_int, [vp, vp, sz, C.c_long, sz, vp, sz, sz, vp, vp]),
        "vbx_improve_extremum_ex_f64": (C.c_int, [vp, vp, sz, C.c_long, sz, vp, sz, i32, sz, i32, vp, vp]),
        "vbx_pitch_f64": (C.c_int, [vp, vp, sz, sz, sz, vp, dbl, dbl, dbl, dbl, sz, vp, vp, vp]),
        "vbx_frame_peak_f64": (C.c_int, [vp, vp, sz, sz, sz, vp]),
        "vbx_pitch_path_f64": (C.c_int, [vp, vp, vp, vp, sz, sz, vp, vp, sz, C.POINTER(PitchPathParams), vp, vp]),
        "vbx_internal_last_path_chunks_redone": (C.c_int, [vp, C.POINTER(C.c_int64)]),
        "vbx_pitch_path_segment_peaks_f64": (C.c_int, [vp, vp, sz, vp, sz, vp]),
        "vbx_pitch_path_shard_begin_f64": (C.c_int, [vp, vp, vp, vp, sz, sz, vp, vp, vp, sz, C.POINTER(PitchPathParams), sz, i32, i32]),
        "vbx_pitch_path_shard_enter_f64": (C.c_int, [vp, vp, vp, vp, vp]),
        "vbx_pitch_path_shard_finish_f64": (C.c_int, [vp, vp, vp, sz, vp]),
        "vbx_lpc_f64": (C.c_int, [vp, vp, sz, sz, sz, vp]),
        "vbx_lpc_mut_f64": (C.c_int, [vp, vp, sz, sz, sz, vp, vp]),
        "vbx_window_table_f32": (C.c_int, [i32, sz, vp]),
        "vbx_autocorrelate_f32": (C.c_int, [vp, vp, sz, sz, sz, vp, sz, vp]),
        "vbx_autocorrelate_f32_wide": (C.c_int, [vp, vp, sz, sz, sz, vp, sz, vp]),
        "vbx_normalize_f32": (C.c_int, [vp, vp, sz, sz]),
        "vbx_lpc_mut_f32": (C.c_int, [vp, vp, sz, sz, sz, vp, vp]),
        "vbx_lpc_mut_f32_wide": (C.c_int, [vp, vp, sz, sz, sz, vp, vp]),
        "vbx_autocorr_lpc_f32": (C.c_int, [vp, vp, sz, sz, sz, vp, sz, i32, vp, vp]),
        "vbx_autocorr_lpc_f32_wide": (C.c_int, [vp, vp, sz, sz, sz, vp, sz, i32, vp, vp]),
        "vbx_lpc_burg_f32": (C.c_int, [vp, vp, sz, sz, sz, vp, sz, vp, vp]),
        "vbx_lpc_burg_f32_wide": (C.c_int, [vp, vp, sz, sz, sz, vp, sz, vp, vp]),
        "vbx_mfcc_f32": (C.c_int, [vp, vp, sz, sz, sz, vp, sz, dbl, dbl, dbl, vp, vp]),
        "vbx_pitch_f32": (C.c_int, [vp, vp, sz, sz, sz, vp, C.c_float, C.c_float, C.c_float, C.c_float, sz, vp, vp, vp]),
        "vbx_pitch_f32_wide": (C.c_int, [vp, vp, sz, sz, sz, vp, C.c_float, C.c_float, C.c_float, C.c_float, sz, vp, vp, vp]),
        "vbx_autocorr_lpc_f64": (C.c_int, [vp, vp, sz, sz, sz, vp, sz, i32, vp, vp]),
        "vbx_lpc_burg_f64": (C.c_int, [vp, vp, sz, sz, sz, vp, sz, vp, vp]),
        "vbx_find_roots_c64": (C.c_int, [vp, vp, sz, sz, vp]),
        "vbx_laguerre_c64": (C.c_int, [vp, vp, sz, sz, _Complex, vp]),
        "vbx_div_polynomial_c64": (C.c_int, [vp, vp, vp, sz, sz, vp, vp]),
        "vbx_degree_c64": (sz, [vp, sz]),
        "vbx_off_low_c64": (sz, [vp, sz]),
        "vbx_ring_frames_f64": (C.c_int, [vp, vp, sz, sz, sz, sz, sz, vp]),
        "vbx_find_roots_c32": (C.c_int, [vp, vp, sz, sz, vp]),
        "vbx_laguerre_c32": (C.c_int, [vp, vp, sz, sz, _Complex32, vp]),
        "vbx_to_resonance_c64": (C.c_int, [vp, vp, sz, sz, dbl, vp, vp]),
        "vbx_estimate_formants_f64": (C.c_int, [vp, vp, sz, sz, vp, sz, vp, sz, vp, vp]),
        "vbx_find_formants_f64": (C.c_int, [vp, vp, sz, sz, sz, dbl, sz, vp, sz, vp, sz, vp, vp, vp, vp, vp]),
        "vbx_mfcc_f64": (C.c_int, [vp, vp, sz, sz, sz, vp, sz, dbl, dbl, dbl, vp, vp]),
        "vbx_dct_f64": (C.c_int, [vp, vp, sz, sz, vp]),
        "vbx_mfcc_bins": (C.c_int, [sz, sz, dbl, dbl, dbl, vp]),
        "vbx_resampled_len": (sz, [sz, dbl]),
        "vbx_resample_linear_f64": (C.c_int, [vp, vp, sz, sz, sz, dbl, vp]),
        "vbx_pcm16_to_f64": (C.c_int, [vp, vp, sz, vp]),
        "vbx_f32_to_f64": (C.c_int, [vp, vp, sz, vp]),
        "vbx_rms_f64": (C.c_int, [vp, vp, sz, sz, sz, vp, vp]),
        "vbx_preemphasis_f64": (C.c_int, [vp, vp, sz, sz, sz, dbl, vp]),
        "vbx_synth_speech_f64": (C.c_int, [vp, vp, sz, C.c_uint64, dbl, C.c_uint64]),
        "vbx_selftest_lanes": (C.c_int, [vp, vp]),
        "vbx_internal_last_unsure_count": (C.c_int, [vp, vp]),
        "vbx_internal_last_burg_direct_count": (C.c_int, [vp, vp]),
        "vbx_internal_last_lpc_exact_count": (C.c_int, [vp, vp]),
        "vbx_internal_estimate_formants_counted": (C.c_int, [vp, vp, sz, sz, vp, vp, sz, vp, sz, vp, vp]),
        "vbx_internal_last_roots_direct_count": (C.c_int, [vp, vp]),
        "vbx_internal_last_spectral_split": (C.c_int, [vp]),
        "vbx_internal_last_mfcc_interp": (C.c_int, [vp]),
        "vbx_internal_last_mfcc_form": (C.c_int, [vp]),
        "vbx_internal_last_pitch_form": (C.c_int, [vp]),
        "vbx_record_doubles": (sz, [C.POINTER(AnalysisParams)]),
        "vbx_analyze_frames_f64": (C.c_int, [vp, vp, sz, sz, sz, C.POINTER(AnalysisParams), vp, sz, vp, sz, vp]),
        "vbx_analyze_frames_pcm16": (C.c_int, [vp, vp, sz, sz, sz, C.POINTER(AnalysisParams), vp, sz, vp, sz, vp]),
        "vbx_analyze_frames_tracked_f64": (C.c_int, [vp, vp, sz, sz, sz, C.POINTER(AnalysisParams), C.POINTER(PitchTrackParams),
                                                     vp, sz, vp, sz, vp, C.POINTER(PitchTrackOutputs)]),
        "vbx_analyze_frames_tracked_pcm16": (C.c_int, [vp, vp, sz, sz, sz, C.POINTER(AnalysisParams), C.POINTER(PitchTrackParams),
                                                       vp, sz, vp, sz, vp, C.POINTER(PitchTrackOutputs)]),
        "vbx_record_doubles_ex": (sz, [C.POINTER(AnalysisParams), C.POINTER(AnalysisExt)]),
        "vbx_analyze_frames_ex_f64": (C.c_int, [vp, vp, sz, sz, sz, C.POINTER(AnalysisParams), C.POINTER(AnalysisExt),
                                                C.POINTER(PitchTrackParams), vp, sz, vp, sz, vp, C.POINTER(PitchTrackOutputs)]),
        "vbx_analyze_frames_ex_pcm16": (C.c_int, [vp, vp, sz, sz, sz, C.POINTER(AnalysisParams), C.POINTER(AnalysisExt),
                                                  C.POINTER(PitchTrackParams), vp, sz, vp, sz, vp, C.POINTER(PitchTrackOutputs)]),
        "vbx_analyze_frames_ex_f32in": (C.c_int, [vp, vp, sz, sz, sz, C.POINTER(AnalysisParams), C.POINTER(AnalysisExt),
                                                  C.POINTER(PitchTrackParams), vp, sz, vp, sz, vp, C.POINTER(PitchTrackOutputs)]),
        "vbx_unpack_samples": (C.c_int, [vp, vp, sz, i32, i32, i32, vp]),
        "vbx_analyze_host": (C.c_int, [vp, vp, sz, C.POINTER(HostAudio), sz, sz, C.POINTER(AnalysisParams), C.POINTER(AnalysisExt),
                                       C.POINTER(PitchTrackParams), vp, sz, vp, sz, vp, C.POINTER(PitchTrackOutputs)]),
        "vbx_unpack_channels": (C.c_int, [vp, vp, sz, i32, i32, vp, sz, vp, sz]),
        "vbx_analyze_host_channels": (C.c_int, [vp, vp, sz, C.POINTER(HostAudio), vp, sz, sz, sz, C.POINTER(AnalysisParams),
                                                C.POINTER(AnalysisExt), C.POINTER(PitchTrackParams), vp, sz, C.POINTER(ChannelOutputs), sz]),
        "vbx_malloc_host": (C.c_int, [vp, C.POINTER(vp), sz]),
        "vbx_free_host": (C.c_int, [vp, vp]),
        "vbx_host_chunk_plan": (C.c_int, [sz, sz, sz, sz, sz, vp, sz, C.POINTER(ShardPlan), C.POINTER(sz), C.POINTER(sz)]),
        "vbx_session_plan": (C.c_int, [sz, sz, sz, sz, sz, C.POINTER(SessionPlan)]),
        "vbx_session_open": (C.c_int, [vp, C.POINTER(HostAudio), sz, sz, C.POINTER(AnalysisParams), C.POINTER(AnalysisExt),
                                       C.POINTER(PitchTrackParams), sz, C.POINTER(vp)]),
        "vbx_session_push": (C.c_int, [vp, vp, sz, vp, sz, vp, sz, C.POINTER(PitchTrackOutputs), C.POINTER(sz)]),
        "vbx_session_push_device": (C.c_int, [vp, vp, sz, vp, sz, vp, sz, C.POINTER(PitchTrackOutputs), C.POINTER(sz)]),
        "vbx_session_mark_utterance": (C.c_int, [vp]),
        "vbx_session_reset": (C.c_int, [vp]),
        "vbx_session_info": (C.c_int, [vp, C.POINTER(sz), C.POINTER(sz), C.POINTER(sz)]),
        "vbx_session_close": (None, [vp]),
        "vbx_session_channels_plan": (C.c_int, [sz, sz, sz, sz, sz, sz, sz, C.POINTER(SessionChannelsPlan), C.POINTER(C.c_int64)]),
        "vbx_session_open_channels": (C.c_int, [vp, C.POINTER(HostAudio), vp, sz, sz, sz, C.POINTER(AnalysisParams), C.POINTER(AnalysisExt),
                                                C.POINTER(PitchTrackParams), sz, C.POINTER(vp)]),
        "vbx_session_push_channels": (C.c_int, [vp, vp, sz, C.POINTER(ChannelOutputs), sz, sz, C.POINTER(sz)]),
        "vbx_session_push_channels_device": (C.c_int, [vp, vp, sz, C.POINTER(ChannelOutputs), sz, sz, C.POINTER(sz)]),
        "vbx_path_stream_open": (C.c_int, [vp, sz, C.POINTER(PitchPathParams), dbl, sz, C.POINTER(vp)]),
        "vbx_path_stream_push": (C.c_int, [vp, vp, vp, vp, vp, sz, i32, vp, sz, vp, vp, vp]),
        "vbx_path_stream_reset": (C.c_int, [vp]),
        "vbx_path_stream_close": (None, [vp]),
        "vbx_session_path_bind": (C.c_int, [vp, dbl, sz, vp, sz, vp, vp, vp]),
        "vbx_internal_session_ingest": (C.c_int, [vp, i32, i32, i32, vp, sz, sz, vp, sz, vp]),
        "vbx_session_path_bind_channels": (C.c_int, [vp, dbl, sz, C.POINTER(ChannelPathOutputs), sz]),
        "vbx_internal_session_ingest_channels": (C.c_int, [vp, i32, i32, vp, sz, vp, sz, sz, sz, vp, sz, vp, sz]),
        "vbx_g711_table": (C.c_int, [i32, C.POINTER(C.c_int16)]),
        "vbx_clips_plan": (C.c_int, [C.POINTER(sz), sz, sz, sz, sz, C.POINTER(ClipRow), C.POINTER(sz), C.POINTER(sz)]),
        "vbx_analyze_clips": (C.c_int, [vp, C.POINTER(vp), C.POINTER(sz), sz, C.POINTER(ClipFormat), sz, sz, C.POINTER(AnalysisParams),
                                        C.POINTER(AnalysisExt), C.POINTER(PitchTrackParams), vp, sz, vp, C.POINTER(PitchTrackOutputs)]),
        "vbx_internal_clips_pack": (C.c_int, [vp, i32, C.POINTER(vp), C.POINTER(sz), sz, sz, vp, C.POINTER(sz)]),
        "vbx_find_formants_resampled_f64": (C.c_int, [vp, vp, sz, sz, sz, dbl, dbl, sz, vp, sz, vp, sz, vp, vp, vp, vp, vp]),
        "vbx_shard_range": (C.c_int, [sz, i32, i32, vp, sz, C.POINTER(sz), C.POINTER(sz)]),
        "vbx_shard_samples": (C.c_int, [sz, sz, sz, sz, C.POINTER(sz), C.POINTER(sz)]),
        "vbx_shard_plan": (C.c_int, [sz, i32, i32, vp, sz, C.POINTER(ShardPlan)]),
        "vbx_shard_local_segments": (C.c_int, [C.POINTER(ShardPlan), vp, sz, vp, sz, C.POINTER(sz)]),
        "vbx_track_stitch_f64": (C.c_int, [vp, vp, sz, sz, sz, sz, vp, vp]),
        "vbx_comm_stitch_tracks_f64": (C.c_int, [vp, vp, vp, sz, sz, C.POINTER(ShardPlan), vp, i32]),
        "vbx_comm_unique_id": (C.c_int, [vp]),
        "vbx_comm_create": (C.c_int, [vp, vp, i32, i32, C.POINTER(vp)]),
        "vbx_comm_destroy": (None, [vp]),
        "vbx_gather_records_f64": (C.c_int, [vp, vp, vp, vp, sz, i32, vp, i32]),
        "vbx_gather_plan": (C.c_int, [vp, i32, i32, i32, sz, vp, vp, vp]),
        "vbx_comm_live_count": (C.c_int, []),
        "vbx_comm_wait": (C.c_int, [vp, vp, i32]),
        "vbx_comm_sync": (C.c_int, [vp]),
        "vbx_comm_selftest": (C.c_int, [vp, vp, sz]),
    }
    for name, (res, args) in sig.items():
        if name.startswith("vbx_internal_") and os.environ.get("VBX_LIB_PATH") and not hasattr(L, name):
            continue
        fn = getattr(L, name)
        fn.restype = res
        fn.argtypes = args
    _lib = L
    return L



def poly_degree(poly):
    p = np.ascontiguousarray(poly, dtype=np.complex128)
    return int(load_library().vbx_degree_c64(p.ctypes.data, p.size))


def poly_off_low(poly):
    p = np.ascontiguousarray(poly, dtype=np.complex128)
    return int(load_library().vbx_off_low_c64(p.ctypes.data, p.size))


def window_table(kind, n):
    out = np.empty(n, dtype=np.float64)
    rc = load_library().vbx_window_table_f64(kind, n, out.ctypes.data)
    if rc != 0:
        raise VoxBoxError("vbx_window_table_f64 failed")
    return out


def frame_count(n_samples, frame_len, hop):
    return int(load_library().vbx_frame_count(n_samples, frame_len, hop))


def hz_to_mel(hz):
    return load_library().vbx_hz_to_mel(hz)


def mel_to_hz(mel):
    return load_library().vbx_mel_to_hz(mel)


def mfcc_bins(frame_len, num_coeffs, lo_hz, hi_hz, sample_rate):
    out = np.zeros(num_coeffs + 2, dtype=np.int32)
    rc = load_library().vbx_mfcc_bins(frame_len, num_coeffs, lo_hz, hi_hz, sample_rate, out.ctypes.data)
    if rc < 0:
        raise VoxBoxError("vbx_mfcc_bins: bad argument")
    return out, bool(rc)


def shard_range(n_frames, world, rank, seg_start=None):
    lo, hi = C.c_size_t(), C.c_size_t()
    seg = None if seg_start is None else np.ascontiguousarray(seg_start, dtype=np.int64)
    rc = load_library().vbx_shard_range(n_frames, world, rank, None if seg is None else seg.ctypes.data,
                                        0 if seg is None else seg.size, C.byref(lo), C.byref(hi))
    if rc != 0:
        raise VoxBoxError("vbx_shard_range: bad argument")
    return lo.value, hi.value


def shard_plan(n_frames, world, rank, seg_start=None):
    plan = ShardPlan()
    seg = None if seg_start is None else np.ascontiguousarray(seg_start, dtype=np.int64)
    rc = load_library().vbx_shard_plan(n_frames, world, rank, None if seg is None else seg.ctypes.data,
                                       0 if seg is None else seg.size, C.byref(plan))
    if rc != 0:
        raise VoxBoxError("vbx_shard_plan: bad argument")
    return plan


def shard_local_segments(plan, seg_start=None):
    seg = None if seg_start is None else np.ascontiguousarray(seg_start, dtype=np.int64)
    n = C.c_size_t()
    L = load_library()
    sp, sn = (None if seg is None else seg.ctypes.data), (0 if seg is None else seg.size)
    if L.vbx_shard_local_segments(C.byref(plan), sp, sn, None, 0, C.byref(n)) != 0:
        raise VoxBoxError("vbx_shard_local_segments: bad argument")
    out = np.zeros(n.value, dtype=np.int64)
    if L.vbx_shard_local_segments(C.byref(plan), sp, sn, out.ctypes.data, out.size, C.byref(n)) != 0:
        raise VoxBoxError("vbx_shard_local_segments: bad argument")
    return out


def host_chunk_plan(n_frames, chunk_frames, c, frame_len, stride, seg_start=None):
# ... 1407 lines not shown
```

Before: 40.22 million.

## Specialise analyze kernel per input type and shrink its kernel-argument block

```diff
diff --git a/vox_box.rs_amd/csrc/k_spectral.hip b/vox_box.rs_amd/csrc/k_spectral.hip
--- a/vox_box.rs_amd/csrc/k_spectral.hip
+++ b/vox_box.rs_amd/csrc/k_spectral.hip
@@ -154,7 +154,20 @@
            L.out_r == nullptr && !L.mfcc_only && rows16;
 }
 
-int launch_analyze(hipStream_t s, const spectral_launch_t &L) {
+static int spectral_spec(const spectral_launch_t &L, bool w3, size_t extra) {
+#if defined(VBX_EXP_PHASES) || VBX_EXP_STOP != 0
+    return SP_SPEC_NONE;
+#else
+    if (!L.allow_spec || !w3 || extra != 0 || L.plan != SPECTRAL_PLAN_1200 || L.n != SP_N || L.mfcc_only || L.out_r != nullptr) return SP_SPEC_NONE;
+    if (L.x.kind != SAMPLE_F64 && L.x.kind != SAMPLE_PCM16) return SP_SPEC_NONE;
+    if (!L.lag_rcp || pitch_full_list_bytes(L.n, L.kmax) != 0) return SP_SPEC_NONE;
+    if (L.out_mfcc != nullptr && !(L.mfcc_defer && L.num_coeffs <= 16)) return SP_SPEC_NONE;
+    return L.x.kind == SAMPLE_PCM16 ? SP_SPEC_PCM16 : SP_SPEC_F64;
+#endif
+}
+
+int launch_analyze(hipStream_t s, const spectral_launch_t &L, int *launched_spec) {
+    if (launched_spec) *launched_spec = SP_SPEC_NONE;
     if (L.x.kind != SAMPLE_F64 && (L.plan != SPECTRAL_PLAN_1200 || L.n != SP_N)) return -1;
     spectral_args_t a;
     a.frames = static_cast<const double *>(L.x.p);
@@ -180,12 +193,13 @@
     if (spectral_list_parked(L)) { a.pp.full_off = -1; extra = 0; }
     const size_t lds = base + extra;
     const bool lpc = L.out_lpc != nullptr, mf = L.out_mfcc != nullptr;
+    const spectral_args_1200_t a12(a);
     if (L.mfcc_only) {
         if (L.interp && L.n != SP_N) {
             a.ip = L.ip;
             const size_t li = spectral_lds_bytes(0) > (size_t)L.ip.lds_bytes ? spectral_lds_bytes(0) : (((size_t)L.ip.lds_bytes + 15) & ~(size_t)15);
             hipLaunchKernelGGL((analyze_kernel<false, true, false, SP_MFCC_ONLY_INTERP>), grid, block, li, s, a);
-        } else hipLaunchKernelGGL((analyze_kernel<false, true, true, SP_MFCC_ONLY>), grid, block, spectral_lds_bytes(0), s, a);
+        } else hipLaunchKernelGGL((analyze_kernel<false, true, true, SP_MFCC_ONLY>), grid, block, spectral_lds_bytes(0), s, a12);
         return 0;
     }
     if (L.out_r != nullptr) {
@@ -196,14 +210,28 @@
     static const bool want3 = [] { const char *e = getenv("VBX_SPECTRAL_W3"); return e == nullptr || atoi(e) != 0; }();
     const bool w3 = want3 && extra == 0 && 12 * lds <= 160 * 1024;
     if (L.x.kind == SAMPLE_F32) {
-        launch_analyze_f32in(s, a, (unsigned)L.F, lds, lpc, mf, w3);
+        launch_analyze_f32in(s, a12, (unsigned)L.F, lds, lpc, mf, w3);
         return 0;
     }
 #define VBX_SP_LAUNCH(LPC_, MF_, FULL_)                                                                              \
     do {                                                                                                              \
-        if (w3) hipLaunchKernelGGL((analyze_kernel<LPC_, MF_, FULL_, SP_ANALYZE, 3>), grid, block, lds, s, a);        \
-        else hipLaunchKernelGGL((analyze_kernel<LPC_, MF_, FULL_>), grid, block, lds, s, a);                          \
+        if (w3) hipLaunchKernelGGL((analyze_kernel<LPC_, MF_, FULL_, SP_ANALYZE, 3>), grid, block, lds, s, a12);      \
+        else hipLaunchKernelGGL((analyze_kernel<LPC_, MF_, FULL_>), grid, block, lds, s, a12);                        \
     } while (0)
+#define VBX_SP_LAUNCH_SPEC(LPC_, MF_)                                                                                                          \
+    do {                                                                                                                                        \
+        if (spec == SP_SPEC_PCM16) hipLaunchKernelGGL((analyze_kernel<LPC_, MF_, true, SP_ANALYZE, 3, sp_launch_pcm16_t>), grid, block, lds, s, a12);   \
+        else hipLaunchKernelGGL((analyze_kernel<LPC_, MF_, true, SP_ANALYZE, 3, sp_launch_f64_t>), grid, block, lds, s, a12);          \
+    } while (0)
+    const int spec = spectral_spec(L, w3, extra);
+    if (spec != SP_SPEC_NONE) {
+        if (launched_spec) *launched_spec = spec;
+        if (lpc && mf) VBX_SP_LAUNCH_SPEC(true, true);
+        else if (lpc) VBX_SP_LAUNCH_SPEC(true, false);
+        else if (mf) VBX_SP_LAUNCH_SPEC(false, true);
+        else VBX_SP_LAUNCH_SPEC(false, false);
+        return 0;
+    }
     if (L.interp && mf && L.n != SP_N) {
         a.ip = L.ip;
         const size_t li = lds > (size_t)L.ip.lds_bytes ? lds : (((size_t)L.ip.lds_bytes + 15) & ~(size_t)15);
@@ -222,6 +250,7 @@
     else if (mf) VBX_SP_LAUNCH(false, true, true);
     else VBX_SP_LAUNCH(false, false, true);
 #undef VBX_SP_LAUNCH
+#undef VBX_SP_LAUNCH_SPEC
     return 0;
 }
 
diff --git a/vox_box.rs_amd/csrc/k_spectral_f32in.hip b/vox_box.rs_amd/csrc/k_spectral_f32in.hip
--- a/vox_box.rs_amd/csrc/k_spectral_f32in.hip
+++ b/vox_box.rs_amd/csrc/k_spectral_f32in.hip
@@ -2,7 +2,7 @@
 
 namespace vbx {
 
-void launch_analyze_f32in(hipStream_t s, const spectral_args_t &a, unsigned grid, size_t lds, bool lpc, bool mfcc, bool waves3) {
+void launch_analyze_f32in(hipStream_t s, const spectral_args_1200_t &a, unsigned grid, size_t lds, bool lpc, bool mfcc, bool waves3) {
     const dim3 g(grid), b(64);
 #define VBX_SP32_LAUNCH(LPC_, MF_)                                                                                \
     do {                                                                                                           \
diff --git a/vox_box.rs_amd/csrc/vbx_api.hip b/vox_box.rs_amd/csrc/vbx_api.hip
--- a/vox_box.rs_amd/csrc/vbx_api.hip
+++ b/vox_box.rs_amd/csrc/vbx_api.hip
@@ -163,6 +163,7 @@
     { const char *e = std::getenv("VBX_MFCC_MFMA"); ctx->mfcc_force_mfma = e && e[0] == '1'; }
     { const char *e = std::getenv("VBX_MFCC_CZT"); ctx->mfcc_czt = e ? (e[0] == '1' ? 1 : 0) : -1; }
     { const char *e = std::getenv("VBX_MFCC_DEFER"); ctx->mfcc_defer = (e && e[0] == '0') ? 0 : 1; }
+    { const char *e = std::getenv("VBX_SPECTRAL_SPEC"); ctx->spectral_spec = (e && e[0] == '0') ? 0 : 1; }
     { const char *e = std::getenv("VBX_LPC_EXACT"); ctx->lpc_policy = (e && e[0] == '0') ? VBX_LPC_POLICY_PLAIN : VBX_LPC_POLICY_EXACT; }
     { const char *e = std::getenv("VBX_POW2_SPLIT"); ctx->pow2_split = e ? (e[0] == '0' ? 0 : 1) : -1; }
     { const char *e = std::getenv("VBX_MFCC_INTERP"); ctx->mfcc_interp = e ? (e[0] == '0' ? 0 : 1) : -1; }
@@ -485,7 +486,9 @@
         }
     }
     L.mfcc_defer = L.out_mfcc != nullptr && !L.mfcc_only && L.num_coeffs >= 1 && L.num_coeffs <= 16 && ctx->mfcc_defer && L.plan == SPECTRAL_PLAN_1200;
-    { Prof p(ctx, prof_name, st); ctx->last_spectral_split = launch_analyze(st, L); }
+    L.allow_spec = ctx->spectral_spec != 0;
+    ctx->last_analyze_spec = 0;
+    { Prof p(ctx, prof_name, st); ctx->last_spectral_split = launch_analyze(st, L, &ctx->last_analyze_spec); }
     if (L.mfcc_defer && L.out_lpc == nullptr) { Prof p(ctx, "mfcc_rows", st); launch_mfcc_rows(st, L.out_mfcc, L.F, L.mfcc_ld, L.num_coeffs, L.dct); }
     {
         Prof p(ctx, "pitch_direct_fallback", st);
@@ -1065,6 +1068,7 @@
 }
 
 int vbx_internal_last_spectral_split(vbx_ctx *ctx) { return ctx ? ctx->last_spectral_split : 0; }
+int vbx_internal_last_analyze_spec(vbx_ctx *ctx) { return ctx ? ctx->last_analyze_spec : 0; }
 int vbx_internal_last_mfcc_interp(vbx_ctx *ctx) { return ctx ? ctx->last_mfcc_interp : 0; }
 int vbx_internal_last_mfcc_form(vbx_ctx *ctx) { return ctx ? ctx->last_mfcc_form : 0; }
 int vbx_internal_last_pitch_form(vbx_ctx *ctx) { return ctx ? ctx->last_pitch_form : 0; }
diff --git a/vox_box.rs_amd/csrc/vbx_ctx.hpp b/vox_box.rs_amd/csrc/vbx_ctx.hpp
--- a/vox_box.rs_amd/csrc/vbx_ctx.hpp
+++ b/vox_box.rs_amd/csrc/vbx_ctx.hpp
@@ -47,6 +47,8 @@
     int mfcc_czt = -1;
     int last_mfcc_interp = 0;
     int last_spectral_split = 0;
+    int last_analyze_spec = 0;
+    int spectral_spec = 1;
     int last_mfcc_form = 0;
     int last_pitch_form = 0;
     int mfcc_defer = 1;
diff --git a/vox_box.rs_amd/csrc/vbx_kernels.hpp b/vox_box.rs_amd/csrc/vbx_kernels.hpp
--- a/vox_box.rs_amd/csrc/vbx_kernels.hpp
+++ b/vox_box.rs_amd/csrc/vbx_kernels.hpp
@@ -176,6 +176,7 @@
     int plan; int n;
     frames_t x;
     long F; long stride; const double *window; const double *lag_window; const double *tab;
+    bool allow_spec;
     bool mfcc_defer;
     bool lag_rcp;
     double sample_rate, threshold, fmin, fmax; int kmax;
@@ -194,7 +195,7 @@
 size_t spectral_split_row_bytes(int n, double sample_rate, double fmin);
 bool spectral_supported(int n, int lpc_order, int mfcc_nb, int mfcc_b_lo, int num_coeffs);
 bool spectral_list_parked(const spectral_launch_t &L);
-int launch_analyze(hipStream_t s, const spectral_launch_t &L);
+int launch_analyze(hipStream_t s, const spectral_launch_t &L, int *launched_spec = nullptr);
 void launch_mfcc_rows(hipStream_t s, double *rows, long F, long ld, int num_coeffs, const double *dct);
 bool lpc_exact_supported(int n, int p);
 void launch_lpc_exact_list(hipStream_t s, const int32_t *frame_list, const int32_t *list_count, int cus, frames_t x, int n, long stride,
diff --git a/vox_box.rs_amd/csrc/vbx_pitch_refine.hpp b/vox_box.rs_amd/csrc/vbx_pitch_refine.hpp
--- a/vox_box.rs_amd/csrc/vbx_pitch_refine.hpp
+++ b/vox_box.rs_amd/csrc/vbx_pitch_refine.hpp
@@ -825,13 +825,13 @@
 #endif
 #define VBX_STOP_AT(k_) do { if (VBX_EXP_STOP == (k_)) return true; } while (0)
 #define VBX_STOP_AT_PICK(k_, c_) do { if (VBX_EXP_STOP == (k_)) { if (lane == 0 && out_count != nullptr) out_count[f] = (c_); return true; } } while (0)
-template <int STAGE = 0, int NB = 0, bool ONCE = false>
+template <int STAGE = 0, int NB = 0, bool ONCE = false, typename LATE = std::nullptr_t>
 __device__ __forceinline__ bool pitch_refine_store(double *ys, int n, const pitch_params_t &pp, long f,
                                                    double *__restrict__ out_cand, long cand_ld,
                                                    int32_t *__restrict__ out_count, int32_t *__restrict__ status,
                                                    unsigned long long *__restrict__ work, double unc_tol = 0.0,
                                                    double2 *full = nullptr, int *io_ncand = nullptr, int cand_cap = 0,
-                                                   uint16_t *list_at = nullptr) {
+                                                   uint16_t *list_at = nullptr, LATE late = nullptr) {
     const int lane = lane_id();
     const double sample_rate = pp.sample_rate, threshold = pp.threshold, fmin = pp.fmin, fmax = pp.fmax;
     const int kmax = pp.kmax;
@@ -1172,6 +1172,7 @@
       else run_groups(std::integral_constant<int, RG>{}, std::false_type{});
     }
 #undef VBX_BAR
+    if constexpr (!std::is_same<LATE, std::nullptr_t>::value) late(out_cand, cand_ld, out_count, status, work);
     VBX_PHASE(work, f, 9);
     const int total_cand = ncand + 1;
     st = __any(st & 4) ? 4 : 0;
diff --git a/vox_box.rs_amd/csrc/vbx_spectral.hpp b/vox_box.rs_amd/csrc/vbx_spectral.hpp
--- a/vox_box.rs_amd/csrc/vbx_spectral.hpp
+++ b/vox_box.rs_amd/csrc/vbx_spectral.hpp
@@ -53,6 +53,34 @@
     int32_t *far_list;
 };
 
+struct spectral_args_1200_t {
+    const double *frames; long n_frames; long stride; const double *window; const double *lag_window;
+    const double2 *tab;
+    int n; int mfcc_q; int pcm; int num_coeffs;
+    double *out_cand; long cand_ld; int32_t *out_count; int32_t *pitch_status; unsigned long long *work;
+    int32_t *unsure_list; int32_t *unsure_count; int nb;
+    pitch_params_t pp;
+    double *out_lpc; long lpc_ld;
+    double *out_mfcc; long mfcc_ld; int32_t *mfcc_status;
+    const int32_t *bins; const double *slopes; const double *dct;
+    explicit spectral_args_1200_t(const spectral_args_t &a)
+        : frames(a.frames), n_frames(a.n_frames), stride(a.stride), window(a.window), lag_window(a.lag_window), tab(a.tab), n(a.n),
+          mfcc_q(a.mfcc_q), pcm(a.pcm), num_coeffs(a.num_coeffs),
+          out_cand(a.out_cand), cand_ld(a.cand_ld), out_count(a.out_count), pitch_status(a.pitch_status), work(a.work),
+          unsure_list(a.unsure_list), unsure_count(a.unsure_count), nb(a.nb), pp(a.pp),
+          out_lpc(a.out_lpc), lpc_ld(a.lpc_ld), out_mfcc(a.out_mfcc), mfcc_ld(a.mfcc_ld), mfcc_status(a.mfcc_status),
+          bins(a.bins), slopes(a.slopes), dct(a.dct) {}
+};
+static_assert(offsetof(spectral_args_1200_t, out_cand) == 64 && offsetof(spectral_args_1200_t, nb) + sizeof(int) <= 128, "the last stores' arguments: one 64-byte line");
+__host__ __device__ constexpr bool sp_wide_args(int mode) { return mode == SP_AC_ONLY || sp_is_interp(mode); }
+
+constexpr int SP_SPEC_NONE = 0, SP_SPEC_F64 = 1, SP_SPEC_PCM16 = 2;
+struct sp_launch_f64_t {};
+struct sp_launch_pcm16_t {};
+template <typename TIN> constexpr int sp_spec_of() {
+    return std::is_same<TIN, sp_launch_f64_t>::value ? SP_SPEC_F64 : std::is_same<TIN, sp_launch_pcm16_t>::value ? SP_SPEC_PCM16 : SP_SPEC_NONE;
+}
+
 constexpr int SP_TAIL = 16;
 __device__ __forceinline__ void spectral_exact_tail(double *ys, int n, const double *__restrict__ xf, const double *__restrict__ window,
                                                     const double *__restrict__ lag_window, double x0, double scale, int lane) {
@@ -105,7 +133,7 @@
 constexpr int SP_LPC_P = SPECTRAL_LPC_ORDER;
 
 
-void launch_analyze_f32in(hipStream_t s, const spectral_args_t &a, unsigned grid, size_t lds, bool lpc, bool mfcc, bool waves3);
+void launch_analyze_f32in(hipStream_t s, const spectral_args_1200_t &a, unsigned grid, size_t lds, bool lpc, bool mfcc, bool waves3);
 int launch_analyze_pow2(hipStream_t s, const spectral_launch_t &L, spectral_args_t &a);
 
 }
diff --git a/vox_box.rs_amd/csrc/vbx_spectral_1200.hpp b/vox_box.rs_amd/csrc/vbx_spectral_1200.hpp
--- a/vox_box.rs_amd/csrc/vbx_spectral_1200.hpp
+++ b/vox_box.rs_amd/csrc/vbx_spectral_1200.hpp
@@ -186,9 +186,22 @@
     return VBX_EXP_FRONT_END_ONCE != 0 && !(!mfcc && full && waves >= 3 && !f32);
 }
 __host__ __device__ constexpr int sp_cell_blocks(int waves, bool f32) { return f32 ? VBX_EXP_CELL_NB_F32IN : VBX_EXP_CELL_NB; }
+template <int MODE> using sp_args_of = typename std::conditional<sp_wide_args(MODE), spectral_args_t, spectral_args_1200_t>::type;
+template <typename ARGS>
+__device__ __forceinline__ const __attribute__((address_space(4))) ARGS *sp_args_where_used() {
+    const __attribute__((address_space(4))) ARGS *p = (const __attribute__((address_space(4))) ARGS *)__builtin_amdgcn_kernarg_segment_ptr();
+    asm volatile("" : "+s"(p));
+    return p;
+}
 template <bool LPC, bool MFCC, bool FULL, int MODE = SP_ANALYZE, int WAVES = VBX_SPECTRAL_WAVES, typename TIN = double>
-__global__ __launch_bounds__(64) __attribute__((amdgpu_waves_per_eu(sp_is_mfcc_only(MODE) ? 2 : WAVES, sp_is_mfcc_only(MODE) ? 4 : WAVES))) void analyze_kernel(const spectral_args_t a) {
+__global__ __launch_bounds__(64) __attribute__((amdgpu_waves_per_eu(sp_is_mfcc_only(MODE) ? 2 : WAVES, sp_is_mfcc_only(MODE) ? 4 : WAVES))) void analyze_kernel(const sp_args_of<MODE> a) {
     constexpr bool F32 = std::is_same<TIN, float>::value;
+    using args_t = sp_args_of<MODE>;
+    constexpr int SPEC = sp_spec_of<TIN>();
+    static_assert(SPEC == SP_SPEC_NONE || (FULL && MODE == SP_ANALYZE && WAVES >= 3), "the launch-specialised form: full f64 / PCM frames, three wavefronts");
+    constexpr bool SP = SPEC != SP_SPEC_NONE;
+#define VBX_SP_PCM_IN (SP ? SPEC == SP_SPEC_PCM16 : (a.pcm & SP_FLAG_PCM) != 0)
+#define VBX_SP_LAG_RCP (SP || (a.pcm & SP_FLAG_LAG_RCP) != 0)
     static_assert(!F32 || (FULL && MODE == SP_ANALYZE), "float samples: the fused analysis of full frames");
     static_assert(MODE != SP_MFCC_ONLY || (MFCC && FULL && !LPC), "the MFCC-only form needs the full frame and has no lag sums");
     static_assert(MODE != SP_AC_ONLY || (!MFCC && !LPC), "the autocorrelation-only form");
@@ -224,7 +237,7 @@
                 xs32[q] = float2{lo, hi};
                 wv[q] = (a.window != nullptr) ? (((uintptr_t)a.window & 15) == 0 ? *reinterpret_cast<const double2 *>(a.window + i)
                                                                                   : double2{a.window[i], a.window[i + 1]}) : double2{1.0, 1.0};
-            } else if (FULL && (a.pcm & SP_FLAG_PCM)) {
+            } else if (FULL && VBX_SP_PCM_IN) {
                 int lo, hi;
                 if ((((uintptr_t)x16) & 3) == 0) { const int w = *reinterpret_cast<const int *>(x16 + i); lo = (short)(w & 0xffff); hi = w >> 16; }
                 else { lo = x16[i]; hi = x16[i + 1]; }
@@ -433,9 +446,14 @@
         }
         wave_sync();
         VBX_PHASE(a.work, f, 13);
+        if constexpr (SP) {
+            mfcc_tail_q(pu, pd, en, a.bins, nullptr, a.num_coeffs, b_lo, lane, a.out_mfcc + f * a.mfcc_ld, nullptr, f, true);
+            if (a.mfcc_status != nullptr && lane == 0) a.mfcc_status[f] = 0;
+        } else {
         if (a.num_coeffs <= 16) mfcc_tail_q(pu, pd, en, a.bins, a.dct, a.num_coeffs, b_lo, lane, a.out_mfcc + f * a.mfcc_ld, a.work, f, (a.pcm & SP_FLAG_MFCC_DEFER) != 0);
         else mfcc_tail_m(pu, pd, en, a.bins, a.dct, a.num_coeffs, b_lo, lane, a.out_mfcc + f * a.mfcc_ld);
         if (a.mfcc_status != nullptr && lane == 0) a.mfcc_status[f] = 0;
+        }
         wave_sync();
     }
 
@@ -463,12 +481,12 @@
         for (int s = 0; s < 11; s++) {
             const int i = 2 * jj[s];
             if (jj[s] >= 0 && i < n) {
-                const double xs = F32 ? (double)x32[i] : (FULL && (a.pcm & SP_FLAG_PCM)) ? pcm16_value(x16[i]) : xf[i];
+                const double xs = F32 ? (double)x32[i] : (FULL && VBX_SP_PCM_IN) ? pcm16_value(x16[i]) : xf[i];
                 const double xe = (a.window != nullptr) ? xs * a.window[i] : xs;
                 r_e[s] = (r_e[s] - x0 * xe) + x0;
             }
             if (jj[s] >= 0 && i + 1 < n) {
-                const double xs = F32 ? (double)x32[i + 1] : (FULL && (a.pcm & SP_FLAG_PCM)) ? pcm16_value(x16[i + 1]) : xf[i + 1];
+                const double xs = F32 ? (double)x32[i + 1] : (FULL && VBX_SP_PCM_IN) ? pcm16_value(x16[i + 1]) : xf[i + 1];
                 const double xo = (a.window != nullptr) ? xs * a.window[i + 1] : xs;
                 r_o[s] = (r_o[s] - x0 * xo) + x0;
             }
@@ -505,7 +523,7 @@
     const double scale = 1.0 / amax;
     double *ys = smem;
     wave_sync();
-    const bool by_table = (a.pcm & SP_FLAG_LAG_RCP) != 0 && fabs(scale) < 1e290 && fabs(scale) > 1e-290;
+    const bool by_table = VBX_SP_LAG_RCP && fabs(scale) < 1e290 && fabs(scale) > 1e-290;
     const double *lag_rcp = a.lag_window + lag_rcp_offset(n);
     if (by_table) {
 #ifndef VBX_EXP_LB
@@ -568,11 +586,29 @@
     wave_sync();
     VBX_PHASE(a.work, f, 5);
     const double unc_tol = SP_UNC_EPS * fabs(s0) * scale;
+    if constexpr (SP) {
+        pitch_params_t pp;
+        pp.sample_rate = a.pp.sample_rate; pp.threshold = a.pp.threshold; pp.fmin = a.pp.fmin; pp.fmax = a.pp.fmax; pp.kmax = a.pp.kmax;
+        pp.full_off = 0; pp.f32 = 0; pp.ncurve = 0;
+        auto late = [&](auto &out_cand, auto &cand_ld, auto &out_count, auto &status, auto &work) __attribute__((always_inline)) {
+            const auto *l = sp_args_where_used<args_t>();
+            out_cand = l->out_cand; cand_ld = l->cand_ld; out_count = l->out_count; status = l->pitch_status; work = l->work;
+        };
+        if (!pitch_refine_store<0, sp_cell_blocks(WAVES, F32), sp_front_end_once(MFCC, FULL, WAVES, F32)>(ys, n, pp, f, nullptr, 0, nullptr, nullptr, nullptr, unc_tol, nullptr,
+                                                                                                        nullptr, 0, nullptr, late)) {
+            const auto *l = sp_args_where_used<args_t>();
+            int32_t *const unsure_count = l->unsure_count;
+            if (lane == 0) l->unsure_list[atomicAdd(unsure_count, 1)] = (int32_t)f;
+        }
+        return;
+    }
     double2 *full = a.pp.full_off > 0 ? reinterpret_cast<double2 *>(reinterpret_cast<char *>(smem) + a.pp.full_off)
                   : a.pp.full_off < 0 ? reinterpret_cast<double2 *>(a.out_cand + f * a.cand_ld) : nullptr;
     if (!pitch_refine_store<0, sp_cell_blocks(WAVES, F32), sp_front_end_once(MFCC, FULL, WAVES, F32)>(ys, n, a.pp, f, a.out_cand, a.cand_ld, a.out_count, a.pitch_status, a.work, unc_tol, full)) {
         if (lane == 0) a.unsure_list[atomicAdd(a.unsure_count, 1)] = (int32_t)f;
     }
 }
-
-}
+#undef VBX_SP_PCM_IN
+#undef VBX_SP_LAG_RCP
+
+}
diff --git a/vox_box.rs_amd/voxbox.py b/vox_box.rs_amd/voxbox.py
--- a/vox_box.rs_amd/voxbox.py
+++ b/vox_box.rs_amd/voxbox.py
@@ -296,6 +296,7 @@
         "vbx_internal_estimate_formants_counted": (C.c_int, [vp, vp, sz, sz, vp, vp, sz, vp, sz, vp, vp]),
         "vbx_internal_last_roots_direct_count": (C.c_int, [vp, vp]),
         "vbx_internal_last_spectral_split": (C.c_int, [vp]),
+        "vbx_internal_last_analyze_spec": (C.c_int, [vp]),
         "vbx_internal_last_mfcc_interp": (C.c_int, [vp]),
         "vbx_internal_last_mfcc_form": (C.c_int, [vp]),
         "vbx_internal_last_pitch_form": (C.c_int, [vp]),
```

Result: faster. 41.34 million, median of 6 (+2.8%).
